# SuperbTUM/real-time-ReID-tracking

Hardware: AMD Instinct MI355X
Metric: crops/sec embedded + NxM distmat ms, ResNet18-SE 128x256 (higher is better)
Workload: dtype f16x3; 1 GPU; BASELINE configs[1]: ResNet18-SE embed 4096 distinct uint8 crops (128x256) per GPU + 4096x4096 L2 distmat; crops_per_gpu=4096, embed_dim=512, chunk=1024

## Files before the change

include/reid_hip_debug.h:

```cpp
#pragma once
#include "reid_hip.h"

#ifdef __cplusplus
extern "C" {
#endif

int reid_debug_set_switch(reid_ctx* ctx, const char* name, long long value);
int reid_debug_get_switch(reid_ctx* ctx, const char* name, long long* value);
int reid_debug_conv_f16(reid_ctx* ctx, int n, int h, int w, int cin, int cout, int r, int stride, int pad, int cfg, int iters,
                        float* ms_per_launch);
int reid_debug_conv_split(reid_ctx* ctx, int n, int h, int w, int c, int cout, int ablate, int iters, float* ms_per_launch);
int reid_debug_conv_f32(reid_ctx* ctx, int n, int h, int w, int cin, int cout, int r, int stride, int pad, int flags,
                        int variant, int iters, float* ms_per_launch);
int reid_debug_conv_c64(reid_ctx* ctx, int n, const float* x, const float* w_krsc, const float* scale, const float* shift,
                        const float* residual, int relu, float* out, float* stats);
int reid_debug_gemm_f16(reid_ctx* ctx, int m, int n, int k, int cfg, int iters, float* ms_per_launch,
                        unsigned long long* diag_host);
int reid_debug_linear(reid_ctx* ctx, int m, int n, int k, int mode, int iters, float* ms_per_launch);
int reid_debug_linear_rows(reid_ctx* ctx, const float* x, const float* w, const float* bias, const float* res, int m, int n, int k,
                           int mode, int flags, float* out);
int reid_debug_conv_layer(reid_ctx* ctx, const float* x, int n, int h, int w, int cin, const float* wgt, int cout, int r, int stride,
                          int pad, const float* scale, const float* shift, const float* residual, int relu, int relu_from, int pack_from,
                          int want_stats, const float* a_scale, const float* a_shift, int a_relu, float* out, uint16_t* packed,
                          float* stats, int* packed_written);
int reid_debug_conv_layer_f16(reid_ctx* ctx, const uint16_t* x, int n, int h, int w, int cin, const uint16_t* wgt, int cout, int r, int stride,
                              int pad, const float* scale, const float* shift, const uint16_t* residual, int relu, int want_stats,
                              uint16_t* out, float* stats, int* form);
int reid_debug_conv_c64_se(reid_ctx* ctx, int n, const uint16_t* x, const uint16_t* w_folded, const float* shift, const uint16_t* residual,
                           int relu, const float* se_w1, const float* se_w2t, uint16_t* out, float* stats, int* form);
int reid_debug_norm_finish(reid_ctx* ctx, int form, int n, int hw, int c, int half, int tiles, const void* x, const float* stats,
                           const float* in_gamma, const float* in_beta, const float* bn_scale, const float* bn_shift, float* out,
                           uint16_t* out16, float* a_scale, float* a_shift);
int reid_debug_se_tail(reid_ctx* ctx, int form, int n, int hw, int c, int mid, int tiles, const float* stats, const float* w1,
                       const float* w2t, const void* y, const void* shortcut, float* out, uint16_t* out16, float* gate);
int reid_debug_sibling_tail(reid_ctx* ctx, int arch, int n, int h, int w, int c, const float* prm, const float* y, const float* shortcut,
                            float* out);
int reid_debug_gem_neck(reid_ctx* ctx, int f16, int n, int hw, int c, float p, const void* x, const float* scale, const float* shift,
                        float* gem_out, float* emb);
int reid_debug_any_norm(reid_ctx* ctx, int n, int hw, int c, int half, const float* x, const float* in_gamma, const float* in_beta,
                        const float* bn_scale, const float* bn_shift, float* out);
int reid_debug_any_se_tail(reid_ctx* ctx, int n, int hw, int c, int mid, const float* w1, const float* w2t, const float* y,
                           const float* shortcut, float* out, float* gate);
int reid_debug_any_gem(reid_ctx* ctx, int n, int hw, int c, float p, const float* x, const float* scale, const float* shift, float* gem_out,
                       float* emb);
int reid_debug_any_conv(reid_ctx* ctx, int hw_precision, const float* x, int n, int h, int w, int cin, const float* wgt, int cout, int r,
                        int stride, int pad, const float* scale, const float* shift, const float* residual, int relu, int relu_from, float* out,
                        int* form_out);
int reid_debug_any_front(reid_ctx* ctx, int fused, const uint8_t* src, int64_t src_bytes, const int64_t* offsets, const int32_t* hw, int n,
                         int pitch, int out_h, int out_w, const float* mean_std6, const float* stem_w, const float* scale, const float* shift,
                         float* out);
int reid_debug_gem_neck_fused(reid_ctx* ctx, int n, int hw, int c, int mid, int tiles, float p, const float* stats, const float* w1,
                              const float* w2t, const float* y, const float* shortcut, const float* scale, const float* shift,
                              float* gem_out, float* emb);
int reid_debug_stem(reid_ctx* ctx, int form, int is_u8, const void* x, int n, const float* w, const float* scale, const float* shift,
                    float* out, uint16_t* out16);
int reid_debug_resize_norm(reid_ctx* ctx, const uint8_t* packed, const long long* offsets, const int* hw, int n, int pitch, float* out);
int reid_debug_swin_crop_front(reid_ctx* ctx, const uint8_t* packed, const long long* offsets, const int* hw, int n, int pitch, int out_h,
                               int out_w, const float* mean_std6, const float* c1_w, const float* c1_b, float* out);
int reid_debug_swin_conv1(reid_ctx* ctx, const float* x, int n, int h, int w, const float* c1_w, const float* c1_b, float* out);
int reid_debug_swin_conv1_mirror(reid_ctx* ctx, const float* x, int n, int h, int w, const float* c1_w, const float* c1_b, float* out);
int reid_debug_swin_crop_front_mirror(reid_ctx* ctx, const uint8_t* packed, const long long* offsets, const int* hw, int n, int pitch, int out_h,
                                      int out_w, const float* mean_std6, const float* c1_w, const float* c1_b, float* out);
int reid_debug_swin_descriptor(reid_ctx* ctx, const float* e1, const float* e2, const float* cls_w, int n, int num_class, int out_rows, int ld,
                               float* out);
int reid_debug_pil_resize(reid_ctx* ctx, const uint8_t* packed, const long long* offsets, const int* hw, int n, int out_h, int out_w,
                          const float* mean_std6, uint8_t* u8_out, float* f32_out);
int reid_debug_maxpool(reid_ctx* ctx, int f16, const void* x, int n, int h, int w, int c, void* out);
int reid_debug_window_attn_cos(reid_ctx* ctx, int mode, const float* qkv, int n, int h, int w, int heads, int shifted, const float* bias,
                               const float* scale, float* out, uint16_t* out16);
int reid_debug_post_norm(reid_ctx* ctx, int side, const float* x, const float* y, int t, int c, const float* g, const float* b, int in_place,
                         float* out, uint16_t* out16);
int reid_debug_window_attn(reid_ctx* ctx, int form, const float* qkv, int n, int h, int w, int heads, int shifted, const float* pos169,
                           float* out, uint16_t* out16);
int reid_debug_layernorm(reid_ctx* ctx, int form, const float* x, int t, int c, const float* g, const float* b, float* out, uint16_t* out16);
int reid_debug_ln_linear(reid_ctx* ctx, const float* x, const float* ln_g, const float* ln_b, const float* w, const float* bias, int t, int c,
                         int n, float* out);
int reid_debug_swin_linear(reid_ctx* ctx, const float* x, const float* w, const float* bias, const float* res, int m, int n, int k,
                           int precision, int flags, int out_form, int ldc, float* out, uint16_t* out16, int* form);
int reid_debug_swin_sfe(reid_ctx* ctx, const float* c1, int n, int h1, int w1, const float* in_g, const float* in_b, const float* bn_s,
                        const float* bn_t, const float* c2_w, const float* c2_b, const float* fc_w, const float* fc_b, float* ab, float* tok);
int reid_debug_swin_tail(reid_ctx* ctx, const float* x, int n, int ntok, const float* g, const float* b, float p, const float* bn_s,
                         const float* bn_t, float* gem, float* emb);
int reid_debug_swin_merge(reid_ctx* ctx, int stage, const float* x, int n, int h, int w, float* out);
int reid_debug_swin_fuse(reid_ctx* ctx, const float* sfe, const float* x1, const float* x2, const float* x3, const float* x4, int n, int h1,
                         int w1, void* a0, void* f3, void* f2, float* f1);
int reid_debug_bank_cost96(reid_ctx* ctx, reid_bank* bank, const int32_t* slots, int t, const float* dets_host, int m, int metric, float gate,
                           float* out_host);
// ... 24 lines not shown
```

real-time-reid-tracking_amd/_ffi.py:

```python
import ctypes as C
import os

_HERE = os.path.dirname(os.path.abspath(__file__))
LIB_PATH = os.path.join(_HERE, "libreid_hip.so")
LIB_PATH = os.environ.get("REID_HIP_LIB", LIB_PATH)

METRIC_L2, METRIC_L2SQR, METRIC_COS_HALF, METRIC_COS, METRIC_DOT = range(5)
COMM_ID_BYTES = 128
K_CONV_GEMM, K_DIST_GEMM, K_ELEMENTWISE, K_SELECT = range(4)

_vp, _i, _sz = C.c_void_p, C.c_int, C.c_size_t
_SIGS = {
    "reid_last_error": (C.c_char_p, []),
    "reid_device_count": (_i, [C.POINTER(_i)]),
    "reid_ctx_create": (_i, [_i, C.POINTER(_vp)]),
    "reid_ctx_destroy": (_i, [_vp]),
    "reid_ctx_set_stream": (_i, [_vp, _vp]),
    "reid_ctx_set_null_stream": (_i, [_vp]),
    "reid_ctx_sync": (_i, [_vp]),
    "reid_device_sync": (_i, [_vp]),
    "reid_ctx_clear_fault": (_i, [_vp]),
    "reid_ctx_set_chunk": (_i, [_vp, _i]),
    "reid_ctx_set_precision": (_i, [_vp, _i]),
    "reid_ctx_precision_ok": (_i, [_vp, _i, _i]),
# ... 46 lines not shown
    "reid_argmin_rows_x3": (_i, [_vp, _vp, _i, _vp, _i, _i, _i, _vp, _vp]),
    "reid_argmin_rows_x3_dev": (_i, [_vp, _vp, _i, _vp, _i, _i, _i, _vp, _vp]),
    "reid_knn_x3": (_i, [_vp, _vp, _i, _vp, _i, _i, _i, _vp, _vp]),
    "reid_knn_x3_dev": (_i, [_vp, _vp, _i, _vp, _i, _i, _i, _vp, _vp]),
    "reid_descriptor_f32_nchw": (_i, [_vp, _vp, _i, _i, _vp]),
    "reid_descriptor_f32_nchw_dev": (_i, [_vp, _vp, _i, _i, _vp]),
    "reid_descriptor_images_u8": (_i, [_vp, _vp, _vp, _vp, _i, _vp, _i, _vp]),
    "reid_descriptor_f32_nchw_hw": (_i, [_vp, _vp, _i, _i, _i, _i, _vp]),
    "reid_descriptor_f32_nchw_hw_dev": (_i, [_vp, _vp, _i, _i, _i, _i, _vp]),
    "reid_descriptor_images_u8_hw": (_i, [_vp, _vp, _vp, _vp, _i, _i, _i, _vp, _i, _vp]),
    "reid_cam_debias": (_i, [_vp, _vp, _vp, _i, _i, C.c_float, _i]),
    "reid_cam_debias_dev": (_i, [_vp, _vp, _vp, _i, _i, C.c_float, _i]),
    "reid_smooth_tracklets": (_i, [_vp, _vp, _vp, _vp, _i, _i, C.c_float]),
    "reid_smooth_tracklets_dev": (_i, [_vp, _vp, _vp, _vp, _i, _i, C.c_float]),
    "reid_bank_create": (_i, [_vp, _i, _i, _i, C.POINTER(_vp)]),
    "reid_bank_destroy": (_i, [_vp]),
    "reid_bank_update": (_i, [_vp, _vp, _vp, _vp, _i]),
    "reid_bank_update_dev": (_i, [_vp, _vp, _vp, _vp, _i]),
    "reid_bank_clear": (_i, [_vp, _vp, _vp, _i]),
    "reid_bank_count": (_i, [_vp, _i, C.POINTER(_i)]),
    "reid_bank_cost": (_i, [_vp, _vp, _vp, _i, _vp, _i, _i, C.c_float, _vp]),
    "reid_bank_cost_dev": (_i, [_vp, _vp, _vp, _i, _vp, _i, _i, C.c_float, _vp]),
    "reid_host_alloc": (_i, [_vp, _sz, C.POINTER(_vp)]),
    "reid_host_free": (_i, [_vp, _vp]),
    "reid_frame_submit": (_i, [_vp, _i, _vp, _vp, _vp, _i]),
    "reid_frame_submit_hw": (_i, [_vp, _i, _vp, _vp, _vp, _i, _i, _i, _vp]),
    "reid_frame_submit_swin": (_i, [_vp, _i, _vp, _vp, _vp, _i, _i, _i, _vp]),
    "reid_frame_cost": (_i, [_vp, _i, _vp, _vp, _i, _i, C.c_float, _vp, _vp, _i]),
    "reid_frame_cost_groups": (_i, [_vp, _i, _i, _vp, _vp, _vp, _vp, _i, C.c_float, _vp, _vp, _i]),
    "reid_frame_match_stream": (_i, [_vp, _i]),
    "reid_frame_fetch": (_i, [_vp, _i, _vp, _vp, _vp]),
    "reid_frame_gather": (_i, [_vp, _i, _i]),
    "reid_frame_update": (_i, [_vp, _i, _vp, _vp, _vp, _i]),
    "reid_rerank_jaccard": (_i, [_vp, _vp, _i, _i, _i, _i, _vp, _vp]),
    "reid_rerank_jaccard_dev": (_i, [_vp, _vp, _i, _i, _i, _i, _vp, _vp]),
    "reid_diou": (_i, [_vp, _vp, _vp, _i, _vp]),
    "reid_diou_cost": (_i, [_vp, _vp, _i, _vp, _i, _vp]),
    "reid_rank_eval": (_i, [_vp, _vp, _vp, _vp, _i, _vp, _vp, _vp, _i, _i, _vp, _vp, _vp]),
    "reid_rank_eval_dev": (_i, [_vp, _vp, _vp, _vp, _i, _vp, _vp, _vp, _i, _i, _vp, _vp, _vp]),
    "reid_comm_unique_id": (_i, [_vp]),
    "reid_comm_init": (_i, [_vp, _i, _i, _vp]),
    "reid_comm_info": (_i, [_vp, C.POINTER(_i), C.POINTER(_i)]),
    "reid_comm_destroy": (_i, [_vp]),
    "reid_allgather_dev": (_i, [_vp, _vp, _vp, _sz]),
    "reid_allgather_rows_dev": (_i, [_vp, _vp, _i, _sz, _vp, _vp, C.POINTER(_i)]),
    "reid_allreduce_f64": (_i, [_vp, C.POINTER(C.c_double), _i, _i]),
    "reid_knn_gallery_sharded_dev": (_i, [_vp, _vp, _i, _vp, _i, _i, _i, _i, _vp, _vp]),
    "reid_conv2d_nhwc": (_i, [_vp, _vp, _i, _i, _i, _i, _vp, _i, _i, _i, _i, _i, _vp, _vp, _vp, _i, _vp]),
    "reid_gemm_nt": (_i, [_vp, _vp, _i, _vp, _i, _i, _vp, _vp]),
}
EXPORTS = tuple(sorted(_SIGS))

DEBUG_LIB_PATH = os.path.join(_HERE, "libreid_hip_debug.so")
DEBUG_EXPORTS = ("reid_debug_any_conv", "reid_debug_any_front", "reid_debug_any_gem", "reid_debug_any_norm", "reid_debug_any_se_tail", "reid_debug_bank_cost96", "reid_debug_coissue", "reid_debug_comm_loopback", "reid_debug_conv_c64", "reid_debug_conv_c64_se", "reid_debug_conv_layer", "reid_debug_conv_layer_f16", "reid_debug_conv_split", "reid_debug_conv_diag", "reid_debug_conv_f16", "reid_debug_conv_f32",
                 "reid_debug_feed", "reid_debug_gem_neck", "reid_debug_gem_neck_fused", "reid_debug_gemm_f16", "reid_debug_knn_merge", "reid_debug_knn_wide", "reid_debug_layernorm", "reid_debug_linear", "reid_debug_linear_rows", "reid_debug_ln_linear", "reid_debug_maxpool", "reid_debug_mfma_bare", "reid_debug_mfma_shape", "reid_debug_norm_finish", "reid_debug_pil_resize", "reid_debug_post_norm", "reid_debug_resize_norm", "reid_debug_se_tail", "reid_debug_stem", "reid_debug_sibling_tail", "reid_debug_swin_conv1", "reid_debug_swin_conv1_mirror", "reid_debug_swin_crop_front", "reid_debug_swin_crop_front_mirror", "reid_debug_swin_descriptor", "reid_debug_swin_fuse", "reid_debug_swin_linear", "reid_debug_swin_merge", "reid_debug_swin_sfe", "reid_debug_swin_tail", "reid_debug_select_exp", "reid_debug_select_x3", "reid_debug_set_switch", "reid_debug_get_switch", "reid_debug_two_linear", "reid_debug_two_linear_ablate", "reid_debug_two_linear_form", "reid_debug_window_attn", "reid_debug_window_attn_cos")

_lib = None
_dbg = None


class ReidHipError(RuntimeError):
    status = None


def lib():
    global _lib
    if _lib is None:
        if not os.path.exists(LIB_PATH):
            raise ReidHipError(
                "HIP extension missing: %s (build it with `python -c 'import __graft_entry__ as g; g.build()'` "
                "or `make -C real-time-reid-tracking_amd/csrc`); there is no CPU fallback" % LIB_PATH)
        l = C.CDLL(LIB_PATH, mode=C.RTLD_GLOBAL)
        for name, (res, args) in _SIGS.items():
            fn = getattr(l, name)
            fn.restype = res
            fn.argtypes = args
        _lib = l
    return _lib


def debug_lib():
    global _dbg
    if _dbg is None:
        lib()
        if not os.path.exists(DEBUG_LIB_PATH):
            raise ReidHipError("debug library missing: %s (make -C real-time-reid-tracking_amd/csrc)" % DEBUG_LIB_PATH)
        _dbg = C.CDLL(DEBUG_LIB_PATH)
    return _dbg


def check(status):
    if status != 0:
        msg = lib().reid_last_error()
        err = ReidHipError("libreid_hip status %d: %s" % (status, msg.decode() if msg else "?"))
        err.status = int(status)
        raise err
```

real-time-reid-tracking_amd/csrc/api.hip:

```cpp
#include "reid_internal.h"
#include "siblings_f16.h"
#include "anysize.h"
#include "anysize_x3.h"
#include "distmat_x3.h"
#include "select_x3.h"
#include "anysize_front.h"
#include <cmath>
#include <dlfcn.h>
#include <mutex>
#include <stdarg.h>
#include <stdio.h>
#include <string.h>
#include <stdlib.h>
#include <sstream>

static thread_local char g_err[1024] = "";

void reid_set_error(const char* fmt, ...) {
    va_list ap;
    va_start(ap, fmt);
    vsnprintf(g_err, sizeof(g_err), fmt, ap);
    va_end(ap);
}

extern "C" const char* reid_last_error(void) { return g_err; }

extern "C" int reid_device_count(int* n) {
    ARG_CHECK(n);
    HIP_TRY(hipGetDeviceCount(n));
    return REID_OK;
}

extern "C" int reid_ctx_create(int device, reid_ctx** out) {
    ARG_CHECK(out);
    int n = 0;
    HIP_TRY(hipGetDeviceCount(&n));
    if (device < 0 || device >= n) {
        reid_set_error("reid_ctx_create: device %d not available (%d visible)", device, n);
        return REID_ERR_ARG;
    }
    DeviceGuard _dev_guard(device);
    reid_ctx* c = new reid_ctx();
    c->device = device;
    if (const char* e = getenv("REID_SWIN_CHUNK_MAX")) {
        const int v = atoi(e);
        if (v > 0 && v < c->swin_chunk_cap) c->swin_chunk_cap = v;
    }
    if (const char* e = getenv("REID_KNN_WIDE_MIN")) c->knn_wide_min = atoll(e);
    HIP_TRY(hipStreamCreateWithFlags(&c->own_stream, hipStreamNonBlocking));
    c->stream = c->own_stream;
    HIP_TRY(hipHostMalloc((void**)&c->fault, 64, hipHostMallocMapped));
    memset(c->fault, 0, 64);
    HIP_TRY(hipEventCreate(&c->t0));
    HIP_TRY(hipEventCreate(&c->t1));
    *out = c;
    return REID_OK;
}

extern "C" int reid_ctx_destroy(reid_ctx* ctx) {
    if (!ctx) return REID_OK;
    DeviceGuard _dev_guard(ctx->device);
// ... 492 lines not shown
        w.num_cams = (int)(cb->second.second / 512);
        w.cam_factor = blob[cf->second.first];
    }
    if (missing) {
        reid_set_error("reid_seres18_load: manifest entry '%s' missing or of unexpected size", first_missing.c_str());
        HIP_TRY(hipFree(w.blob));
        w = Se18Weights();
        return REID_ERR_ARG;
    }
    {
        std::vector<float> ep(8 * 1024, 0.f);
        for (int i = 0; i < 8; ++i) {
            const Se18Block& b = w.blk[i];
            const int half = b.ibn ? b.c / 2 : 0;
            for (int ch = 0; ch < b.c; ++ch) {
                ep[i * 1024 + ch] = ch < half ? 1.f : blob[(b.bn1_scale - w.blob) + (ch - half)];
                ep[i * 1024 + 512 + ch] = ch < half ? 0.f : blob[(b.bn1_shift - w.blob) + (ch - half)];
            }
        }
        HIP_TRY(hipMalloc((void**)&w.ep, ep.size() * sizeof(float)));
        HIP_TRY(hipMemcpy(w.ep, ep.data(), ep.size() * sizeof(float), hipMemcpyHostToDevice));
    }
    HIP_TRY(hipMalloc((void**)&w.blob16, n_floats * sizeof(_Float16)));
    HIP_TRY(hipMalloc((void**)&w.stem_w16, 64 * 256 * sizeof(_Float16)));
    HIP_TRY(hipMalloc((void**)&w.stem_w16s, 64 * 256 * sizeof(_Float16)));
    HIP_TRY(hipMalloc((void**)&w.zero_page, 256));
    HIP_TRY(hipMemsetAsync(w.zero_page, 0, 256, ctx->stream));
    REID_TRY(launch_f32_to_f16(ctx, w.blob, n_floats, w.blob16));
    REID_TRY(launch_stem_w16(ctx, w.stem_w, w.stem_w16));
    REID_TRY(launch_stem_w16_scaled(ctx, w.stem_w, w.stem_scale, w.stem_w16s));
    for (int i = 0; i < 2; ++i) {
        HIP_TRY(hipMalloc((void**)&w.l1_conv2_w16s[i], 64 * 576 * sizeof(_Float16)));
        REID_TRY(launch_scale_rows_f16(ctx, w.blk[i].conv2_w, w.blk[i].bn2_scale, 64, 576, w.l1_conv2_w16s[i]));
    }
    HIP_TRY(hipStreamSynchronize(ctx->stream));
    w.loaded = true;
    return REID_OK;
}

extern "C" int reid_seres18_dims(reid_ctx* ctx, int* embed_dim, int* num_class) {
    ARG_CHECK(ctx);
    CTX_GUARD(ctx);
    if (!ctx->se18.loaded) {
        reid_set_error("no weights loaded");
        return REID_ERR_STATE;
    }
    if (embed_dim) *embed_dim = 512;
    if (num_class) *num_class = ctx->se18.num_class;
    return REID_OK;
}

static const int IMG_H = 256, IMG_W = 128;

static bool conv_split_path(reid_ctx* ctx, int n, int H, int W, int Cin, int Cout, int R, int S, int stride, int pad) {
    if (ctx->precision != 2 || Cin % 64 != 0 || Cout % 64 != 0 || !ctx->se18.zero_page) return false;
    Gemm16Params q;
    memset(&q, 0, sizeof(q));
    q.H = H; q.W = W; q.Cin = ctx->split_terms * Cin; q.R = R; q.S = S; q.stride = stride; q.pad = pad;
    q.Ho = (H + 2 * pad - R) / stride + 1;
    q.Wo = (W + 2 * pad - S) / stride + 1;
    q.M = n * q.Ho * q.Wo; q.N = Cout;
    const bool halo = R == 3 && S == 3 && stride == 1 && pad == 1 && conv3x3_f16_supported(q);
    const bool enough = halo || (Cout % 128 == 0 && (long long)(q.M / 256) * (Cout / 128) >= (R == 3 ? ctx->split_gemm_min_tiles * 3 / 4 : ctx->split_gemm_min_tiles));
    if (q.M % 128 == 0 && !enough && !halo && ctx->conv_x3s == 2) {
        q.split_terms = ctx->split_terms; q.ldb = (long long)R * S * q.Cin; q.ldc = Cout;
        return conv_x3s_supported(ctx, q);
    }
    return q.M % 128 == 0 && enough;
}

int conv_gemm(reid_ctx* ctx, int amode, const void* x, int n, int H, int W, int Cin, const float* wgt, int Cout, int R,
                     int S, int stride, int pad, int Kpad, const float* a_scale, const float* a_shift, int a_relu,
                     const float* col_scale, const float* col_shift, const float* residual, int relu, float* stats,
                     float* out, int relu_from, const _Float16* x_packed, _Float16* out_packed, int pack_from, bool* packed_written) {
    if (packed_written) *packed_written = false;
    GemmParams p;
    memset(&p, 0, sizeof(p));
    p.A = x;
    p.H = H; p.W = W; p.Cin = Cin; p.R = R; p.S = S; p.stride = stride; p.pad_y = pad; p.pad_x = pad;
    p.Ho = (H + 2 * pad - R) / stride + 1;
    p.Wo = (W + 2 * pad - S) / stride + 1;
    p.a_scale = a_scale; p.a_shift = a_shift; p.a_relu = a_relu;
    p.B = wgt; p.ldb = Kpad;
    p.M = n * p.Ho * p.Wo; p.N = Cout; p.K = Kpad;
    p.C = out; p.ldc = Cout;
    p.col_scale = col_scale; p.col_shift = col_shift; p.residual = residual; p.relu = relu; p.stats = stats;
    p.relu_from = relu_from;
    p.diag = ctx->conv_diag;
    const double ktrue = (double)R * S * Cin;
    const double flops = 2.0 * p.M * Cout * ktrue;
    const double in_bytes = (double)n * H * W * Cin * (amode == A_STEM_U8 ? 1.0 : 4.0);
    const double bytes = in_bytes + ((double)p.M * Cout + (double)Cout * ktrue) * 4.0 + (residual ? (double)p.M * Cout * 4.0 : 0.0);
    if (amode == A_IM2COL && !a_scale && conv_split_path(ctx, n, H, W, Cin, Cout, R, S, stride, pad)) {
        Gemm16Params q;
        memset(&q, 0, sizeof(q));
        const int T = ctx->split_terms;
        q.split_terms = T;
        q.H = H; q.W = W; q.Cin = T * Cin; q.R = R; q.S = S; q.stride = stride; q.pad = pad;
        q.Ho = p.Ho; q.Wo = p.Wo;
        q.M = p.M; q.N = Cout; q.K = R * S * T * Cin; q.ldb = q.K;
        const bool halo = R == 3 && S == 3 && stride == 1 && pad == 1 && conv3x3_f16_supported(q);
        {
            const _Float16* a16 = x_packed;
            if (!a16) {
                _Float16* buf;
                const long long rows_in = (long long)n * H * W;
                REID_TRY(ctx_ws(ctx, "split.a", (size_t)rows_in * 2 * Cin * 2, (void**)&buf));
// ... 11 lines not shown
            q.B = (const _Float16*)it->second;
            q.C32 = out; q.ldc = Cout;
            q.col_scale = col_scale; q.col_shift = col_shift; q.res32 = residual; q.relu = relu; q.relu_from = relu_from;
            q.stats = stats;
            q.acc_scale = 1.0f / 2048.0f;
            q.zero_page = ctx->se18.zero_page;
            if (out_packed && packed_written && pack_from % 32 == 0) {
                q.pack16 = out_packed;
                q.pack_from = pack_from;
                *packed_written = true;
            }
            if (halo) return launch_conv3x3_split(ctx, q, REID_K_CONV_GEMM, flops, bytes);
            if (conv_x3s_supported(ctx, q)) return launch_conv_x3s(ctx, q, REID_K_CONV_GEMM, flops, bytes);
            return launch_gemm_f16_split(ctx, q, REID_K_CONV_GEMM, flops, bytes);
        }
    }
    if (amode == A_IM2COL && ctx->f32_conv && conv_f32_supported(p)) return launch_conv_f32(ctx, p, REID_K_CONV_GEMM, flops, bytes);
    return launch_gemm_f32(ctx, amode, E_CONV, p, REID_K_CONV_GEMM, flops, bytes);
}

int conv_weights_fresh(reid_ctx* ctx, const float* d_w) {
    auto it = ctx->split_w.find(d_w);
    if (it != ctx->split_w.end()) {
        HIP_TRY(hipStreamSynchronize(ctx->stream));
        (void)hipFree(it->second);
        ctx->split_w.erase(it);
    }
    return REID_OK;
}

int conv_weights_splittable(reid_ctx* ctx, const float* h_w, size_t count, const char* who) {
    if (ctx->precision != 2) return REID_OK;
    for (size_t i = 0; i < count; ++i)
        if (!(fabsf(h_w[i]) * 2048.0f < 65504.0f)) {
            reid_set_error("%s: weight %zu (%g) is outside the range the fp32-class arithmetic (reid_ctx_set_precision 2) can split "
                           "(|w| 2^11 < 65504); use mode 0", who, i, (double)h_w[i]);
            return REID_ERR_ARG;
        }
    return REID_OK;
}

static int split_weights_of(reid_ctx* ctx, const float* wgt, int Cout, int taps, int Cin, const _Float16** out) {
    auto it = ctx->split_w.find(wgt);
    if (it == ctx->split_w.end()) {
        void* w16;
        HIP_TRY(hipMalloc(&w16, (size_t)Cout * taps * ctx->split_terms * Cin * 2));
        REID_TRY(launch_split_weights(ctx, wgt, Cout, taps, Cin, ctx->split_terms, (_Float16*)w16));
        it = ctx->split_w.emplace(wgt, w16).first;
    }
    *out = (const _Float16*)it->second;
    return REID_OK;
}

#ifdef REID_EXPERIMENTS
static int seres18_chain_layer4(reid_ctx* ctx, int n, const Se18Block& ka, const Se18Block& kb, const _Float16* in16, const float* sc,
                                float* y, float* out_a, float* out, float* stats) {
    const int H = 16, W = 8, hw = 128, C = 512, SK = 4, nnt = C / 128;
    const int nmt = (n * hw + 255) / 256;
    _Float16 *c1_16, *a16;
    float* skws;
    int* cnt;
    REID_TRY(ctx_ws(ctx, "split.c1", (size_t)n * hw * C * 2 * 2, (void**)&c1_16));
    REID_TRY(ctx_ws(ctx, "chain.a16", (size_t)n * hw * C * 2 * 2, (void**)&a16));
    const size_t part = (size_t)nmt * nnt * SK * 256 * 128;
    REID_TRY(ctx_ws(ctx, "chain.splitk", 4 * part * sizeof(float), (void**)&skws));
    const bool fresh = ctx->ws.find("chain.cnt") == ctx->ws.end();
    REID_TRY(ctx_ws(ctx, "chain.cnt", (4 * 1024 + 64 + 8 * 64) * sizeof(int), (void**)&cnt));
    if (fresh) HIP_TRY(hipMemsetAsync(cnt, 0, (4 * 1024 + 64 + 8 * 64) * sizeof(int), ctx->stream));
    ChainParams cp;
    memset(&cp, 0, sizeof(cp));
    cp.n_img = n;
    cp.flags = ctx->chain;
    cp.counters = cnt + 4 * 1024;
    cp.fault = ctx->fault;
    auto conv = [&](int idx, const _Float16* a, int cin, const float* wgt, const float* scale, const float* shift, const float* res, int relu,
                    float* stats_out, _Float16* pack) -> int {
        Gemm16Params& q = cp.conv[idx];
        q.H = H; q.W = W; q.Cin = 3 * cin; q.R = 3; q.S = 3; q.stride = 1; q.pad = 1; q.Ho = H; q.Wo = W;
        q.M = n * hw; q.N = C; q.K = 9 * 3 * cin; q.ldb = q.K;
        q.split_terms = 3;
        q.A = a;
        REID_TRY(split_weights_of(ctx, wgt, C, 9, cin, &q.B));
        q.C32 = y; q.ldc = C;
        q.col_scale = scale; q.col_shift = shift; q.res32 = res; q.relu = relu; q.relu_from = 0;
        q.stats = stats_out;
        q.acc_scale = 1.0f / 2048.0f;
        q.zero_page = ctx->se18.zero_page;
        q.pack16 = pack; q.pack_from = 0;
        q.split_k = SK; q.splitk_ws = skws + (size_t)idx * part; q.splitk_cnt = cnt + idx * 1024;
        q.fault = ctx->fault;
        return REID_OK;
    };
    REID_TRY(conv(0, in16, ka.cin, ka.conv1_w, ka.bn1_scale, ka.bn1_shift, nullptr, 1, nullptr, c1_16));
    REID_TRY(conv(1, c1_16, C, ka.conv2_w, ka.bn2_scale, ka.bn2_shift, nullptr, 0, stats, nullptr));
    REID_TRY(conv(2, a16, C, kb.conv1_w, kb.bn1_scale, kb.bn1_shift, nullptr, 1, nullptr, c1_16));
    REID_TRY(conv(3, c1_16, C, kb.conv2_w, kb.bn2_scale, kb.bn2_shift, out_a, 1, stats, nullptr));
    const int slices = 2;
    auto se = [&](int idx, const Se18Block& k, const float* shortcut, float* o, _Float16* pk) {
        ChainElem& e = cp.el[idx];
        e.x = y; e.stats = stats; e.sc = shortcut; e.g = k.se_w1; e.b = k.se_w2; e.out = o; e.packed = pk;
        e.c = C; e.half = 0; e.hw = hw; e.tiles = 1; e.mid = k.mid; e.slices = slices;
    };
    se(0, ka, sc, out_a, a16);
    se(1, kb, out_a, out, nullptr);
    const int conv_items = nmt * nnt * SK, se_items = n * slices;
    const int kinds[6] = {0, 0, 2, 0, 0, 2}, idxs[6] = {0, 1, 0, 2, 3, 1};
    const int targets[6] = {0, nnt * SK, nnt * SK, slices, nnt * SK, nnt * SK};
    int first = 0;
    for (int s = 0; s < 6; ++s) {
        ChainStage& st = cp.st[s];
        st.kind = kinds[s]; st.idx = idxs[s]; st.first = first; st.items = kinds[s] == 0 ? conv_items : se_items;
        st.dep = s - 1; st.target = targets[s]; st.sk = SK;
        first += st.items;
    }
    cp.n_stages = 6;
    cp.total_items = first;
    prof_begin(ctx, REID_K_CONV_GEMM, 2.0 * n * hw * C * 9.0 * (ka.cin + 3.0 * C), 0.0);
    const int st = launch_chain(ctx, cp, W);
    prof_end(ctx);
    return st;
}
#endif

struct Se18Bufs {
    float *stem, *pool, *t[4], *stats, *a_scale, *a_shift, *se, *gem;
    float* stage[11];
};

static int seres18_forward(reid_ctx* ctx, const void* x, bool is_u8, int n, float* d_emb, float* d_logits) {
    Se18Weights& w = ctx->se18;
    if (!w.loaded) {
        reid_set_error("reid_embed_*: call reid_seres18_load first");
        return REID_ERR_STATE;
    }
    Se18Bufs b;
    const size_t per = 131072;
    const bool keep = ctx->debug_keep != 0;
    REID_TRY(ctx_ws(ctx, "se18.stem", (size_t)n * 524288 * 4, (void**)&b.stem));
    REID_TRY(ctx_ws(ctx, "se18.pool", (size_t)n * per * 4, (void**)&b.pool));
    const int nt = keep ? 1 : 4;
    float* tbase = nullptr;
    REID_TRY(ctx_ws(ctx, "se18.t", (size_t)n * per * 4 * (keep ? 4 * 8 : 4), (void**)&tbase));
    REID_TRY(ctx_ws(ctx, "se18.stats", (size_t)n * 2048 * 4, (void**)&b.stats));
    REID_TRY(ctx_ws(ctx, "se18.ascale", (size_t)n * 512 * 4, (void**)&b.a_scale));
    REID_TRY(ctx_ws(ctx, "se18.ashift", (size_t)n * 512 * 4, (void**)&b.a_shift));
    REID_TRY(ctx_ws(ctx, "se18.se", (size_t)n * 512 * 4, (void**)&b.se));
    REID_TRY(ctx_ws(ctx, "se18.gem", (size_t)n * 512 * 4, (void**)&b.gem));
    (void)nt;

    const bool pool_fused = ctx->f32_conv == 1 && ctx->f32_stem_pool && ctx->debug_keep != 1;
    _Float16* cur16 = nullptr;
    const bool split_mode = ctx->precision == 2 && w.arch == 0 && ctx->f32_conv == 1;
    if (split_mode) REID_TRY(ctx_ws(ctx, "split.cur", (size_t)n * per * 2 * 2, (void**)&cur16));
    const bool stem_split = split_mode && pool_fused && ctx->stem_split;
    if (stem_split) {
        REID_TRY(launch_stem_split(ctx, x, is_u8, n, w.stem_w, w.stem_scale, w.stem_shift, b.pool, cur16));
    } else if (pool_fused) {
        REID_TRY(launch_stem_f32(ctx, x, is_u8, n, w.stem_w, w.stem_scale, w.stem_shift, b.pool, true));
    } else if (ctx->f32_conv == 1) {
        REID_TRY(launch_stem_f32(ctx, x, is_u8, n, w.stem_w, w.stem_scale, w.stem_shift, b.stem, false));
    } else {
        REID_TRY(conv_gemm(ctx, is_u8 ? A_STEM_U8 : A_STEM_F32, x, n, IMG_H, IMG_W, 3, w.stem_w, 64, 7, 7, 2, 3, 192, nullptr,
                           nullptr, 0, w.stem_scale, w.stem_shift, nullptr, 0, nullptr, b.stem));
    }
    if (!pool_fused) REID_TRY(launch_maxpool3s2(ctx, b.stem, n, 128, 64, 64, b.pool));
    b.stage[0] = b.stem;
    b.stage[1] = b.pool;

    const float* cur = b.pool;
    int H = 64, W = 32;
    bool gem_done = false;
    if (split_mode && !stem_split) REID_TRY(launch_split_pack(ctx, b.pool, (long long)n * 64 * 32, 64, cur16));
    for (int i = 0; i < 8; ++i) {
        const Se18Block& k = w.blk[i];
#ifdef REID_EXPERIMENTS
        if (i == 6 && (ctx->chain & 1) && cur16 && !keep && n <= 64 && ctx->pack_epilogue && ctx->split_terms == 3) {
            float* fr[3];
            int nf = 0;
            for (int j = 0; j < 4 && nf < 3; ++j)
                if (tbase + (size_t)j * n * per != cur) fr[nf++] = tbase + (size_t)j * n * per;
            float *sc = fr[0], *y = fr[1], *out_a = fr[2], *out = const_cast<float*>(cur);
            REID_TRY(conv_gemm(ctx, A_IM2COL, cur, n, H, W, k.cin, k.ds_w, k.c, 1, 1, k.stride, 0, k.cin, nullptr, nullptr, 0, k.ds_scale, k.ds_shift,
                               nullptr, 0, nullptr, sc, 0, cur16));
            REID_TRY(seres18_chain_layer4(ctx, n, k, w.blk[7], cur16, sc, y, out_a, out, b.stats));
            b.stage[8] = out_a;
            b.stage[9] = out;
            cur = out;
            break;
        }
#endif
        float* tb[4];
        for (int j = 0; j < 4; ++j) tb[j] = tbase + ((size_t)(keep ? i * 4 : 0) + j) * n * per;
        float* free_[3];
        int nf = 0;
        for (int j = 0; j < 4 && nf < 3; ++j)
            if (tb[j] != cur) free_[nf++] = tb[j];
        float* c1 = free_[0];
        float* y = free_[1];
        float* sc = free_[2];
        const int Ho = (H + 2 - 3) / k.stride + 1, Wo = (W + 2 - 3) / k.stride + 1;
        const int hw = Ho * Wo, tiles = hw / 128;
        const int half = k.ibn ? k.c / 2 : 0;
        _Float16* c1_16 = nullptr;
        if (ctx->f32_conv == 1) {
            bool packed_c1 = false;
            if (cur16 && !keep && ctx->pack_epilogue) REID_TRY(ctx_ws(ctx, "split.c1", (size_t)n * hw * k.c * 2 * 2, (void**)&c1_16));
            if (k.ibn) {
                REID_TRY(conv_gemm(ctx, A_IM2COL, cur, n, H, W, k.cin, k.conv1_w, k.c, 3, 3, k.stride, 1, 9 * k.cin, nullptr, nullptr,
                                   0, w.ep + (size_t)i * 1024, w.ep + (size_t)i * 1024 + 512, nullptr, 1, b.stats, c1, half, cur16,
                                   c1_16, half, &packed_c1));
                if (cur16 && !keep) {
                    if (!c1_16) REID_TRY(ctx_ws(ctx, "split.c1", (size_t)n * hw * k.c * 2 * 2, (void**)&c1_16));
                    REID_TRY(launch_in_apply_pack(ctx, c1, b.stats, n, tiles, k.c, half, hw, k.in_gamma, k.in_beta, c1_16, packed_c1));
                } else {
                    REID_TRY(launch_in_apply(ctx, c1, b.stats, n, tiles, k.c, half, hw, k.in_gamma, k.in_beta));
                }
            } else {
                REID_TRY(conv_gemm(ctx, A_IM2COL, cur, n, H, W, k.cin, k.conv1_w, k.c, 3, 3, k.stride, 1, 9 * k.cin, nullptr, nullptr,
                                   0, k.bn1_scale, k.bn1_shift, nullptr, 1, nullptr, c1, 0, cur16, c1_16, 0, &packed_c1));
                if (!packed_c1) c1_16 = nullptr;
            }
            REID_TRY(conv_gemm(ctx, A_IM2COL, c1, n, Ho, Wo, k.c, k.conv2_w, k.c, 3, 3, 1, 1, 9 * k.c, nullptr, nullptr, 0,
                               k.bn2_scale, k.bn2_shift, k.ds ? nullptr : cur, k.ds ? 0 : 1, b.stats, y, 0, c1_16));
        } else {
        REID_TRY(conv_gemm(ctx, A_IM2COL, cur, n, H, W, k.cin, k.conv1_w, k.c, 3, 3, k.stride, 1, 9 * k.cin, nullptr, nullptr, 0,
                           nullptr, nullptr, nullptr, 0, b.stats, c1));
        REID_TRY(launch_norm_finalize(ctx, b.stats, n, tiles, k.c, half, hw, k.in_gamma, k.in_beta, k.bn1_scale, k.bn1_shift,
                                      b.a_scale, b.a_shift));
        REID_TRY(conv_gemm(ctx, A_IM2COL, c1, n, Ho, Wo, k.c, k.conv2_w, k.c, 3, 3, 1, 1, 9 * k.c, b.a_scale, b.a_shift, 1,
                           k.bn2_scale, k.bn2_shift, k.ds ? nullptr : cur, k.ds ? 0 : 1, b.stats, y));
        }
        const float* shortcut = cur;
        if (k.ds) {
            REID_TRY(conv_gemm(ctx, A_IM2COL, cur, n, H, W, k.cin, k.ds_w, k.c, 1, 1, k.stride, 0, k.cin, nullptr, nullptr, 0,
                               k.ds_scale, k.ds_shift, nullptr, 0, nullptr, sc, 0, cur16));
            shortcut = sc;
        }
        float* out = c1;
        if (w.arch == 1) {
            REID_TRY(launch_ta_tail(ctx, y, shortcut, n, Ho, Wo, k.c, k.ta, out));
        } else if (w.arch == 2) {
            REID_TRY(launch_ema_tail(ctx, y, shortcut, n, Ho, Wo, k.c, k.ema, out));
        } else if (ctx->f32_conv == 1) {
            bool fp32_read = true;
            if (cur16 && !keep && i < 7 && w.blk[i + 1].ds && ctx->pack_epilogue) {
                const Se18Block& nx = w.blk[i + 1];
                fp32_read = !(conv_split_path(ctx, n, Ho, Wo, nx.cin, nx.c, 3, 3, nx.stride, 1) &&
                              conv_split_path(ctx, n, Ho, Wo, nx.cin, nx.c, 1, 1, nx.stride, 0));
            }
            if (i == 7 && !keep && n >= ctx->gem_tail_min) {
                REID_TRY(launch_gem_neck_tail(ctx, b.stats, n, tiles, k.c, k.mid, hw, k.se_w1, k.se_w2, y, shortcut, w.gem_p, w.neck_scale,
                                              w.neck_shift, b.gem, d_emb));
                gem_done = true;
            } else {
                REID_TRY(launch_se_tail(ctx, b.stats, n, tiles, k.c, k.mid, hw, k.se_w1, k.se_w2, y, shortcut, fp32_read ? out : nullptr,
                                        i < 7 ? cur16 : nullptr));
            }
        } else {
            REID_TRY(launch_se_finalize(ctx, b.stats, n, tiles, k.c, k.mid, hw, k.se_w1, k.se_w2, b.se));
            REID_TRY(launch_se_combine(ctx, y, shortcut, b.se, n, hw, k.c, out));
        }
        b.stage[2 + i] = out;
        cur = out;
        H = Ho;
        W = Wo;
    }
    if (!gem_done) REID_TRY(launch_gem_neck(ctx, cur, n, H * W, 512, w.gem_p, w.neck_scale, w.neck_shift, b.gem, d_emb));
    {
        const int32_t* d_cam;
        REID_TRY(ctx_take_side(ctx, n, w.num_cams, "reid_embed (camera bias)", &d_cam));
        if (d_cam) REID_TRY(launch_add_indexed_rows(ctx, d_emb, n, 1, 512, w.cam_bias, d_cam, w.cam_factor));
    }
    b.stage[10] = b.gem;
    if (d_logits) {
        if (!w.cls_w) {
            reid_set_error("logits requested but the weight blob has no classifier (cls.w)");
            return REID_ERR_STATE;
        }
        GemmParams p;
        memset(&p, 0, sizeof(p));
        p.A = d_emb; p.lda = 512;
        p.B = w.cls_w; p.ldb = 512;
        p.M = n; p.N = w.num_class; p.K = 512;
        p.C = d_logits; p.ldc = w.num_class;
        REID_TRY(launch_gemm_f32(ctx, A_DENSE, E_BIAS, p, REID_K_CONV_GEMM, 2.0 * n * w.num_class * 512,
                                 ((double)n * 512 + (double)w.num_class * 512 + (double)n * w.num_class) * 4.0));
    }
    ctx->last_n = n;
    ctx->last_f16 = false;
    for (int s = 0; s < 11; ++s) { ctx->stage_ptr[s] = b.stage[s]; ctx->stage_elems[s] = 0; }
    return REID_OK;
}

int open_beside_self(const char* file, const char* what, std::initializer_list<const char*> names, void** fns) {
    Dl_info info;
    std::string path = file;
    if (dladdr((const void*)&open_beside_self, &info) && info.dli_fname) {
        const std::string self = info.dli_fname;
        const size_t slash = self.rfind('/');
        if (slash != std::string::npos) path = self.substr(0, slash + 1) + path;
    }
    void* h = dlopen(path.c_str(), RTLD_NOW | RTLD_LOCAL);
    if (!h) {
// ... 1465 lines not shown
```

real-time-reid-tracking_amd/csrc/conv3x3_x3.hip:

```cpp
#include "reid_internal.h"
#include "conv3x3_geom.h"
#include "lin_math.h"
#include <type_traits>
#include <utility>

typedef _Float16 f16;
typedef f16 half8 __attribute__((ext_vector_type(8)));
typedef float f32x16 __attribute__((ext_vector_type(16)));

namespace {

#define GPTR(p) ((const __attribute__((address_space(1))) void*)(p))
#define LPTR(p) ((__attribute__((address_space(3))) void*)(uintptr_t)(p))
#define RAW_BARRIER() asm volatile("s_barrier" ::: "memory")
#define LDS_READ(dst, addr, off) asm volatile("ds_read_b128 %0, %1 offset:%2" : "=v"(dst) : "v"(addr), "n"(off))

template <int N>
__device__ __forceinline__ void lgkm_wait2(half8& x, half8& y) { asm volatile("s_waitcnt lgkmcnt(%2)" : "+v"(x), "+v"(y) : "n"(N)); }
template <int N>
__device__ __forceinline__ void lgkm_wait1(half8& x) { asm volatile("s_waitcnt lgkmcnt(%1)" : "+v"(x) : "n"(N)); }

__device__ __forceinline__ void wait_vm(int n) {
    switch (n) {
        case 0: asm volatile("s_waitcnt vmcnt(0)" ::: "memory"); break;
// ... 263 lines not shown
                            dst[p.N] = (f16)((v - (float)hv) * 2048.0f);
                        } else {
                            p.C32[(long long)(m_blk + row) * ldc + col] = v;
                        }
                    }
                }
            }
            s1[b] = t1;
            s2[b] = t2;
        }
    }
    if (p.fault && !(vmax < 65504.f)) p.fault[0] = 1;
    if (p.stats) {
        float* stat_lds = (float*)lds;
#pragma unroll
        for (int b = 0; b < TN; ++b) {
            const int lcol = b * 32 + li;
            const float t1 = s1[b] + __shfl_xor(s1[b], 32);
            const float t2 = s2[b] + __shfl_xor(s2[b], 32);
            if (lh == 0) {
                stat_lds[(wm * BN + lcol) * 2 + 0] = t1;
                stat_lds[(wm * BN + lcol) * 2 + 1] = t2;
            }
        }
        __syncthreads();
        for (int t = tid; t < 2 * BN; t += 256) {
            const int half = t / BN, cc = t - half * BN;
            if (half * 128 >= m_valid) continue;
            float* o = p.stats + ((long long)(mtile * 2 + half) * p.N + n_blk + cc) * 2;
            o[0] = stat_lds[((half * 2) * BN + cc) * 2 + 0] + stat_lds[((half * 2 + 1) * BN + cc) * 2 + 0];
            o[1] = stat_lds[((half * 2) * BN + cc) * 2 + 1] + stat_lds[((half * 2 + 1) * BN + cc) * 2 + 1];
        }
    }
}

typedef float f32x4 __attribute__((ext_vector_type(4)));

__device__ __forceinline__ int pi16(int i) { return i < 8 ? i : (i < 12 ? i + 4 : i - 4); }

typedef unsigned u32x2 __attribute__((ext_vector_type(2)));
typedef unsigned u32x4 __attribute__((ext_vector_type(4)));

__device__ __forceinline__ float row16_sum(float v) {
    v += __builtin_bit_cast(float, __builtin_amdgcn_update_dpp(0, __builtin_bit_cast(int, v), 0xB1, 0xf, 0xf, false));
    v += __builtin_bit_cast(float, __builtin_amdgcn_update_dpp(0, __builtin_bit_cast(int, v), 0x4E, 0xf, 0xf, false));
    v += __builtin_bit_cast(float, __builtin_amdgcn_update_dpp(0, __builtin_bit_cast(int, v), 0x141, 0xf, 0xf, false));
    v += __builtin_bit_cast(float, __builtin_amdgcn_update_dpp(0, __builtin_bit_cast(int, v), 0x140, 0xf, 0xf, false));
    return v;
}

template <int N>
__device__ __forceinline__ void lgkm_wait0() { asm volatile("s_waitcnt lgkmcnt(%0)" ::"n"(N) : "memory"); }

template <int TW, int IMGS, int BN, bool LIN = false, int COH = 0>
__device__ __forceinline__ void x3m16_tail(const Gemm16Params& p, f32x4 (&acc)[4][BN / 16], char* lds, int tid, int wm, int mtile, int n_blk,
                                           int tile_id, int ksplit, int SK) {
    constexpr int TM = 4, TN = BN / 16;
    const int lane = tid & 63;
    const int l16 = lane & 15, lq = lane >> 4;
    const int pj = pi16(l16);
    asm volatile("s_nop 15\n\ts_nop 15" ::: "memory");
#pragma unroll
    for (int a = 0; a < TM; ++a) {
        if constexpr (TN == 8)
            asm volatile("" : "+v"(acc[a][0]), "+v"(acc[a][1]), "+v"(acc[a][2]), "+v"(acc[a][3]), "+v"(acc[a][4]), "+v"(acc[a][5]), "+v"(acc[a][6]), "+v"(acc[a][7]));
        else
            asm volatile("" : "+v"(acc[a][0]), "+v"(acc[a][1]), "+v"(acc[a][2]), "+v"(acc[a][3]));
    }
    __syncthreads();

    bool sk_path = false;
    if (SK > 1) {
        sk_path = true;
        constexpr int PART_B = 256 * BN * 4;
        char* part = (char*)(p.splitk_ws + (long long)tile_id * SK * (256 * BN));
        const __amdgpu_buffer_rsrc_t w_rs = __builtin_amdgcn_make_buffer_rsrc((void*)part, 0, SK * PART_B, 0x00020000);
        const int nb_own = TN / SK;
        const unsigned own32 = (unsigned)(uintptr_t)lds + 4096u + (unsigned)tid * 16u;
#pragma unroll
        for (int a = 0; a < TM; ++a)
#pragma unroll
            for (int b = 0; b < TN; ++b) {
                if (b / nb_own == ksplit)
                    asm volatile("ds_write_b128 %0, %1" ::"v"(own32 + (unsigned)((a * nb_own + (b - ksplit * nb_own)) * 4096)), "v"(acc[a][b]) : "memory");
                else
                    __builtin_amdgcn_raw_buffer_store_b128(__builtin_bit_cast(u32x4, acc[a][b]), w_rs, tid * 16, ksplit * PART_B + (a * TN + b) * 4096, 16 );
            }
        asm volatile("s_waitcnt vmcnt(0)" ::: "memory");
        __syncthreads();
        if (tid == 0) {
            __hip_atomic_fetch_add(p.splitk_cnt + tile_id, 1, __ATOMIC_RELAXED, __HIP_MEMORY_SCOPE_AGENT);
            int spins = 0;
            while (__hip_atomic_load(p.splitk_cnt + tile_id, __ATOMIC_RELAXED, __HIP_MEMORY_SCOPE_AGENT) < SK) {
                __builtin_amdgcn_s_sleep(1);
                if (++spins > (1 << 23)) {
                    if (p.fault) p.fault[2] = 1;
                    break;
                }
            }
        }
        __syncthreads();
    }

    if (p.ablate & 32) return;
    const int ldc = (int)p.ldc;
    const int m_blk = mtile * 256;
    const int m_valid = p.M - m_blk;
    const bool wave_live = wm * 64 < m_valid;
    const int pq = lq < 2 ? lq : 5 - lq;
    const int lrow = TW == 8 ? 32 * (pj >> 3) + (pj & 7) : pj;
    const int col0 = n_blk + 4 * pq;
    const __amdgpu_buffer_rsrc_t c_rs = __builtin_amdgcn_make_buffer_rsrc((void*)(p.C32 + (long long)m_blk * ldc), 0, 256 * ldc * 4, 0x00020000);
    const __amdgpu_buffer_rsrc_t r_rs =
        __builtin_amdgcn_make_buffer_rsrc((void*)((p.res32 ? p.res32 : p.C32) + (long long)m_blk * ldc), 0, 256 * ldc * 4, 0x00020000);
    const __amdgpu_buffer_rsrc_t k_rs =
        __builtin_amdgcn_make_buffer_rsrc((void*)((p.pack16 ? p.pack16 : (f16*)p.C32) + (long long)m_blk * 2 * p.N), 0, 256 * 2 * p.N * 2, 0x00020000);
    int voff_a[TM], koff_a[TM];
#pragma unroll
    for (int a = 0; a < TM; ++a) {
        const bool row_ok = wm * 64 + (TW == 8 ? a * 8 : a * 16) + lrow < m_valid;
        voff_a[a] = row_ok ? (lrow * ldc + col0) * 4 : 0x7fffff00;
        koff_a[a] = row_ok ? (lrow * 2 * p.N + col0) * 2 : 0x7fffff00;
    }
    const bool has_stats = p.stats != nullptr;
    float vmax = 0.f;
    auto run = [&](auto res_c, auto st_c) {
        constexpr bool RES = decltype(res_c)::value, ST = decltype(st_c)::value;
#pragma unroll
        for (int b = 0; b < TN; ++b) {
            const int col = col0 + b * 16, tcol = n_blk + b * 16;
            f32x4 cs = f32x4{p.acc_scale, p.acc_scale, p.acc_scale, p.acc_scale}, sh = f32x4{0.f, 0.f, 0.f, 0.f};
            if (p.col_scale) {
                cs = *(const f32x4*)(p.col_scale + col) * p.acc_scale;
                sh = *(const f32x4*)(p.col_shift + col);
            } else if (LIN && p.col_shift) {
                sh = *(const f32x4*)(p.col_shift + col);
            }
            const bool gelu = LIN && p.act == 1;
            const float lo = (p.relu && tcol >= p.relu_from) ? 0.f : -INFINITY;
            const bool pk = p.pack16 && tcol >= p.pack_from;
            constexpr int AB = BN == 64 ? 4 : 1;
            f32x4 t1 = f32x4{0.f, 0.f, 0.f, 0.f}, t2 = f32x4{0.f, 0.f, 0.f, 0.f};
#pragma unroll
            for (int a0 = 0; a0 < TM; a0 += AB) {
                f32x4 v[AB];
#pragma unroll
                for (int i = 0; i < AB; ++i) {
                    const int a = a0 + i;
                    v[i] = acc[a][b] * cs + sh;
                    if (gelu) {
                        const gelu_f32x2 g0 = gelu2_f16_storage(gelu_f32x2{v[i][0], v[i][1]}), g1 = gelu2_f16_storage(gelu_f32x2{v[i][2], v[i][3]});
                        v[i] = f32x4{g0.x, g0.y, g1.x, g1.y};
                    }
                    if constexpr (RES)
                        v[i] += __builtin_bit_cast(f32x4, __builtin_amdgcn_raw_buffer_load_b128(r_rs, voff_a[a] + b * 64, (wm * 64 + (TW == 8 ? a * 8 : a * 16)) * ldc * 4, COH));
                    if (!LIN) {
#pragma unroll
                        for (int e = 0; e < 4; ++e) v[i][e] = fmaxf(v[i][e], lo);
                    }
                    if constexpr (ST) {
                        t1 += v[i];
                        t2 += v[i] * v[i];
                    }
                }
                if (pk) {
#pragma unroll
                    for (int i = 0; i < AB; ++i) {
                        const int ubase = wm * 64 + (TW == 8 ? (a0 + i) * 8 : (a0 + i) * 16);
                        u32x2 hw, lw;
#pragma unroll
                        for (int h = 0; h < 2; ++h) {
                            const float v0 = v[i][2 * h], v1 = v[i][2 * h + 1];
                            vmax = fmaxf(vmax, fmaxf(fabsf(v0), fabsf(v1)));
                            const f16 h0 = cvt_f16_rn(v0), h1 = cvt_f16_rn(v1);
                            const f16 l0 = cvt_f16_rn((v0 - (float)h0) * 2048.0f), l1 = cvt_f16_rn((v1 - (float)h1) * 2048.0f);
                            hw[h] = (unsigned)__builtin_bit_cast(unsigned short, h0) | ((unsigned)__builtin_bit_cast(unsigned short, h1) << 16);
                            lw[h] = (unsigned)__builtin_bit_cast(unsigned short, l0) | ((unsigned)__builtin_bit_cast(unsigned short, l1) << 16);
                        }
                        __builtin_amdgcn_raw_buffer_store_b64(hw, k_rs, koff_a[a0 + i] + b * 32, ubase * 2 * p.N * 2, COH);
                        __builtin_amdgcn_raw_buffer_store_b64(lw, k_rs, koff_a[a0 + i] + b * 32 + p.N * 2, ubase * 2 * p.N * 2, COH);
// ... 69 lines not shown
                    rr[a] = __builtin_bit_cast(f32x4, __builtin_amdgcn_raw_buffer_load_b128(r_rs, voff_a[a] + b * 64, (wm * 64 + (TW == 8 ? a * 8 : a * 16)) * ldc * 4, COH));
            }
#pragma unroll
            for (int a = 0; a < TM; ++a) {
                f32x4 x = v[a] * cs + sh;
                if constexpr (RES) x += rr[a];
                if (pk) vm_sk = range_acc(range_acc(range_acc(range_acc(vm_sk, x[0]), x[1]), x[2]), x[3]);
#pragma unroll
                for (int e = 0; e < 4; ++e) x[e] = fmaxf(x[e], lo);
                if constexpr (ST) {
                    t1 += x;
                    t2 += x * x;
                }
                const int ubase = wm * 64 + (TW == 8 ? a * 8 : a * 16);
                if (pk) {
                    u32x2 hw, lw;
#pragma unroll
                    for (int h = 0; h < 2; ++h) {
                        const float v0 = x[2 * h], v1 = x[2 * h + 1];
                        const f16 h0 = cvt_f16_rn(v0), h1 = cvt_f16_rn(v1);
                        const f16 l0 = cvt_f16_rn((v0 - (float)h0) * 2048.0f), l1 = cvt_f16_rn((v1 - (float)h1) * 2048.0f);
                        hw[h] = (unsigned)__builtin_bit_cast(unsigned short, h0) | ((unsigned)__builtin_bit_cast(unsigned short, h1) << 16);
                        lw[h] = (unsigned)__builtin_bit_cast(unsigned short, l0) | ((unsigned)__builtin_bit_cast(unsigned short, l1) << 16);
                    }
                    __builtin_amdgcn_raw_buffer_store_b64(hw, k_rs, koff_a[a] + b * 32, ubase * 2 * p.N * 2, COH);
                    __builtin_amdgcn_raw_buffer_store_b64(lw, k_rs, koff_a[a] + b * 32 + p.N * 2, ubase * 2 * p.N * 2, COH);
                } else {
                    __builtin_amdgcn_raw_buffer_store_b128(__builtin_bit_cast(u32x4, x), c_rs, voff_a[a] + b * 64, ubase * ldc * 4, COH);
                }
            }
            if constexpr (ST) {
                float* stat_lds = (float*)lds;
#pragma unroll
                for (int e = 0; e < 4; ++e) {
                    const float r1 = row16_sum(t1[e]), r2 = row16_sum(t2[e]);
                    if (l16 == 0) {
                        const int lcol = b * 16 + 4 * pq + e;
                        stat_lds[(wm * BN + lcol) * 2 + 0] = r1;
                        stat_lds[(wm * BN + lcol) * 2 + 1] = r2;
                    }
                }
            }
        }
    };
    auto run_sk_n = [&](auto sk_c) {
        if (p.res32) {
            if (has_stats) run_sk(sk_c, std::true_type{}, std::true_type{});
            else run_sk(sk_c, std::true_type{}, std::false_type{});
        } else {
            if (has_stats) run_sk(sk_c, std::false_type{}, std::true_type{});
            else run_sk(sk_c, std::false_type{}, std::false_type{});
        }
    };
    if (sk_path) {
        if constexpr (!LIN) {
            if (wave_live) {
                if (SK == 2) run_sk_n(std::integral_constant<int, 2>{});
                else if (SK == 4) run_sk_n(std::integral_constant<int, 4>{});
                else if constexpr (TN == 8) run_sk_n(std::integral_constant<int, 8>{});
            }
            range_raise(p.fault, vm_sk);
        }
    } else if (wave_live) {
        if (p.res32) {
            if (has_stats) run(std::true_type{}, std::true_type{});
            else run(std::true_type{}, std::false_type{});
        } else {
            if (has_stats) run(std::false_type{}, std::true_type{});
            else run(std::false_type{}, std::false_type{});
        }
    }
    if (p.fault && !(vmax < 65504.f)) p.fault[0] = 1;
    if (sk_path) {
        __syncthreads();
        if (tid == 0) {
            const int old = __hip_atomic_fetch_add(p.splitk_cnt + 512 + tile_id, 1, __ATOMIC_RELAXED, __HIP_MEMORY_SCOPE_AGENT);
            if (old == SK - 1) {
                __hip_atomic_store(p.splitk_cnt + tile_id, 0, __ATOMIC_RELAXED, __HIP_MEMORY_SCOPE_AGENT);
                __hip_atomic_store(p.splitk_cnt + 512 + tile_id, 0, __ATOMIC_RELAXED, __HIP_MEMORY_SCOPE_AGENT);
            }
        }
    }
    if (has_stats) {
        const float* stat_lds = (const float*)lds;
        __syncthreads();
        const int cc_lo = sk_path ? ksplit * (BN / SK) : 0, cc_hi = sk_path ? cc_lo + BN / SK : BN;
        for (int t = tid; t < 2 * BN; t += 256) {
            const int half = t / BN, cc = t - half * BN;
            if (half * 128 >= m_valid || cc < cc_lo || cc >= cc_hi) continue;
            float* o = p.stats + ((long long)(mtile * 2 + half) * p.N + n_blk + cc) * 2;
            const float o0 = stat_lds[((half * 2) * BN + cc) * 2 + 0] + stat_lds[((half * 2 + 1) * BN + cc) * 2 + 0];
            const float o1 = stat_lds[((half * 2) * BN + cc) * 2 + 1] + stat_lds[((half * 2 + 1) * BN + cc) * 2 + 1];
            if constexpr (COH != 0) {
                __hip_atomic_store(o, o0, __ATOMIC_RELAXED, __HIP_MEMORY_SCOPE_AGENT);
                __hip_atomic_store(o + 1, o1, __ATOMIC_RELAXED, __HIP_MEMORY_SCOPE_AGENT);
            } else {
                o[0] = o0;
                o[1] = o1;
            }
        }
    }
}

template <int TW, int IMGS, int BN, int COH, class WaitFn>
__device__ __forceinline__ void x3m16_item(const Gemm16Params& p, char* lds, int tile_id, int ksplit, int SK, WaitFn&& wait_deps) {
    constexpr int TH = 256 / (IMGS * TW);
    constexpr int WP = TW + 2, HP = TH + 2;
    constexpr int NPX = IMGS * HP * WP;
    constexpr int NPI = (NPX + 15) / 16;
    static_assert(NPI <= 24, "one halo piece per wave and tile over six tiles");
    constexpr int HALO_BYTES = NPI * 1024;
    constexpr int B_BYTES = BN * 64;
    constexpr int BJ = BN / 64;
    constexpr int TM = 4, TN = BN / 16;
    constexpr int NS = 4;
    constexpr int NHB = BN == 64 ? 1 : 2;
    static_assert((BN == 64 ? 4 : 2) * (NHB * HALO_BYTES + NS * B_BYTES) <= 160 * 1024, "blocks per CU");

    const int tid = threadIdx.x, lane = tid & 63;
    const int wm = __builtin_amdgcn_readfirstlane(tid >> 6);
    const int l16 = lane & 15, lq = lane >> 4;

// ... 791 lines not shown
            if (!last) issue_w(c + 1, 1, (s0 + 3) & 3);
            const unsigned ba = bx + (unsigned)(((s0 + 1) & 3) * B_SLOT);
            if (!(abl & 4)) { LIN_B_READS(fb, ba); }
            lgkm_wait1<7>(fb[0]); MMA(0, 0);
            lgkm_wait1<6>(fb[1]); MMA(0, 1);
            lgkm_wait1<5>(fb[2]); MMA(0, 2);
            lgkm_wait1<4>(fb[3]); MMA(0, 3);
            lgkm_wait1<3>(fb[4]); MMA(0, 4);
            lgkm_wait1<2>(fb[5]); MMA(0, 5);
            lgkm_wait1<1>(fb[6]); MMA(0, 6);
            lgkm_wait1<0>(fb[7]); MMA(0, 7);
#pragma unroll
            for (int b = 0; b < TN; ++b) MMA(1, b);
#pragma unroll
            for (int b = 0; b < TN; ++b) MMA(2, b);
#pragma unroll
            for (int b = 0; b < TN; ++b) MMA(3, b);
        }
        {
            if (last) wait_vm_imm<0>(); else wait_vm_imm<2 * BJ + 4>();
            RAW_BARRIER();
            if (!last) issue_a(2 * c + 3, sa_h);
            const unsigned ao = (unsigned)(sa_l * A_SLOT);
            if (!(abl & 4)) {
                LDS_READ(fa[0], aa[0] + ao, 0);
                LDS_READ(fa[1], aa[1] + ao, 0);
                LDS_READ(fa[2], aa[2] + ao, 0);
                LDS_READ(fa[3], aa[3] + ao, 0);
            }
            lgkm_wait1<3>(fa[0]);
#pragma unroll
            for (int b = 0; b < TN; ++b) MMAW(0, b);
            lgkm_wait1<2>(fa[1]);
#pragma unroll
            for (int b = 0; b < TN; ++b) MMAW(1, b);
            lgkm_wait1<1>(fa[2]);
#pragma unroll
            for (int b = 0; b < TN; ++b) MMAW(2, b);
            lgkm_wait1<0>(fa[3]);
#pragma unroll
            for (int b = 0; b < TN; ++b) MMAW(3, b);
        }
#undef LIN_B_READS
#undef MMAW
#undef MMA
        const int nh = sa_h == 0 ? 2 : sa_h - 1;
        sa_l = sa_h;
        sa_h = nh;
    }
    x3m16_tail<16, 1, BN, true>(p, acc, lds, tid, wm, mtile, n_blk, 0, 0, 1);
#endif
}

template <int BN>
__global__ __launch_bounds__(256, 2) void conv_x3s_kernel(const Gemm16Params p) {
#if defined(__HIP_DEVICE_COMPILE__)
    constexpr int TM = 4, TN = BN / 16, BJ = BN / 64;
    constexpr int A_SLOT = 256 * 64, B_SLOT = BN * 64;
    static_assert(2 * (3 * A_SLOT + 4 * B_SLOT) <= 160 * 1024, "two blocks per CU");
    static_assert(TN == 8, "fragment reads below are written for the 128-wide tile");
    __shared__ __attribute__((aligned(16))) char lds[3 * A_SLOT + 4 * B_SLOT];
    const int tid = threadIdx.x, lane = tid & 63;
    const int wm = __builtin_amdgcn_readfirstlane(tid >> 6);
    const int l16 = lane & 15, lq = lane >> 4;
    const int nnt = p.N / BN;
    const int SK = p.split_k > 1 ? p.split_k : 1;
    int mtile, ntile, tile_id, ksplit;
    {
        const int nwg = gridDim.x, b = blockIdx.x, xcd = b & 7, q = nwg >> 3, r = nwg & 7;
        const int L = (xcd < r ? xcd * (q + 1) : r * (q + 1) + (xcd - r) * q) + (b >> 3);
        tile_id = L / SK;
        ksplit = L - tile_id * SK;
        mtile = tile_id / nnt;
        ntile = tile_id - mtile * nnt;
    }
    const int m_blk = mtile * 256, n_blk = ntile * BN;
    const int m_valid = p.M - m_blk < 256 ? p.M - m_blk : 256;
    const int C = p.Cin / 3;
    const int ncr = C / 32;
    const int nq = p.R * p.S * ncr;
    const int q0 = ksplit * nq / SK, q1 = (ksplit + 1) * nq / SK;
    const int pix_b = 2 * C * 2;
    const unsigned a32 = (unsigned)(uintptr_t)lds, b32 = a32 + 3 * A_SLOT;

    const int n_img = p.M / (p.Ho * p.Wo);
    const __amdgpu_buffer_rsrc_t a_rs = __builtin_amdgcn_make_buffer_rsrc((void*)p.A, 0, (int)((long long)n_img * p.H * p.W * pix_b), 0x00020000);
    const __amdgpu_buffer_rsrc_t w_rs =
        __builtin_amdgcn_make_buffer_rsrc((void*)(p.B + (long long)n_blk * p.ldb), 0, (int)((long long)BN * p.ldb * 2), 0x00020000);
    int av[4], rmask[4], cmask[4], wv[BJ];
#pragma unroll
    for (int j = 0; j < 4; ++j) {
        const int row = (wm * 4 + j) * 16 + (lane >> 2);
        const int cg = (lane & 3) ^ (((row >> 3) & 1) << 1);
        const int m = m_blk + row;
        const int img = m / (p.Ho * p.Wo), rem = m - img * (p.Ho * p.Wo);
        const int oy = rem / p.Wo, ox = rem - oy * p.Wo;
        const int iy0 = oy * p.stride - p.pad, ix0 = ox * p.stride - p.pad;
        av[j] = ((img * p.H + iy0) * p.W + ix0) * pix_b + cg * 16;
        int rm = 0, cm = 0;
        if (row < m_valid) {
#pragma unroll
            for (int t = 0; t < 3; ++t) {
                rm |= ((unsigned)(iy0 + t) < (unsigned)p.H && t < p.R) ? 1 << t : 0;
                cm |= ((unsigned)(ix0 + t) < (unsigned)p.W && t < p.S) ? 1 << t : 0;
            }
        }
        rmask[j] = rm; cmask[j] = cm;
    }
// ... 83 lines not shown
        {
            if (last) wait_vm_imm<4>(); else wait_vm_imm<BJ + 8>();
            RAW_BARRIER();
            if (!last) issue_w(nt, nc, 1, (s0 + 3) & 3);
            const unsigned ba = bx + (unsigned)(((s0 + 1) & 3) * B_SLOT);
            LIN_B_READS(fb, ba);
            lgkm_wait1<7>(fb[0]); MMA(0, 0);
            lgkm_wait1<6>(fb[1]); MMA(0, 1);
            lgkm_wait1<5>(fb[2]); MMA(0, 2);
            lgkm_wait1<4>(fb[3]); MMA(0, 3);
            lgkm_wait1<3>(fb[4]); MMA(0, 4);
            lgkm_wait1<2>(fb[5]); MMA(0, 5);
            lgkm_wait1<1>(fb[6]); MMA(0, 6);
            lgkm_wait1<0>(fb[7]); MMA(0, 7);
#pragma unroll
            for (int b = 0; b < TN; ++b) MMA(1, b);
#pragma unroll
            for (int b = 0; b < TN; ++b) MMA(2, b);
#pragma unroll
            for (int b = 0; b < TN; ++b) MMA(3, b);
        }
        {
            if (last) wait_vm_imm<0>(); else wait_vm_imm<2 * BJ + 4>();
            RAW_BARRIER();
            if (!last) {
                issue_a(nr, ns, nc, 1, sa_h);
                advance();
            }
            const unsigned ao = (unsigned)(sa_l * A_SLOT);
            LDS_READ(fa[0], aa[0] + ao, 0);
            LDS_READ(fa[1], aa[1] + ao, 0);
            LDS_READ(fa[2], aa[2] + ao, 0);
            LDS_READ(fa[3], aa[3] + ao, 0);
            lgkm_wait1<3>(fa[0]);
#pragma unroll
            for (int b = 0; b < TN; ++b) MMAW(0, b);
            lgkm_wait1<2>(fa[1]);
#pragma unroll
            for (int b = 0; b < TN; ++b) MMAW(1, b);
            lgkm_wait1<1>(fa[2]);
#pragma unroll
            for (int b = 0; b < TN; ++b) MMAW(2, b);
            lgkm_wait1<0>(fa[3]);
#pragma unroll
            for (int b = 0; b < TN; ++b) MMAW(3, b);
        }
#undef LIN_B_READS
#undef MMAW
#undef MMA
        const int nh = sa_h == 0 ? 2 : sa_h - 1;
        sa_l = sa_h;
        sa_h = nh;
    }
    x3m16_tail<16, 1, BN, false>(p, acc, lds, tid, wm, mtile, n_blk, tile_id, ksplit, SK);
#endif
}

static int x3_split(const reid_ctx* ctx, int tiles, int ncr, bool wide, int slots = 512) {
    int sk = 1;
    while (ctx->f16_split_k && tiles * sk * 2 <= slots && ncr % (sk * 2) == 0 && sk * 2 <= (wide ? 8 : 4)) sk *= 2;
    const int cap = ctx->x3_sk_cap > 0 ? ctx->x3_sk_cap : 4;
    return sk > cap ? cap : sk;
}

static bool x3_wide_tiles(const reid_ctx* ctx, const Gemm16Params& p) {
    if (p.N % 128 != 0 || (p.W == 16 && (ctx->x3_narrow & 1)) || (p.W == 8 && (ctx->x3_narrow & 2))) return false;
    if (p.W == 8 && p.N == 256 && !(ctx->x3_narrow & 4)) {
        const int nmt = (p.M + 255) / 256, ncr = p.Cin / 3 / 32;
        const int t128 = nmt * 2, t64 = nmt * 4;
        const int s128 = x3_split(ctx, t128, ncr, true);
        (void)t64;
        if (t128 * s128 < 256) return false;
    }
    if (p.W == 8 && p.N == 512 && ctx->x3_l4_narrow_nmt > 0) {
        const int nmt = (p.M + 255) / 256, ncr = p.Cin / 3 / 32;
        const int t128 = nmt * 4, s128 = x3_split(ctx, t128, ncr, true);
        if (s128 == 4 && t128 * s128 > 256 && nmt <= ctx->x3_l4_narrow_nmt) return false;
        if (s128 == 1 && t128 % 256 != 0 && t128 % 256 <= 128) return false;
        if (s128 == 2 && t128 > 128 && t128 * 4 <= 768) return false;
    }
    return true;
}

static int x3_slots(const Gemm16Params& p, bool wide) { return (!wide && p.W == 8 && p.N == 512 && (p.M + 255) / 256 > 32) ? 768 : 512; }

template <int TW, int IMGS>
int launch_x3m16(reid_ctx* ctx, const Gemm16Params& p0) {
    Gemm16Params p = p0;
    const int nmt = (p.M + 255) / 256;
    const bool wide = x3_wide_tiles(ctx, p);
    const int tiles = nmt * (wide ? p.N / 128 : p.N / 64);
    const int sk = x3_split(ctx, tiles, p.Cin / 3 / 32, wide, x3_slots(p, wide));
    if (sk > 1) {
        float* ws;
        int* cnt;
        const bool fresh = ctx->ws.find("x3.splitk_cnt") == ctx->ws.end();
        ARG_CHECK(tiles <= 512);
        REID_TRY(ctx_ws(ctx, "x3.splitk_ws", (size_t)tiles * sk * 256 * (wide ? 128 : 64) * sizeof(float), (void**)&ws));
        REID_TRY(ctx_ws(ctx, "x3.splitk_cnt", 1024 * sizeof(int), (void**)&cnt));
        if (fresh) HIP_TRY(hipMemsetAsync(cnt, 0, 1024 * sizeof(int), ctx->stream));
        p.split_k = sk; p.splitk_ws = ws; p.splitk_cnt = cnt;
    } else {
        p.split_k = 1;
    }
    const bool unrolled = ctx->x3_unroll && (long long)p.M * (p.Cin / 3) * 4 < 0x7f000000ll && (long long)p.N * p.ldb * 2 < 0x7f000000ll;
    if (wide && unrolled) hipLaunchKernelGGL((conv3x3_x3u_kernel<TW, IMGS, 128, 2>), dim3(tiles * sk), dim3(256), 0, ctx->stream, p);
    else if (wide) hipLaunchKernelGGL((conv3x3_x3m16_kernel<TW, IMGS, 128>), dim3(tiles * sk), dim3(256), 0, ctx->stream, p);
    else if (unrolled && ctx->x3_unroll == 3) hipLaunchKernelGGL((conv3x3_x3u_kernel<TW, IMGS, 64, 3>), dim3(tiles * sk), dim3(256), 0, ctx->stream, p);
#ifdef REID_EXPERIMENTS
// ... 17 lines not shown
    const int nmt = (p.M + 255) / 256;
    return nmt * (x3_wide_tiles(ctx, p) ? p.N / 128 : p.N / 64);
}

bool conv3x3_x3_supported(const reid_ctx* ctx, const Gemm16Params& p) {
    if (!ctx->split_x3 || p.split_terms != 3 || p.Cin % 96 != 0 || p.N % 64 != 0 || p.M % 128 != 0 || !conv3x3_f16_supported(p)) return false;
    if (p.relu_from % 16 != 0 || (p.pack16 && p.pack_from % 32 != 0)) return false;
    if (p.N % 128 != 0 && ctx->split_x3 < 3) return false;
    const int nmt = (p.M + 255) / 256;
    const long long blocks = (long long)nmt * (p.N % 128 == 0 ? p.N / 128 : p.N / 64);
    if (blocks >= ctx->split_x3_min_blocks) return true;
    if (ctx->split_x3 < 2 || !ctx->split_x3_small) return false;
    if (ctx->split_x3_small == 1) return true;
    const int tiles = launch_tiles(ctx, p);
    if (p.W == 8) return true;
    if (p.W == 32) return p.M / 256 > 256 || tiles >= 384;
    return p.M / 256 > 128 || tiles >= 384;
}

int launch_conv3x3_x3(reid_ctx* ctx, const Gemm16Params& p0) {
    Gemm16Params p = p0;
    p.fault = ctx->fault;
    p.ablate |= ctx->x3_ablate;
    if (ctx->split_x3 >= 2) {
        if (p.W == 32) REID_TRY((launch_x3m16<32, 1>(ctx, p)));
        else if (p.W == 16) REID_TRY((launch_x3m16<16, 1>(ctx, p)));
        else REID_TRY((launch_x3m16<8, 2>(ctx, p)));
    } else if (p.W == 32) launch_x3<32, 1>(ctx, p);
    else if (p.W == 16) launch_x3<16, 1>(ctx, p);
    else launch_x3<8, 2>(ctx, p);
    LAUNCH_CHECK();
    return REID_OK;
}

#ifdef REID_EXPERIMENTS
int launch_chain(reid_ctx* ctx, const ChainParams& cp, int W) {
    ARG_CHECK(cp.n_img >= 1 && cp.n_img <= 64 && cp.n_stages >= 1 && cp.n_stages <= 8 && cp.counters && W == 8);
    const int blocks = cp.total_items < 512 ? cp.total_items : 512;
    hipLaunchKernelGGL((chain_kernel<8, 2, 128>), dim3(blocks), dim3(256), 0, ctx->stream, cp);
    LAUNCH_CHECK();
    return REID_OK;
}
#endif

bool conv_x3s_supported(const reid_ctx* ctx, const Gemm16Params& p) {
    if (!ctx->conv_x3s || ctx->split_x3 < 2 || p.split_terms != 3 || p.Cin % 96 != 0 || p.N % 128 != 0 || p.M % 128 != 0) return false;
    if (!((p.R == 1 || p.R == 3) && p.S == p.R && p.pad == (p.R - 1) / 2 && (p.stride == 1 || p.stride == 2))) return false;
    if (p.R == 3 && p.stride == 1) return false;
    if (p.relu_from % 16 != 0 || (p.pack16 && p.pack_from % 32 != 0)) return false;
    const long long a_bytes = (long long)(p.M / (p.Ho * p.Wo)) * p.H * p.W * (p.Cin / 3) * 4;
    return a_bytes < 0x7f000000ll && 128ll * p.ldb * 2 < 0x7f000000ll && 256ll * p.ldc * 4 < 0x7f000000ll && (long long)p.M * 2 < 0x7f000000ll;
}

int launch_conv_x3s(reid_ctx* ctx, const Gemm16Params& p0, int kind, double flops, double bytes) {
    Gemm16Params p = p0;
    p.fault = ctx->fault;
    p.ablate = 0;
    const int tiles = ((p.M + 255) / 256) * (p.N / 128), nq = p.R * p.S * (p.Cin / 3 / 32);
    int sk = 1;
    while (ctx->f16_split_k && tiles * sk * 2 <= 512 && nq / (sk * 2) >= 2 && sk * 2 <= ctx->x3s_sk_cap) sk *= 2;
    if (sk > 1) {
        float* ws;
        int* cnt;
        const bool fresh = ctx->ws.find("x3.splitk_cnt") == ctx->ws.end();
        ARG_CHECK(tiles <= 512);
        REID_TRY(ctx_ws(ctx, "x3.splitk_ws", (size_t)tiles * sk * 256 * 128 * sizeof(float), (void**)&ws));
        REID_TRY(ctx_ws(ctx, "x3.splitk_cnt", 1024 * sizeof(int), (void**)&cnt));
        if (fresh) HIP_TRY(hipMemsetAsync(cnt, 0, 1024 * sizeof(int), ctx->stream));
        p.split_k = sk; p.splitk_ws = ws; p.splitk_cnt = cnt;
    } else {
        p.split_k = 1;
    }
    prof_begin(ctx, kind, flops, bytes);
    hipLaunchKernelGGL((conv_x3s_kernel<128>), dim3(tiles * sk), dim3(256), 0, ctx->stream, p);
    prof_end(ctx);
    LAUNCH_CHECK();
    return REID_OK;
}

bool lin_x3_supported(const reid_ctx* ctx, const Gemm16Params& p) {
    const int Kr = p.K / 3;
    return ctx->lin_x3 && ctx->split_x3 >= 2 && p.lin && p.split_terms == 3 && p.K % 96 == 0 && p.N % 128 == 0 && p.n_real == p.N && p.lda == 2 * Kr &&
           p.ldb == 3 * Kr && !p.scat_h && !p.par4 && (p.C32 != nullptr) != (p.pack_out != 0) &&
           256ll * p.lda * 2 < 0x7f000000ll && 128ll * p.ldb * 2 < 0x7f000000ll && 256ll * p.ldc * 4 < 0x7f000000ll;
}

int launch_lin_x3(reid_ctx* ctx, const Gemm16Params& p0, int kind, double flops, double bytes) {
    Gemm16Params p = p0;
    p.fault = ctx->fault;
    p.ablate = ctx->x3_ablate;
    p.stats = nullptr; p.col_scale = nullptr; p.relu = 0; p.split_k = 1;
    if (p.pack_out) {
        p.pack16 = p.C;
        p.pack_from = 0;
        p.C32 = nullptr;
    } else {
        p.pack16 = nullptr;
    }
    prof_begin(ctx, kind, flops, bytes);
    hipLaunchKernelGGL((lin_x3_kernel<128>), dim3(((p.M + 255) / 256) * (p.N / 128)), dim3(256), 0, ctx->stream, p);
    ctx->conv_form = 7128000;
    prof_end(ctx);
    LAUNCH_CHECK();
    return REID_OK;
}
```

real-time-reid-tracking_amd/csrc/debug.hip:

```cpp
#include "reid_internal.h"
#include "pil_launch.h"
#include <string.h>
#include <stdlib.h>
#include <vector>

namespace {
struct Switch { const char* name; int reid_ctx::* field; };
const Switch kSwitches[] = {
    {"f16_cfg", &reid_ctx::f16_cfg}, {"f16_lin_256", &reid_ctx::f16_lin_256}, {"f16_split_k", &reid_ctx::f16_split_k},
    {"bank_fast", &reid_ctx::bank_fast}, {"side_copy", &reid_ctx::side_copy}, {"f32_stem_pool", &reid_ctx::f32_stem_pool},
    {"stem_split", &reid_ctx::stem_split}, {"split_pair", &reid_ctx::split_pair}, {"split_lean_epi", &reid_ctx::split_lean_epi},
    {"knn_wide", &reid_ctx::knn_wide}, {"f16_loader_prio", &reid_ctx::f16_loader_prio}, {"f16_frag_ahead", &reid_ctx::f16_frag_ahead},
    {"pack_epilogue", &reid_ctx::pack_epilogue}, {"f16_wide_splitk", &reid_ctx::f16_wide_splitk}, {"f32_split_k", &reid_ctx::f32_split_k},
    {"swin_fold", &reid_ctx::swin_fold}, {"swin_stop", &reid_ctx::swin_stop}, {"select_two_pass", &reid_ctx::select_two_pass},
    {"split_terms", &reid_ctx::split_terms}, {"f32_conv", &reid_ctx::f32_conv}, {"swin_attn_mfma", &reid_ctx::swin_attn_mfma},
    {"swin_attn_split", &reid_ctx::swin_attn_split}, {"swin_two_linear", &reid_ctx::swin_two_linear},
    {"f16_loader_waves", &reid_ctx::f16_loader_waves}, {"f16_halo", &reid_ctx::f16_halo}, {"f16_stem_fused", &reid_ctx::f16_stem_fused},
    {"f16_se_tail", &reid_ctx::f16_se_tail}, {"f16_c64", &reid_ctx::f16_c64}, {"swin_chunk_cap", &reid_ctx::swin_chunk_cap},
    {"split_x3", &reid_ctx::split_x3}, {"x3_ablate", &reid_ctx::x3_ablate}, {"x3_unroll", &reid_ctx::x3_unroll}, {"x3_narrow", &reid_ctx::x3_narrow}, {"conv_x3s", &reid_ctx::conv_x3s}, {"x3s_sk_cap", &reid_ctx::x3s_sk_cap}, {"x3_l4_narrow_nmt", &reid_ctx::x3_l4_narrow_nmt}, {"split_x3_small", &reid_ctx::split_x3_small}, {"split_x3_min_blocks", &reid_ctx::split_x3_min_blocks}, {"f32_dist_bk16", &reid_ctx::f32_dist_bk16}, {"lin_x3", &reid_ctx::lin_x3},
    {"host_pipeline", &reid_ctx::host_pipeline}, {"x3_sk_cap", &reid_ctx::x3_sk_cap}, {"chain", &reid_ctx::chain}, {"split_gemm_min_tiles", &reid_ctx::split_gemm_min_tiles},
    {"rerank_hbm_acc", &reid_ctx::rerank_hbm_acc}, {"gem_tail_min", &reid_ctx::gem_tail_min}, {"anysize_force", &reid_ctx::anysize_force},
    {"any_front", &reid_ctx::any_front},
};
}

extern "C" int reid_debug_set_switch(reid_ctx* ctx, const char* name, long long value) {
    ARG_CHECK(ctx && name);
    CTX_GUARD(ctx);
    HIP_TRY(hipStreamSynchronize(ctx->stream));
    if (!strcmp(name, "knn_wide_min")) {
        ctx->knn_wide_min = value;
        return REID_OK;
    }
    for (const Switch& s : kSwitches)
        if (!strcmp(name, s.name)) {
            if (!strcmp(name, "split_terms") && value != 3 && value != 4) break;
            ctx->*(s.field) = (int)value;
            return REID_OK;
        }
    reid_set_error("reid_debug_set_switch: no switch '%s' (or a value it does not take)", name);
    return REID_ERR_ARG;
}

extern "C" int reid_debug_get_switch(reid_ctx* ctx, const char* name, long long* value) {
    ARG_CHECK(ctx && name && value);
    if (!strcmp(name, "knn_wide_min")) {
        *value = ctx->knn_wide_min;
        return REID_OK;
    }
    for (const Switch& s : kSwitches)
        if (!strcmp(name, s.name)) {
            *value = ctx->*(s.field);
            return REID_OK;
        }
    reid_set_error("reid_debug_get_switch: no switch '%s'", name);
    return REID_ERR_ARG;
}

extern "C" int reid_debug_conv_f16(reid_ctx* ctx, int n, int h, int w, int cin, int cout, int r, int stride, int pad, int cfg,
                                   int iters, float* ms_per_launch) {
    ARG_CHECK(ctx && ms_per_launch && ctx->se18.loaded);
    CTX_GUARD(ctx);
    typedef _Float16 f16;
    const int ho = (h + 2 * pad - r) / stride + 1, wo = (w + 2 * pad - r) / stride + 1;
    const size_t nin = (size_t)n * h * w * cin, nw = (size_t)cout * r * r * cin, nout = (size_t)n * ho * wo * cout;
    f16 *x, *wt, *out;
    REID_TRY(ctx_ws(ctx, "dbg.x", nin * 2, (void**)&x));
    REID_TRY(ctx_ws(ctx, "dbg.w", nw * 2, (void**)&wt));
    REID_TRY(ctx_ws(ctx, "dbg.out", nout * 2, (void**)&out));
    const size_t src_n = ctx->se18.n_floats;
    for (size_t o = 0; o < nin; o += src_n) REID_TRY(launch_f32_to_f16(ctx, ctx->se18.blob, nin - o < src_n ? nin - o : src_n, x + o));
    for (size_t o = 0; o < nw; o += src_n) REID_TRY(launch_f32_to_f16(ctx, ctx->se18.blob, nw - o < src_n ? nw - o : src_n, wt + o));
    if (getenv("REID_DEBUG_ZERO")) {
        HIP_TRY(hipMemsetAsync(x, 0, nin * 2, ctx->stream));
        HIP_TRY(hipMemsetAsync(wt, 0, nw * 2, ctx->stream));
// ... 475 lines not shown
    }
    if (dx) REID_TRY(dbg_download(ctx, out, dx, nx));
    if (dh) REID_TRY(dbg_download(ctx, (_Float16*)out16, dh, form == 2 || form == 3 ? nx * 2 : nx));
    if (da) {
        REID_TRY(dbg_download(ctx, a_scale, da, nab));
        REID_TRY(dbg_download(ctx, a_shift, dbb, nab));
    }
    HIP_TRY(hipStreamSynchronize(ctx->stream));
    return ctx_fault_status(ctx);
}

extern "C" int reid_debug_se_tail(reid_ctx* ctx, int form, int n, int hw, int c, int mid, int tiles, const float* stats, const float* w1,
                                  const float* w2t, const void* y, const void* shortcut, float* out, uint16_t* out16, float* gate) {
    ARG_CHECK(ctx && form >= 0 && form <= 11 && n >= 1 && hw >= 1 && c >= 4 && mid >= 1 && tiles >= 1 && stats && w1 && w2t && y && shortcut);
    const bool f16 = form >= 10, tail = form >= 1 && form <= 9;
    const bool want_out = !f16 && (!tail || ((form - 1) % 3 != 1)), want_pk = tail && (form - 1) % 3 != 0;
    ARG_CHECK((!want_out || out) && ((!want_pk && !f16) || out16) && ((form != 0 && form != 11) || gate));
    CTX_ENTER(ctx);
    const size_t ny = (size_t)n * hw * c;
    float *dst, *dw1, *dw2, *dy = nullptr, *dsc = nullptr, *dout = nullptr, *dgate = nullptr;
    _Float16 *dy16 = nullptr, *dsc16 = nullptr, *dh = nullptr;
    REID_TRY(dbg_upload(ctx, "dbgt.stats", stats, (size_t)n * tiles * c * 2, &dst));
    REID_TRY(dbg_upload(ctx, "dbgt.w1", w1, (size_t)mid * c, &dw1));
    REID_TRY(dbg_upload(ctx, "dbgt.w2", w2t, (size_t)mid * c, &dw2));
    if (f16) {
        REID_TRY(dbg_upload(ctx, "dbgt.x16", (const _Float16*)y, ny, &dy16));
        REID_TRY(dbg_upload(ctx, "dbgt.sc16", (const _Float16*)shortcut, ny, &dsc16));
        REID_TRY(dbg_output(ctx, "dbgt.pk", ny, &dh));
    } else {
        REID_TRY(dbg_upload(ctx, "dbgt.x", (const float*)y, ny, &dy));
        REID_TRY(dbg_upload(ctx, "dbgt.sc", (const float*)shortcut, ny, &dsc));
        if (want_out) REID_TRY(dbg_output(ctx, "dbgt.out", ny, &dout));
        if (want_pk) REID_TRY(dbg_output(ctx, "dbgt.pk", ny * 2, &dh));
    }
    if (form == 0 || form == 11) REID_TRY(dbg_output(ctx, "dbgt.a", (size_t)n * c, &dgate));
    if (form == 0) {
        REID_TRY(launch_se_finalize(ctx, dst, n, tiles, c, mid, hw, dw1, dw2, dgate));
        REID_TRY(launch_se_combine(ctx, dy, dsc, dgate, n, hw, c, dout));
    } else if (tail) {
        REID_TRY(launch_se_tail_form(ctx, (form - 1) / 3 - 1, dst, n, tiles, c, mid, hw, dw1, dw2, dy, dsc, dout, dh));
    } else if (form == 10) {
        REID_TRY(launch_se_tail_f16(ctx, dst, n, tiles, c, mid, hw, dw1, dw2, dy16, dsc16, dh));
    } else {
        REID_TRY(launch_se_finalize(ctx, dst, n, tiles, c, mid, hw, dw1, dw2, dgate));
        REID_TRY(launch_se_combine_f16(ctx, dy16, dsc16, dgate, n, hw, c, dh));
    }
    if (dout) REID_TRY(dbg_download(ctx, out, dout, ny));
    if (dh) REID_TRY(dbg_download(ctx, (_Float16*)out16, dh, f16 ? ny : ny * 2));
    if (dgate) REID_TRY(dbg_download(ctx, gate, dgate, (size_t)n * c));
    HIP_TRY(hipStreamSynchronize(ctx->stream));
    return ctx_fault_status(ctx);
}

extern "C" int reid_debug_sibling_tail(reid_ctx* ctx, int arch, int n, int h, int w, int c, const float* prm, const float* y,
                                       const float* shortcut, float* out) {
    ARG_CHECK(ctx && (arch == 1 || arch == 2) && n >= 1 && h >= 1 && w >= 1 && c >= 32 && c % 32 == 0 && prm && y && shortcut && out);
    CTX_ENTER(ctx);
    const size_t ny = (size_t)n * h * w * c, cg = (size_t)c / 32;
    float *dp, *dy, *dsc, *dout;
    REID_TRY(dbg_upload(ctx, "dbgt.w1", prm, arch == 1 ? (size_t)300 : cg * cg * 10 + 4 * cg, &dp));
    REID_TRY(dbg_upload(ctx, "dbgt.x", y, ny, &dy));
    REID_TRY(dbg_upload(ctx, "dbgt.sc", shortcut, ny, &dsc));
    REID_TRY(dbg_output(ctx, "dbgt.out", ny, &dout));
    if (arch == 1) REID_TRY(launch_ta_tail(ctx, dy, dsc, n, h, w, c, dp, dout));
    else REID_TRY(launch_ema_tail(ctx, dy, dsc, n, h, w, c, dp, dout));
    REID_TRY(dbg_download(ctx, out, dout, ny));
    HIP_TRY(hipStreamSynchronize(ctx->stream));
    return ctx_fault_status(ctx);
}

extern "C" int reid_debug_gem_neck(reid_ctx* ctx, int f16, int n, int hw, int c, float p, const void* x, const float* scale,
                                   const float* shift, float* gem_out, float* emb) {
    ARG_CHECK(ctx && n >= 1 && hw >= 1 && c >= 64 && x && scale && shift && emb);
    CTX_ENTER(ctx);
    const size_t nx = (size_t)n * hw * c, ne = (size_t)n * c;
    float *dx = nullptr, *dp, *dsc, *dsh, *dg = nullptr, *de;
    _Float16* dh = nullptr;
    REID_TRY(dbg_upload(ctx, "dbgt.p", &p, 1, &dp));
    REID_TRY(dbg_upload(ctx, "dbgt.bns", scale, (size_t)c, &dsc));
    REID_TRY(dbg_upload(ctx, "dbgt.bnh", shift, (size_t)c, &dsh));
    if (gem_out) REID_TRY(dbg_output(ctx, "dbgt.a", ne, &dg));
    REID_TRY(dbg_output(ctx, "dbgt.b", ne, &de));
    if (f16) {
        REID_TRY(dbg_upload(ctx, "dbgt.x16", (const _Float16*)x, nx, &dh));
        REID_TRY(launch_gem_neck_f16(ctx, dh, n, hw, c, dp, dsc, dsh, dg, de));
    } else {
        REID_TRY(dbg_upload(ctx, "dbgt.x", (const float*)x, nx, &dx));
        REID_TRY(launch_gem_neck(ctx, dx, n, hw, c, dp, dsc, dsh, dg, de));
    }
    if (dg) REID_TRY(dbg_download(ctx, gem_out, dg, ne));
    REID_TRY(dbg_download(ctx, emb, de, ne));
    HIP_TRY(hipStreamSynchronize(ctx->stream));
    return ctx_fault_status(ctx);
}

extern "C" int reid_debug_any_norm(reid_ctx* ctx, int n, int hw, int c, int half, const float* x, const float* in_gamma, const float* in_beta,
                                   const float* bn_scale, const float* bn_shift, float* out) {
    ARG_CHECK(ctx && n >= 1 && hw >= 1 && c >= 64 && half >= 32 && half <= c && x && in_gamma && in_beta && out &&
              (bn_scale == nullptr) == (bn_shift == nullptr));
    CTX_ENTER(ctx);
    const size_t nx = (size_t)n * hw * c;
    float *dx, *dg, *db, *dbs = nullptr, *dbh = nullptr;
    REID_TRY(dbg_output(ctx, "dbgt.x", nx + c, &dx));
    HIP_TRY(hipMemcpyAsync(dx, x, nx * 4, hipMemcpyHostToDevice, ctx->stream));
    REID_TRY(dbg_upload(ctx, "dbgt.gamma", in_gamma, (size_t)half, &dg));
    REID_TRY(dbg_upload(ctx, "dbgt.beta", in_beta, (size_t)half, &db));
// ... 963 lines not shown
```

real-time-reid-tracking_amd/csrc/elementwise.hip:

```cpp
#include "reid_internal.h"
#include <math.h>

typedef float f32x4 __attribute__((ext_vector_type(4)));

namespace {

__device__ __forceinline__ float wave_sum(float v) {
#pragma unroll
    for (int o = 32; o > 0; o >>= 1) v += __shfl_xor(v, o);
    return v;
}
__device__ __forceinline__ double wave_sum_d(double v) {
#pragma unroll
    for (int o = 32; o > 0; o >>= 1) v += __shfl_xor(v, o);
    return v;
}

template <int NV, int B>
__device__ __forceinline__ void tile_batch(const float* __restrict__ st, int& t, int c, double (&s)[NV]) {
    float v[B][NV];
#pragma unroll
    for (int u = 0; u < B; ++u)
#pragma unroll
        for (int k = 0; k < NV; ++k) v[u][k] = st[(long long)(t + u) * c * 2 + k];
#pragma unroll
    for (int u = 0; u < B; ++u)
#pragma unroll
        for (int k = 0; k < NV; ++k) s[k] += (double)v[u][k];
    t += B;
}
template <int NV>
__device__ __forceinline__ void tile_sums(const float* __restrict__ st, int tiles, int c, double (&s)[NV]) {
#pragma unroll
    for (int k = 0; k < NV; ++k) s[k] = 0.0;
    int t = 0;
    while (tiles - t >= 16) tile_batch<NV, 16>(st, t, c, s);
    if (tiles - t >= 8) tile_batch<NV, 8>(st, t, c, s);
    if (tiles - t >= 4) tile_batch<NV, 4>(st, t, c, s);
    if (tiles - t >= 2) tile_batch<NV, 2>(st, t, c, s);
    if (tiles - t >= 1) tile_batch<NV, 1>(st, t, c, s);
}

typedef _Float16 h4 __attribute__((ext_vector_type(4)));
__device__ __forceinline__ void store_pair(_Float16* __restrict__ p, int c, const f32x4 v) {
    const h4 hi = {(_Float16)v.x, (_Float16)v.y, (_Float16)v.z, (_Float16)v.w};
    const h4 lo = {(_Float16)((v.x - (float)hi.x) * 2048.0f), (_Float16)((v.y - (float)hi.y) * 2048.0f),
                   (_Float16)((v.z - (float)hi.z) * 2048.0f), (_Float16)((v.w - (float)hi.w) * 2048.0f)};
    *(h4*)p = hi;
    *(h4*)(p + c) = lo;
}

__global__ void nchw_to_nhwc3_kernel(const float* __restrict__ x, long long npix, int hw, float* __restrict__ out) {
    for (long long i = blockIdx.x * (long long)blockDim.x + threadIdx.x; i < npix; i += (long long)gridDim.x * blockDim.x) {
        const long long img = i / hw;
        const int p = (int)(i - img * hw);
        const float* src = x + img * 3 * hw + p;
        float* dst = out + i * 3;
        dst[0] = src[0];
        dst[1] = src[hw];
        dst[2] = src[2 * hw];
    }
}

__device__ __forceinline__ void lin_tap(int d, int dst, int src, int& s, float& f) {
#pragma clang fp contract(off)
    const double scale = (double)src / (double)dst;
    float fx = (float)(((double)d + 0.5) * scale - 0.5);
    int sx = (int)floorf(fx);
    fx = fx - (float)sx;
    if (sx < 0) { sx = 0; fx = 0.f; }
    if (sx >= src - 1) { sx = src - 1; fx = 0.f; }
    s = sx;
    f = fx;
}
__global__ void resize_norm_kernel(const uint8_t* __restrict__ packed, const long long* __restrict__ offsets,
                                   const int* __restrict__ hw, int n, int H, int W, int pitch, float* __restrict__ out) {
#pragma clang fp contract(off)
    const long long total = (long long)n * H * W;
    for (long long i = blockIdx.x * (long long)blockDim.x + threadIdx.x; i < total; i += (long long)gridDim.x * blockDim.x) {
        const int img = (int)(i / (H * W));
        const int rem = (int)(i - (long long)img * H * W);
        const int dy = rem / W, dx = rem - dy * W;
        const int h = hw[2 * img], w = hw[2 * img + 1];
        const uint8_t* src = packed + offsets[img];
        const long long ps = pitch ? pitch : w;
        int sx, sy;
        float fx, fy;
        lin_tap(dx, W, w, sx, fx);
        lin_tap(dy, H, h, sy, fy);
        const int sx1 = min(sx + 1, w - 1), sy1 = min(sy + 1, h - 1);
        const float gx = 1.0f - fx, gy = 1.0f - fy;
#pragma unroll
        for (int c = 0; c < 3; ++c) {
// ... 154 lines not shown
            xp += xs;
            pp += ps;
        }
    } else {
        for (int i = tid; i < total; i += 256) {
            const int row = i / q, cc = i - row * q;
            const f32x4 v = *(const f32x4*)(x + (pix0 + row) * c + cc * 4);
            finish(v, cc * 4 < half, *(const f32x4*)&sa[cc * 4], *(const f32x4*)&sb[cc * 4], packed + (pix0 + row) * 2 * c + cc * 4);
        }
    }
    range_raise(fault, vm);
}

__global__ __launch_bounds__(256) void se_finalize_kernel(const float* __restrict__ stats, int tiles, int c, int mid,
                                                          int hw, const float* __restrict__ w1,
                                                          const float* __restrict__ w2, float* __restrict__ s) {
    __shared__ float pooled[512];
    __shared__ float hid[64];
    const int img = blockIdx.x, tid = threadIdx.x, lane = tid & 63, wave = tid >> 6;
    for (int ch = tid; ch < c; ch += 256) {
        double acc = 0.0;
        for (int t = 0; t < tiles; ++t) acc += (double)stats[(((long long)img * tiles + t) * c + ch) * 2];
        pooled[ch] = (float)(acc / hw);
    }
    __syncthreads();
    for (int m = wave; m < mid; m += 4) {
        float acc = 0.f;
        for (int ch = lane; ch < c; ch += 64) acc += w1[m * c + ch] * pooled[ch];
        acc = wave_sum(acc);
        if (lane == 0) hid[m] = fmaxf(acc, 0.f);
    }
    __syncthreads();
    for (int ch = tid; ch < c; ch += 256) {
        float acc = 0.f;
        for (int m = 0; m < mid; ++m) acc += w2[m * c + ch] * hid[m];
        s[(long long)img * c + ch] = 1.0f / (1.0f + expf(-acc));
    }
}

__global__ void se_combine_kernel(const float* __restrict__ y, const float* __restrict__ sc, const float* __restrict__ s,
                                  long long total4, int hw, int c, float* __restrict__ out) {
    const int c4n = c >> 2;
    for (long long i = blockIdx.x * (long long)blockDim.x + threadIdx.x; i < total4; i += (long long)gridDim.x * blockDim.x) {
        const int cc = (int)(i % c4n);
        const long long pix = i / c4n;
        const long long img = pix / hw;
        const f32x4 yy = *(const f32x4*)(y + i * 4);
        const f32x4 rr = *(const f32x4*)(sc + i * 4);
        const f32x4 ss = *(const f32x4*)(s + img * c + cc * 4);
        f32x4 o = ss * yy + rr;
        o.x = fmaxf(o.x, 0.f); o.y = fmaxf(o.y, 0.f); o.z = fmaxf(o.z, 0.f); o.w = fmaxf(o.w, 0.f);
        *(f32x4*)(out + i * 4) = o;
    }
}

template <bool SMALL>
__device__ __forceinline__ void se_gate(const float* __restrict__ stats, int tiles, int c, int mid, int hw, const float* __restrict__ w1,
                                        const float* __restrict__ w2, int img, float* pooled, float* hid, float* gate) {
    const int tid = threadIdx.x, lane = tid & 63, wave = __builtin_amdgcn_readfirstlane(tid >> 6);
    constexpr int MJ = SMALL ? 8 : 16, MW2 = 32;
    constexpr int W1PRE = SMALL ? 8 : 4;
    const int c4v = c >> 2;
    f32x4 w1v[W1PRE][2];
    float w2v[SMALL ? 2 : 1][SMALL ? MW2 : 1];
#pragma unroll
    for (int j = 0; j < W1PRE; ++j)
#pragma unroll
        for (int k = 0; k < 2; ++k)
            w1v[j][k] = *(const f32x4*)(w1 + (long long)min(wave + 4 * j, mid - 1) * c + min(lane + 64 * k, c4v - 1) * 4);
    if constexpr (SMALL) {
#pragma unroll
        for (int q = 0; q < 2; ++q)
#pragma unroll
            for (int m = 0; m < MW2; ++m) {
                const int ch = tid + 256 * q;
                if (ch < c && m < mid) w2v[q][m] = w2[m * c + ch];
            }
    }
    for (int ch = tid; ch < c; ch += 256) {
        double acc[1];
        tile_sums<1>(stats + ((long long)img * tiles * c + ch) * 2, tiles, c, acc);
        pooled[ch] = (float)(acc[0] / hw);
    }
    __syncthreads();
    {
        float acc[16];
#pragma unroll
        for (int j = 0; j < 16; ++j) acc[j] = 0.f;
#pragma unroll
        for (int g = 0; g < MJ / 4; ++g) {
            if (wave + 16 * g >= mid) break;
            f32x4 wg[4][2];
#pragma unroll
            for (int jj = 0; jj < 4; ++jj)
#pragma unroll
                for (int k = 0; k < 2; ++k) {
                    const int j = 4 * g + jj, m = wave + 4 * j, c4 = lane + 64 * k;
                    if (j < W1PRE) wg[jj][k] = w1v[j < W1PRE ? j : 0][k];
                    else wg[jj][k] = *(const f32x4*)(w1 + (long long)min(m, mid - 1) * c + min(c4, c4v - 1) * 4);
                }
#pragma unroll
            for (int jj = 0; jj < 4; ++jj)
#pragma unroll
                for (int k = 0; k < 2; ++k) {
                    const int j = 4 * g + jj, m = wave + 4 * j, c4 = lane + 64 * k;
                    if (m < mid && c4 < c4v) {
                        const f32x4 wv = wg[jj][k];
                        const f32x4 pv = *(const f32x4*)(pooled + c4 * 4);
                        acc[j] += wv.x * pv.x + wv.y * pv.y + wv.z * pv.z + wv.w * pv.w;
                    }
                }
        }
#pragma unroll
        for (int j = 0; j < 16; ++j) {
            if (wave + 4 * j < mid) {
                const float v = wave_sum(acc[j]);
                if (lane == 0) hid[wave + 4 * j] = fmaxf(v, 0.f);
            }
        }
    }
    __syncthreads();
    if constexpr (SMALL) {
#pragma unroll
        for (int q = 0; q < 2; ++q) {
            const int ch = tid + 256 * q;
            if (ch < c) {
                float acc = 0.f;
#pragma unroll
                for (int m = 0; m < MW2; ++m)
                    if (m < mid) acc += w2v[q][m] * hid[m];
                gate[ch] = 1.0f / (1.0f + expf(-acc));
            }
        }
    } else {
        for (int ch = tid; ch < c; ch += 256) {
            float acc = 0.f;
            for (int m0 = 0; m0 < mid; m0 += 8) {
                float wv[8];
#pragma unroll
                for (int u = 0; u < 8; ++u)
                    if (m0 + u < mid) wv[u] = w2[(m0 + u) * c + ch];
#pragma unroll
                for (int u = 0; u < 8; ++u)
                    if (m0 + u < mid) acc += wv[u] * hid[m0 + u];
            }
            gate[ch] = 1.0f / (1.0f + expf(-acc));
        }
    }
    __syncthreads();
}

template <bool SMALL>
__global__ __launch_bounds__(256) void se_tail_kernel(const float* __restrict__ stats, int tiles, int c, int mid, int hw,
                                                      const float* __restrict__ w1, const float* __restrict__ w2,
                                                      const float* __restrict__ y, const float* __restrict__ sc, int rows,
                                                      float* __restrict__ out, _Float16* __restrict__ packed, int* __restrict__ fault) {
    __shared__ __attribute__((aligned(16))) float pooled[512];
    __shared__ float hid[64];
    __shared__ __attribute__((aligned(16))) float gate[512];
    const int img = blockIdx.y, tid = threadIdx.x;
    se_gate<SMALL>(stats, tiles, c, mid, hw, w1, w2, img, pooled, hid, gate);
    const int c4n = c >> 2;
    const long long pix0 = (long long)img * hw + (long long)blockIdx.x * rows;
    const long long base = pix0 * c;
    const int total4 = rows * c4n;
    unsigned vm = 0u;
    auto finish = [&](const f32x4 ss, const f32x4 yy, const f32x4 rr, long long off, long long pk) {
        f32x4 o = ss * yy + rr;
        if (packed) vm = range_acc(range_acc(range_acc(range_acc(vm, o.x), o.y), o.z), o.w);
        o.x = fmaxf(o.x, 0.f); o.y = fmaxf(o.y, 0.f); o.z = fmaxf(o.z, 0.f); o.w = fmaxf(o.w, 0.f);
        if (out) *(f32x4*)(out + off) = o;
        if (packed) store_pair(packed + pk, c, o);
    };
    if (256 % c4n == 0) {
        const int cc = tid % c4n;
        const f32x4 ss = *(const f32x4*)&gate[cc * 4];
        long long off = base + (long long)tid * 4;
        long long pk = (pix0 + tid / c4n) * 2 * c + cc * 4;
        const long long ps = (long long)(256 / c4n) * 2 * c;
        int i = tid;
        for (; i + 3 * 256 < total4; i += 4 * 256) {
            f32x4 yy[4], rr[4];
#pragma unroll
            for (int u = 0; u < 4; ++u) {
                yy[u] = *(const f32x4*)(y + off + u * 1024);
                rr[u] = *(const f32x4*)(sc + off + u * 1024);
            }
#pragma unroll
            for (int u = 0; u < 4; ++u) finish(ss, yy[u], rr[u], off + u * 1024, pk + u * ps);
            off += 4096;
            pk += 4 * ps;
        }
        for (; i < total4; i += 256) {
            finish(ss, *(const f32x4*)(y + off), *(const f32x4*)(sc + off), off, pk);
            off += 1024;
            pk += ps;
        }
    } else {
        for (int i = tid; i < total4; i += 256) {
            const int cc = i % c4n;
            const long long off = base + (long long)i * 4;
            finish(*(const f32x4*)&gate[cc * 4], *(const f32x4*)(y + off), *(const f32x4*)(sc + off), off,
// ... 169 lines not shown
                       in_gamma, in_beta, packed, in_half_only ? 1 : 0, ctx->fault);
    prof_end(ctx);
    LAUNCH_CHECK();
    return REID_OK;
}

int launch_se_finalize(reid_ctx* ctx, const float* stats, int n_img, int tiles, int c, int mid, int hw, const float* w1,
                       const float* w2, float* s) {
    ARG_CHECK(c <= 512 && mid <= 64);
    prof_begin(ctx, REID_K_ELEMENTWISE, 0, (double)n_img * c * (tiles * 8.0 + 4.0));
    hipLaunchKernelGGL(se_finalize_kernel, dim3(n_img), dim3(256), 0, ctx->stream, stats, tiles, c, mid, hw, w1, w2, s);
    prof_end(ctx);
    LAUNCH_CHECK();
    return REID_OK;
}

int launch_se_combine(reid_ctx* ctx, const float* y, const float* sc, const float* s, int n_img, int hw, int c, float* out) {
    ARG_CHECK(c % 4 == 0);
    const long long total4 = (long long)n_img * hw * (c / 4);
    prof_begin(ctx, REID_K_ELEMENTWISE, 0, total4 * 48.0);
    hipLaunchKernelGGL(se_combine_kernel, dim3(grid_for(total4, 256)), dim3(256), 0, ctx->stream, y, sc, s, total4, hw, c, out);
    prof_end(ctx);
    LAUNCH_CHECK();
    return REID_OK;
}

int tail_slices(int n_img, int hw) {
    int s = 1;
    while ((long long)n_img * s < 1024 && hw / (s * 2) >= 16 && hw % (s * 2) == 0) s *= 2;
    return s;
}

int launch_se_tail(reid_ctx* ctx, const float* stats, int n_img, int tiles, int c, int mid, int hw, const float* w1, const float* w2,
                   const float* y, const float* sc, float* out, _Float16* packed) {
    return launch_se_tail_form(ctx, -1, stats, n_img, tiles, c, mid, hw, w1, w2, y, sc, out, packed);
}

int launch_se_tail_form(reid_ctx* ctx, int form, const float* stats, int n_img, int tiles, int c, int mid, int hw, const float* w1,
                        const float* w2, const float* y, const float* sc, float* out, _Float16* packed) {
    ARG_CHECK(c % 4 == 0 && c <= 512 && mid <= 64 && (out || packed) && form >= -1 && form <= 1 && (form != 1 || mid <= 32));
    const int slices = tail_slices(n_img, hw);
    prof_begin(ctx, REID_K_ELEMENTWISE, 0, (double)n_img * hw * c * 12.0);
    if (form < 0 ? (long long)slices * n_img <= 512 && c >= 512 && mid <= 32 : form == 1)
        hipLaunchKernelGGL(se_tail_kernel<true>, dim3(slices, n_img), dim3(256), 0, ctx->stream, stats, tiles, c, mid, hw, w1, w2, y, sc,
                           hw / slices, out, packed, ctx->fault);
    else
        hipLaunchKernelGGL(se_tail_kernel<false>, dim3(slices, n_img), dim3(256), 0, ctx->stream, stats, tiles, c, mid, hw, w1, w2, y, sc,
                           hw / slices, out, packed, ctx->fault);
    prof_end(ctx);
    LAUNCH_CHECK();
    return REID_OK;
}

int launch_gem_neck(reid_ctx* ctx, const float* x, int n_img, int hw, int c, const float* p, const float* scale,
                    const float* shift, float* gem_out, float* emb) {
    ARG_CHECK(c % 64 == 0);
    prof_begin(ctx, REID_K_ELEMENTWISE, 0, (double)n_img * hw * c * 4.0);
    hipLaunchKernelGGL(gem_neck_kernel, dim3(c / 64, n_img), dim3(256), 0, ctx->stream, x, hw, c, p, scale, shift, gem_out, emb,
                       ctx->fault, nullptr, nullptr, nullptr, 0, 0, nullptr, nullptr);
    prof_end(ctx);
    LAUNCH_CHECK();
    return REID_OK;
}

int launch_gem_neck_tail(reid_ctx* ctx, const float* stats, int n_img, int tiles, int c, int mid, int hw, const float* w1, const float* w2,
                         const float* y, const float* sc, const float* p, const float* scale, const float* shift, float* gem_out,
                         float* emb) {
    ARG_CHECK(c % 64 == 0 && c <= 512 && mid <= 64 && y && sc && stats && w1 && w2);
    int gx = 1;
    while (gx < c / 64 && (long long)n_img * gx < 1024 && (c / 64) % (gx * 2) == 0) gx *= 2;
    prof_begin(ctx, REID_K_ELEMENTWISE, 0, (double)n_img * hw * c * 8.0);
    hipLaunchKernelGGL(gem_neck_kernel, dim3(gx, n_img), dim3(256), 0, ctx->stream, nullptr, hw, c, p, scale, shift, gem_out, emb,
                       ctx->fault, y, sc, stats, tiles, mid, w1, w2);
    prof_end(ctx);
    LAUNCH_CHECK();
    return REID_OK;
}

int launch_row_sqnorm(reid_ctx* ctx, const float* x, int m, int d, long long ld, float* out) {
    prof_begin(ctx, REID_K_ELEMENTWISE, 0, (double)m * d * 4.0);
    hipLaunchKernelGGL(row_sqnorm_kernel, dim3((m + 3) / 4), dim3(256), 0, ctx->stream, x, m, d, ld, out);
    prof_end(ctx);
    LAUNCH_CHECK();
    return REID_OK;
}

namespace {
__global__ void add_indexed_rows_kernel(float* __restrict__ x, long long per_img, int C, const float* __restrict__ table,
                                        const int32_t* __restrict__ idx, float coeff) {
    const int img = blockIdx.y;
    const float* row = table + (long long)idx[img] * C;
    float* xi = x + (long long)img * per_img;
    for (long long i = (long long)blockIdx.x * blockDim.x + threadIdx.x; i < per_img; i += (long long)gridDim.x * blockDim.x)
        xi[i] += coeff * row[i % C];
}
}

int launch_add_indexed_rows(reid_ctx* ctx, float* x, int n, long long hw, int C, const float* table, const int32_t* d_idx, float coeff) {
    ARG_CHECK(x && table && d_idx && n >= 1 && hw >= 1 && C >= 1);
    const long long per_img = hw * C;
    const int gx = (int)((per_img + 256 * 8 - 1) / (256 * 8));
    prof_begin(ctx, REID_K_ELEMENTWISE, (double)n * per_img * 2.0, (double)n * per_img * 8.0);
    hipLaunchKernelGGL(add_indexed_rows_kernel, dim3(gx < 1 ? 1 : gx, n), dim3(256), 0, ctx->stream, x, per_img, C, table, d_idx, coeff);
    prof_end(ctx);
    LAUNCH_CHECK();
    return REID_OK;
// ... 2 lines not shown
```

real-time-reid-tracking_amd/csrc/reid_internal.h:

```cpp
#pragma once
#include <hip/hip_runtime.h>
#include <stdint.h>
#include <stddef.h>
#include <stdio.h>
#include <initializer_list>
#include <string>
#include <map>
#include <tuple>
#include <vector>
#include "../../include/reid_hip.h"
struct reid_ctx;

void reid_set_error(const char* fmt, ...);

#define HIP_TRY(expr)                                                                         \
    do {                                                                                      \
        hipError_t _e = (expr);                                                               \
        if (_e != hipSuccess) {                                                               \
            reid_set_error("%s:%d %s -> %s", __FILE__, __LINE__, #expr, hipGetErrorString(_e)); \
            return REID_ERR_HIP;                                                              \
        }                                                                                     \
    } while (0)

#define REID_TRY(expr)            \
// ... 68 lines not shown
    int* counts;
    unsigned long long* final_keys;
};
int select_segments(int m, int n);
bool dist_select_supported(const SelectParams& p);
int launch_dist_bound(reid_ctx* ctx, const SelectParams& p);
int launch_dist_select(reid_ctx* ctx, const SelectParams& p, float* d_D, int32_t* d_I);

enum A16Mode {
    A16_DENSE = 0,
    A16_IM2COL = 1,
    A16_STEM = 2
};
struct Gemm16Params {
    const _Float16* A;
    long long lda;
    int H, W, Cin, Ho, Wo, R, S, stride, pad, Hp, Wp;
    const _Float16* B;
    long long ldb;
    int M, N, K;
    _Float16* C;
    long long ldc;
    const float* col_scale;
    const float* col_shift;
    const _Float16* residual;
    int relu;
    float* stats;
    const _Float16* zero_page;
    unsigned long long* diag;
    int lin, act, n_real;
    int asym, pad_y, pad_x;
    int scat_h, scat_w, scat_py, scat_px;
    float* C32;
    const float* res32;
    unsigned scat_mhw, scat_mw;
    int par4;
    long long par_stride;
    int split_k;
    float* splitk_ws;
    int* splitk_cnt;
    _Float16* pack16;
    int pack_from;
    int loader_prio;
    int frag_ahead;
    float acc_scale;
    int relu_from;
    int split_terms;
    int pack_out;
    int a_k;
    int pair_early;
    int general_epi;
    int ablate;
    int* fault;
};

__device__ __forceinline__ float l2sqr_of(float dot, float rs, float cq) { return fmaf(-2.0f, dot, rs + cq); }
__device__ __forceinline__ float l2_of_sqr(float v) { return sqrtf(__builtin_elementwise_maximum(v, 1e-12f)); }

__device__ __forceinline__ unsigned range_acc(unsigned m, float v) {
    const unsigned b = __float_as_uint(v) & 0x7fffffffu;
    return b > m ? b : m;
}
__device__ __forceinline__ void range_raise(int* fault, unsigned m) {
    if (fault && m >= 0x477fe000u) fault[0] = 1;
}

template <class P>
inline void set_scatter(P& p, int scat_h, int scat_w, int py, int px) {
    p.scat_h = scat_h; p.scat_w = scat_w; p.scat_py = py; p.scat_px = px;
    p.scat_mhw = p.scat_mw = 0;
    if (scat_h > 0) {
        p.scat_mhw = (unsigned)(((1ull << 32) + (unsigned long long)(scat_h * scat_w) - 1) / (unsigned long long)(scat_h * scat_w));
        p.scat_mw = (unsigned)(((1ull << 32) + (unsigned long long)scat_w - 1) / (unsigned long long)scat_w);
    }
}

struct reid_ctx;
int launch_gemm_f16(reid_ctx* ctx, int amode, const Gemm16Params& p, int kind, double flops, double bytes);
bool conv3x3_f16_supported(const Gemm16Params& p);
int launch_conv3x3_f16(reid_ctx* ctx, const Gemm16Params& p, int kind, double flops, double bytes);
int launch_conv3x3_split(reid_ctx* ctx, const Gemm16Params& p, int kind, double flops, double bytes);
bool conv3x3_x3_supported(const reid_ctx* ctx, const Gemm16Params& p);
int launch_conv3x3_x3(reid_ctx* ctx, const Gemm16Params& p);
bool lin_x3_supported(const reid_ctx* ctx, const Gemm16Params& p);
int launch_lin_x3(reid_ctx* ctx, const Gemm16Params& p, int kind, double flops, double bytes);
bool conv_x3s_supported(const reid_ctx* ctx, const Gemm16Params& p);
int launch_conv_x3s(reid_ctx* ctx, const Gemm16Params& p, int kind, double flops, double bytes);
int launch_gemm_f16_split(reid_ctx* ctx, const Gemm16Params& p, int kind, double flops, double bytes);
bool two_linear_supported(const reid_ctx*, long long T, int C, int hid);
int launch_two_linear(reid_ctx*, const _Float16* a16, long long T, int C, int hid, const float* w1, const float* b1, const float* w2,
                      const float* b2, int act, const float* res, float* out, const float* x32 = nullptr, const float* ln_g = nullptr,
                      const float* ln_b = nullptr);
bool ln_linear_supported(const reid_ctx*, long long T, int C, int n);
int launch_ln_linear(reid_ctx*, const float* x32, const float* ln_g, const float* ln_b, long long T, int C, int n, const float* w, const float* bias,
                     float* out, int ldc);
int launch_window_attn_cos(reid_ctx* ctx, int mode, const void* qkv, int ldq, int n_img, int H, int W, int heads, int shifted,
                           const float* bias_t, const float* scale, void* out);
int launch_post_norm(reid_ctx* ctx, int side_mode, const float* x, const float* y, long long T, int C, const float* g, const float* b,
                     float* out, _Float16* side);
void swin_bias_table(const float* pos169, float* tab4096);
int swin_attn_ldq(const reid_ctx* ctx, int C);
int launch_window_attn(reid_ctx* ctx, const void* qkv, int n, int Hs, int Ws, int heads, int shifted, const float* pos, const float* bias_tab,
                       void* out);
int launch_swin_layernorm(reid_ctx* ctx, int form, const float* x, long long T, int C, const float* g, const float* b, void* out);
int launch_sfe_norm_fc(reid_ctx* ctx, const float* c1, int n, int h1, int w1, const float* in_g, const float* in_b, const float* bn_s,
                       const float* bn_t, const float* c2_w, const float* c2_b, const float* fc_w, const float* fc_b, float* ab, float* tok);
int launch_swin_tail(reid_ctx* ctx, const float* x, int n, int ntok, const float* g, const float* b, const float* p, const float* bn_s,
                     const float* bn_t, float* gem, float* emb);
int swin_loaded_merge(reid_ctx* ctx, int stage, const float* x, int n, int h, int w, float* scratch, float* out);
int swin_loaded_fuse(reid_ctx* ctx, const float* sfe, float* const* xs, int n, int h1, int w1, float* scratch16, float* a0, float* f3, float* f2,
                     float* f1);
int swin_linear_for_test(reid_ctx* ctx, int f16_storage, const float* x32, const _Float16* x16, long long m, int k, const void* w,
                         const float* bias, int n, int act, const float* res, float* out32, _Float16* out16, int ldc);
int launch_sfe_conv1(reid_ctx* ctx, const float* x, int n, int h, int w, const float* c1_w, const float* c1_b, float* c1);
int swin_crops_check(int out_h, int out_w, const float* mean_std6);
int launch_swin_crop_front(reid_ctx* ctx, const uint8_t* d_src, const long long* d_off, const int* d_hw, int n, int h, int w, int pitch,
                           const float* mean_std6, const float* c1_w, const float* c1_b, float* c1);
int launch_sfe_conv1_mirror(reid_ctx* ctx, const float* x, int n, int h, int w, const float* c1_w, const float* c1_b, float* c1);
int launch_swin_crop_front_mirror(reid_ctx* ctx, const uint8_t* d_src, const long long* d_off, const int* d_hw, int n, int h, int w, int pitch,
                                  const float* mean_std6, const float* c1_w, const float* c1_b, float* c1);
int launch_swin_descriptor(reid_ctx* ctx, const float* e1, const float* e2, const float* cls_w, int n, int num_class, long long ld, float* out);
int launch_split_pack(reid_ctx* ctx, const float* x, long long rows, int C, _Float16* out, const float* d_scale = nullptr);
int launch_split_weights(reid_ctx* ctx, const float* w, int cout, int taps, int cin, int terms, _Float16* out, const float* d_scale = nullptr);
int launch_prep_u8_pad_f16(reid_ctx*, const uint8_t* crops, int n, int h, int w, int hp, int wp, _Float16* out);
int launch_prep_f32_pad_f16(reid_ctx*, const float* nhwc3, int n, int h, int w, int hp, int wp, _Float16* out);
int launch_maxpool3s2_f16(reid_ctx*, const _Float16* x, int n, int h, int w, int c, _Float16* out);
int launch_affine_relu_f16(reid_ctx*, _Float16* x, const float* a_scale, const float* a_shift, int n_img, int hw, int c);
int launch_norm_apply_f16(reid_ctx*, _Float16* x, const float* stats, int n_img, int tiles, int c, int half, int hw,
                          const float* in_gamma, const float* in_beta, const float* bn_scale, const float* bn_shift);
int launch_se_tail_f16(reid_ctx*, const float* stats, int n_img, int tiles, int c, int mid, int hw, const float* w1, const float* w2t,
                       const _Float16* y, const _Float16* sc, _Float16* out);
int launch_se_combine_f16(reid_ctx*, const _Float16* y, const _Float16* sc, const float* s, int n_img, int hw, int c,
                          _Float16* out);
int launch_gem_neck_f16(reid_ctx*, const _Float16* x, int n_img, int hw, int c, const float* p, const float* scale,
                        const float* shift, float* gem_out, float* emb);
int launch_f32_to_f16(reid_ctx*, const float* x, size_t n, _Float16* out);
int launch_stem_w16(reid_ctx*, const float* stem_w_f32, _Float16* out);
bool conv3x3_c64_f16_supported(int H, int W, int Cin, int Cout, int R, int S, int stride, int pad);
int launch_scale_rows_f16(reid_ctx*, const float* w, const float* scale, int rows, int k, _Float16* out);
int launch_conv3x3_c64_f16(reid_ctx*, const _Float16* in, int n, const _Float16* w_scaled, const float* shift,
                           const _Float16* residual, int relu, float* stats, _Float16* out, const _Float16* zero_page,
                           const float* se_w1 = nullptr, const float* se_w2t = nullptr);
int launch_stem_w16_scaled(reid_ctx*, const float* stem_w_f32, const float* scale, _Float16* out);
int launch_stem_pool_f16(reid_ctx*, const _Float16* pad_in, const uint8_t* crops_u8, int n, const _Float16* w16s, const float* shift,
                         _Float16* pooled);
int launch_conv_w16_chunked(reid_ctx*, const float* w_f32, int cout, int rs, int cin, _Float16* out);
int launch_gemm_f32(reid_ctx* ctx, int amode, int epi, const GemmParams& p, int kind, double flops, double bytes);
int launch_ta_tail(reid_ctx* ctx, const float* y, const float* sc, int n_img, int H, int W, int C, const float* wts, float* out);
int launch_ema_tail(reid_ctx* ctx, const float* y, const float* sc, int n_img, int H, int W, int C, const float* prm, float* out);
int launch_stem_split(reid_ctx* ctx, const void* x, bool is_u8, int n, const float* wgt, const float* scale, const float* shift, float* out,
                      _Float16* packed);
int launch_stem_f32(reid_ctx* ctx, const void* x, bool is_u8, int n, const float* wgt, const float* scale, const float* shift,
                    float* out, bool pooled);
bool gemm_f32_dma_supported(int amode, int epi, const GemmParams& p);
int launch_gemm_f32_dma(reid_ctx* ctx, int epi, const GemmParams& p, int kind, double flops, double bytes);
bool conv_f32_supported(const GemmParams& p);
int launch_conv_f32(reid_ctx* ctx, const GemmParams& p, int kind, double flops, double bytes);
bool conv_f32_general_supported(const GemmParams& p);
int launch_conv_f32_general(reid_ctx* ctx, const GemmParams& p, int kind, double flops, double bytes);

int launch_nchw_to_nhwc3(reid_ctx*, const float* x_nchw, int n, int h, int w, float* out_nhwc);
int launch_resize_norm(reid_ctx*, const uint8_t* packed, const long long* offsets, const int* hw, int n, int H, int W,
                       int pitch, float* out_nhwc);
int launch_maxpool3s2(reid_ctx*, const float* x, int n, int h, int w, int c, float* out);
int launch_norm_finalize(reid_ctx*, const float* stats, int n_img, int tiles, int c, int half, int hw,
                         const float* in_gamma, const float* in_beta, const float* bn_scale, const float* bn_shift,
                         float* a_scale, float* a_shift);
int launch_in_apply(reid_ctx*, float* x, const float* stats, int n_img, int tiles, int c, int half, int hw, const float* in_gamma,
                    const float* in_beta);
int launch_se_finalize(reid_ctx*, const float* stats, int n_img, int tiles, int c, int mid, int hw, const float* w1,
                       const float* w2, float* s);
int tail_slices(int n_img, int hw);
int launch_se_tail(reid_ctx*, const float* stats, int n_img, int tiles, int c, int mid, int hw, const float* w1, const float* w2,
                   const float* y, const float* sc, float* out, _Float16* packed = nullptr);
int launch_se_tail_form(reid_ctx*, int form, const float* stats, int n_img, int tiles, int c, int mid, int hw, const float* w1,
                        const float* w2, const float* y, const float* sc, float* out, _Float16* packed);
int launch_se_combine(reid_ctx*, const float* y, const float* sc, const float* s, int n_img, int hw, int c, float* out);
int launch_in_apply_pack(reid_ctx*, const float* x, const float* stats, int n_img, int tiles, int c, int half, int hw,
                         const float* in_gamma, const float* in_beta, _Float16* packed,
                         bool in_half_only = false);
int launch_gem_neck(reid_ctx*, const float* x, int n_img, int hw, int c, const float* p, const float* scale,
                    const float* shift, float* gem_out, float* emb);
int launch_gem_neck_tail(reid_ctx*, const float* stats, int n_img, int tiles, int c, int mid, int hw, const float* w1, const float* w2,
                         const float* y, const float* sc, const float* p, const float* scale, const float* shift, float* gem_out,
                         float* emb);
int launch_row_sqnorm(reid_ctx*, const float* x, int m, int d, long long ld, float* out);
int launch_argmin_rows(reid_ctx*, const float* dist, int m, int n, long long ld, int32_t* idx, float* val);
int launch_topk_rows(reid_ctx*, const float* dist, int m, int n, long long ld, int k, float* D, int32_t* I);
int launch_rank_eval(reid_ctx*, const float* score, int nq, int ng, long long ld, const long long* ql,
                     const long long* qc, const long long* gl, const long long* gc, int32_t* cmc_sum, double* ap,
                     int32_t* valid);
int launch_diou_cost(reid_ctx*, const double* tracks, int t, const double* dets, int m, double* out, int as_cost);

struct ProfSlot {
    double ms = 0, flops = 0, bytes = 0;
    long long launches = 0;
};

struct Se18Block {
    int c, cin, stride, ibn, ds, mid;
    const float *conv1_w, *in_gamma, *in_beta, *bn1_scale, *bn1_shift, *conv2_w, *bn2_scale, *bn2_shift;
    const float *ds_w, *ds_scale, *ds_shift, *se_w1, *se_w2;
    const float *ta, *ema;
};

struct Se18Weights {
    bool loaded = false;
    float* blob = nullptr;
    size_t n_floats = 0;
    int num_class = 0;
    int arch = 0;
    const float *stem_w, *stem_scale, *stem_shift;
    Se18Block blk[8];
    const float *gem_p, *neck_scale, *neck_shift, *cls_w;
    const float* cam_bias = nullptr;
    int num_cams = 0;
    float cam_factor = -1.0f;
    _Float16* blob16 = nullptr;
    _Float16* stem_w16 = nullptr;
    _Float16* l1_conv2_w16s[2] = {nullptr, nullptr};
    _Float16* stem_w16s = nullptr;
    _Float16* zero_page = nullptr;
    float* ep = nullptr;
    const _Float16* h(const float* p) const { return blob16 + (p - blob); }
};

struct reid_comm_loop {
    virtual int allgather(int rank, const void* d_send, void* d_recv, size_t bytes, hipStream_t st) = 0;
    virtual int allreduce(int rank, double* inout, int count, int op) = 0;
// ... 2 lines not shown
};
struct reid_comm {
    void* comm = nullptr;
    int rank = 0, world = 1;
    reid_comm_loop* loop = nullptr;
};
void comm_release(reid_ctx* ctx);
int launch_knn_merge(reid_ctx* ctx, const float* Dall, const int32_t* Iall, int world, int nq, int kk, int k, float* D, int32_t* I);

struct reid_ctx {
    int device = 0;
    reid_comm* comm = nullptr;
    hipStream_t stream = nullptr;
    hipStream_t own_stream = nullptr;
    int chunk = 1024;
    int precision = 0;
    bool profile = false;
    ProfSlot prof[REID_K_COUNT];
    std::vector<std::pair<hipEvent_t, hipEvent_t>> ev_pool;
    struct Pending { int kind; hipEvent_t a, b; double flops, bytes; };
    std::vector<Pending> pending;
    hipEvent_t t0 = nullptr, t1 = nullptr;
    std::map<std::string, std::pair<void*, size_t>> ws;
    std::map<std::string, std::pair<void*, size_t>> pinned;
    std::map<const void*, void*> split_w;
    int bank_fast = 1;
    Se18Weights se18;
    int last_n = 0;
    int swin_last_n = 0, swin_last_tok = 0;
    int debug_keep = 0;
    bool last_f16 = false;
    int f16_wide_splitk = 1;
    int f16_frag_ahead = 1;
    int f16_loader_prio = 1;
    int f16_loader_waves = 1;
    int f16_halo = 1;
    int gem_tail_min = 120;
    int f16_se_tail = 1;
    int f16_c64 = 2;
    int f16_stem_fused = 2;
    int f32_conv = 1;
    int f32_split_k = 1;
    int lin_x3 = 1;
    int f32_dist_bk16 = 1;
    int pack_epilogue = 1;
    int split_lean_epi = 1;
    int split_x3 = 3;
    int split_gemm_min_tiles = 128;
    int chain = 0;
    int x3_sk_cap = 0;
    int split_x3_small = 2;
    int x3s_sk_cap = 8;
    int conv_x3s = 1;
    int x3_l4_narrow_nmt = 31;
    int x3_narrow = 1;
    int x3_unroll = 3;
    int x3_ablate = 0;
    int split_x3_min_blocks = 512;
    int split_pair = 0;
    int stem_split = 1;
    int f32_stem_pool = 1;
    int split_terms = 3;
    int knn_wide = 1;
    long long knn_wide_min = 1ll << 25;
    int knn_wide_force = 0;
    int select_exp = 0;
    int select_two_pass = 0;
    int rerank_hbm_acc = 0;
    int swin_stop = -1;
    int swin_fold = 1;
    int swin_two_linear = 1;
    int swin_attn_split = 0;
    int two_linear_ablate = 0;
    int swin_attn_mfma = 1;
    int f16_split_k = 1;
    int swin_chunk_cap = 1024;
    int f16_lin_256 = 1;
    int f16_cfg = 0;
    int frame_m[2] = {0, 0};
    float* frame_emb[2] = {nullptr, nullptr};
    int frame_d[2] = {512, 512};
    int frame_pending[2] = {0, 0}, frame_has[2] = {0, 0};
    size_t frame_tm[2] = {0, 0};
    hipEvent_t frame_ev[2] = {nullptr, nullptr};
    hipStream_t match_stream = nullptr;
    int match_async = 0;
    hipEvent_t join_ev = nullptr;
    hipEvent_t fwd_ev[2] = {nullptr, nullptr}, match_ev[2] = {nullptr, nullptr};
    hipStream_t copy_stream = nullptr;
    hipEvent_t copy_ev = nullptr;
    std::vector<hipEvent_t> pipe_ev;
    int host_pipeline = 1;
    int side_copy = 1;
    std::vector<int32_t> side_idx;
    size_t side_cursor = 0;
    const char* frame_out[2] = {nullptr, nullptr};
    float* stage_ptr[11] = {nullptr};
    size_t stage_elems[11] = {0};
    int anysize_force = 0;
    int any_front = 2;
    int hw_precision = -1;
    int any_conv_form = 0;
    unsigned long long* conv_diag = nullptr;
    int conv_form = 0;
    std::string split_bad_se18, split_bad_swin;
    int* fault = nullptr;
// ... 230 lines not shown
```

real-time-reid-tracking_amd/engine.py:

```python
import ctypes as C

import numpy as np

from . import _ffi
from ._ffi import check

_ENGINES = {}

IMG_H, IMG_W = 256, 128
SIZE_MIN, SIZE_MAX = 32, 512
HW_PRECISION_NAMES = {"f32": 0, "fp32": 0, "exact": 0, "f16x3": 2, "fp32-class": 2}
DISTMAT_PRECISION_NAMES = {"f32": 0, "f16x3": 2}
SELECT_X3_KMAX = 24


def check_hw(size):
    try:
        h, w = size
        if int(h) != h or int(w) != w:
            raise TypeError
        h, w = int(h), int(w)
    except (TypeError, ValueError):
        raise ValueError("size must be (H, W) integers, got %r" % (size,))
    if not (SIZE_MIN <= h <= SIZE_MAX and SIZE_MIN <= w <= SIZE_MAX):
# ... 649 lines not shown
        return out.view(np.float16), st, form.value

    def debug_conv_c64_se(self, x, w_folded, shift=None, residual=None, relu=False, se_w1=None, se_w2t=None, stats=False):
        bits = lambda a: None if a is None else np.ascontiguousarray(a).view(np.uint16)
        xb, wb, rb = bits(x), bits(w_folded), bits(residual)
        n = xb.shape[0]
        if xb.shape[1:] != (64, 32, 64) or wb.size != 64 * 576 or (rb is not None and rb.shape != xb.shape):
            raise ValueError("debug_conv_c64_se expects x / residual [n, 64, 32, 64] and w_folded [64, 576]")
        out = np.empty(xb.shape, np.uint16)
        st = np.empty((n, 64, 2), np.float32) if stats else None
        sh, w1, w2 = (None if a is None else _f32(a) for a in (shift, se_w1, se_w2t))
        if (sh is not None and sh.size != 64) or any(a is not None and a.size != 512 for a in (w1, w2)):
            raise ValueError("debug_conv_c64_se expects shift [64] and se_w1 / se_w2t [8, 64]")
        form = C.c_int(0)
        check(_ffi.debug_lib().reid_debug_conv_c64_se(
            self.h, C.c_int(n), _ptr(xb), _ptr(wb), _ptr(sh), _ptr(rb), C.c_int(int(bool(relu))), _ptr(w1), _ptr(w2), _ptr(out), _ptr(st),
            C.byref(form)))
        return out.view(np.float16), st, form.value

    def debug_norm_finish(self, form, x, stats, in_gamma, in_beta, bn_scale=None, bn_shift=None, hw=None):
        stats = _f32(stats)
        n, tiles, c, _ = stats.shape
        half = int(np.asarray(in_gamma).size)
        hw = int(hw) if x is None else x.shape[1]
        xa = None if form == 0 else (np.ascontiguousarray(x, np.uint16) if form >= 4 else _f32(x))
        out = np.empty((n, hw, c), np.float32) if 1 <= form <= 3 else None
        o16 = np.empty((n * hw, 2 * c), np.uint16) if form in (2, 3) else (np.empty((n, hw, c), np.uint16) if form >= 4 else None)
        ab = [np.empty((n, c), np.float32) for _ in range(2)] if form in (0, 5) else [None, None]
        opt = [_f32(a) if a is not None else None for a in (in_gamma, in_beta, bn_scale, bn_shift)]
        check(_ffi.debug_lib().reid_debug_norm_finish(
            self.h, C.c_int(form), C.c_int(n), C.c_int(hw), C.c_int(c), C.c_int(half), C.c_int(tiles), _ptr(xa), _ptr(stats),
            _ptr(opt[0]), _ptr(opt[1]), _ptr(opt[2]), _ptr(opt[3]), _ptr(out), _ptr(o16), _ptr(ab[0]), _ptr(ab[1])))
        return out, o16, ab[0], ab[1]

    def debug_se_tail(self, form, stats, w1, w2t, y, shortcut):
        stats = _f32(stats)
        n, tiles, c, _ = stats.shape
        mid = w1.shape[0]
        hw = y.shape[1]
        f16 = form >= 10
        cv = (lambda a: np.ascontiguousarray(a, np.uint16)) if f16 else _f32
        ya, sa = cv(y), cv(shortcut)
        tail = 1 <= form <= 9
        want_out = not f16 and (not tail or (form - 1) % 3 != 1)
        want_pk = tail and (form - 1) % 3 != 0
        out = np.empty((n, hw, c), np.float32) if want_out else None
        o16 = np.empty((n, hw, c), np.uint16) if f16 else (np.empty((n * hw, 2 * c), np.uint16) if want_pk else None)
        gate = np.empty((n, c), np.float32) if form in (0, 11) else None
        check(_ffi.debug_lib().reid_debug_se_tail(
            self.h, C.c_int(form), C.c_int(n), C.c_int(hw), C.c_int(c), C.c_int(mid), C.c_int(tiles), _ptr(stats), _ptr(_f32(w1)),
            _ptr(_f32(w2t)), _ptr(ya), _ptr(sa), _ptr(out), _ptr(o16), _ptr(gate)))
        return out, o16, gate

    def debug_sibling_tail(self, arch, prm, y, shortcut):
        y, shortcut = _f32(y), _f32(shortcut)
        n, h, w, c = y.shape
        out = np.empty((n, h, w, c), np.float32)
        check(_ffi.debug_lib().reid_debug_sibling_tail(self.h, C.c_int(arch), C.c_int(n), C.c_int(h), C.c_int(w), C.c_int(c), _ptr(_f32(prm)),
                                                       _ptr(y), _ptr(shortcut), _ptr(out)))
        return out

    def debug_gem_neck(self, x, p, scale, shift, f16=False):
        x = np.ascontiguousarray(x, np.uint16) if f16 else _f32(x)
        n, hw, c = x.shape
        g, e = np.empty((n, c), np.float32), np.empty((n, c), np.float32)
        check(_ffi.debug_lib().reid_debug_gem_neck(
            self.h, C.c_int(int(bool(f16))), C.c_int(n), C.c_int(hw), C.c_int(c), C.c_float(p), _ptr(x), _ptr(_f32(scale)),
            _ptr(_f32(shift)), _ptr(g), _ptr(e)))
        return g, e

    def debug_gem_neck_fused(self, stats, w1, w2t, y, shortcut, p, scale, shift):
        stats = _f32(stats)
        n, tiles, c, _ = stats.shape
        y, shortcut = _f32(y), _f32(shortcut)
        g, e = np.empty((n, c), np.float32), np.empty((n, c), np.float32)
        check(_ffi.debug_lib().reid_debug_gem_neck_fused(
            self.h, C.c_int(n), C.c_int(y.shape[1]), C.c_int(c), C.c_int(w1.shape[0]), C.c_int(tiles), C.c_float(p), _ptr(stats),
            _ptr(_f32(w1)), _ptr(_f32(w2t)), _ptr(y), _ptr(shortcut), _ptr(_f32(scale)), _ptr(_f32(shift)), _ptr(g), _ptr(e)))
        return g, e

    def debug_stem(self, form, x, w, scale, shift):
        is_u8 = np.asarray(x).dtype == np.uint8
        x = np.ascontiguousarray(x, np.uint8) if is_u8 else _f32(x)
        n = x.shape[0]
        if x.shape[1:] != (IMG_H, IMG_W, 3) or np.shape(w) != (64, 7, 7, 3):
            raise ValueError("debug_stem expects x[n, 256, 128, 3] and w[64, 7, 7, 3]")
        out = np.empty((n, 128, 64, 64) if form == 0 else (n, 64, 32, 64), np.float32) if form in (0, 1, 2, 6) else None
        o16 = np.empty((n * 2048, 128), np.uint16) if form == 2 else (np.empty((n, 64, 32, 64), np.uint16) if form in (3, 4, 5) else None)
        check(_ffi.debug_lib().reid_debug_stem(self.h, C.c_int(form), C.c_int(int(is_u8)), _ptr(x), C.c_int(n), _ptr(_f32(w)),
                                               _ptr(_f32(scale)), _ptr(_f32(shift)), _ptr(out), _ptr(o16)))
        return out, o16

    def debug_resize_norm(self, packed, offsets, hw, pitch=0):
        packed = np.ascontiguousarray(packed, np.uint8).reshape(-1)
        offsets = np.ascontiguousarray(offsets, np.int64)
        hw = np.ascontiguousarray(hw, np.int32).reshape(-1, 2)
        n = len(offsets)
        end = max(int(o) + ((int(h) - 1) * (pitch or int(w)) + int(w)) * 3 for o, (h, w) in zip(offsets, hw))
        if len(hw) != n or end > packed.size:
            raise ValueError("debug_resize_norm: a window leaves the buffer")
        out = np.empty((n, IMG_H, IMG_W, 3), np.float32)
        check(_ffi.debug_lib().reid_debug_resize_norm(self.h, _ptr(packed), _ptr(offsets), _ptr(hw), C.c_int(n), C.c_int(int(pitch)), _ptr(out)))
        return out

    def debug_pil_resize(self, images, size, mean_std=None, want_u8=True, packed=None, offsets=None, hw=None):
        try:
# ... 504 lines not shown
```

Baseline: 84470 crops/s.

## Fuse downsample 1x1 conv with SE gate, residual and pack in ds blocks

In the fp32-class split mode, the downsample blocks no longer run a separate 1x1 shortcut conv followed by an SE-tail kernel. The SE gate is computed first, then one x3s GEMM kernel with a new SE epilogue applies the BN scale/shift and adds gate*y. The same epilogue does ReLU and writes the fp32 output plus the packed f16 hi/lo representation for the next layer. This removes the shortcut tensor round trip through memory and one or more launches. In exchange it adds a separately loaded shared library, an extra workspace buffer, and restrictions: no split-K, and Ho*Wo must be a multiple of 128.

Result: no change. 85010 crops/s (median of 6 runs) (+0.6%).

```diff
diff --git a/include/reid_hip_debug.h b/include/reid_hip_debug.h
--- a/include/reid_hip_debug.h
+++ b/include/reid_hip_debug.h
@@ -33,6 +33,9 @@
                            uint16_t* out16, float* a_scale, float* a_shift);
 int reid_debug_se_tail(reid_ctx* ctx, int form, int n, int hw, int c, int mid, int tiles, const float* stats, const float* w1,
                        const float* w2t, const void* y, const void* shortcut, float* out, uint16_t* out16, float* gate);
+int reid_debug_ds_tail(reid_ctx* ctx, int form, int n, int h, int w, int cin, int cout, int stride, int mid, int tiles,
+                       const uint16_t* x16, const float* wgt, const float* scale, const float* shift, const float* y, const float* stats,
+                       const float* w1, const float* w2t, float* out, uint16_t* out16);
 int reid_debug_sibling_tail(reid_ctx* ctx, int arch, int n, int h, int w, int c, const float* prm, const float* y, const float* shortcut,
                             float* out);
 int reid_debug_gem_neck(reid_ctx* ctx, int f16, int n, int hw, int c, float p, const void* x, const float* scale, const float* shift,
diff --git a/real-time-reid-tracking_amd/_ffi.py b/real-time-reid-tracking_amd/_ffi.py
--- a/real-time-reid-tracking_amd/_ffi.py
+++ b/real-time-reid-tracking_amd/_ffi.py
@@ -122,7 +122,7 @@
 EXPORTS = tuple(sorted(_SIGS))
 
 DEBUG_LIB_PATH = os.path.join(_HERE, "libreid_hip_debug.so")
-DEBUG_EXPORTS = ("reid_debug_any_conv", "reid_debug_any_front", "reid_debug_any_gem", "reid_debug_any_norm", "reid_debug_any_se_tail", "reid_debug_bank_cost96", "reid_debug_coissue", "reid_debug_comm_loopback", "reid_debug_conv_c64", "reid_debug_conv_c64_se", "reid_debug_conv_layer", "reid_debug_conv_layer_f16", "reid_debug_conv_split", "reid_debug_conv_diag", "reid_debug_conv_f16", "reid_debug_conv_f32",
+DEBUG_EXPORTS = ("reid_debug_any_conv", "reid_debug_any_front", "reid_debug_any_gem", "reid_debug_any_norm", "reid_debug_any_se_tail", "reid_debug_bank_cost96", "reid_debug_coissue", "reid_debug_comm_loopback", "reid_debug_conv_c64", "reid_debug_conv_c64_se", "reid_debug_conv_layer", "reid_debug_conv_layer_f16", "reid_debug_conv_split", "reid_debug_conv_diag", "reid_debug_conv_f16", "reid_debug_conv_f32", "reid_debug_ds_tail",
                  "reid_debug_feed", "reid_debug_gem_neck", "reid_debug_gem_neck_fused", "reid_debug_gemm_f16", "reid_debug_knn_merge", "reid_debug_knn_wide", "reid_debug_layernorm", "reid_debug_linear", "reid_debug_linear_rows", "reid_debug_ln_linear", "reid_debug_maxpool", "reid_debug_mfma_bare", "reid_debug_mfma_shape", "reid_debug_norm_finish", "reid_debug_pil_resize", "reid_debug_post_norm", "reid_debug_resize_norm", "reid_debug_se_tail", "reid_debug_stem", "reid_debug_sibling_tail", "reid_debug_swin_conv1", "reid_debug_swin_conv1_mirror", "reid_debug_swin_crop_front", "reid_debug_swin_crop_front_mirror", "reid_debug_swin_descriptor", "reid_debug_swin_fuse", "reid_debug_swin_linear", "reid_debug_swin_merge", "reid_debug_swin_sfe", "reid_debug_swin_tail", "reid_debug_select_exp", "reid_debug_select_x3", "reid_debug_set_switch", "reid_debug_get_switch", "reid_debug_two_linear", "reid_debug_two_linear_ablate", "reid_debug_two_linear_form", "reid_debug_window_attn", "reid_debug_window_attn_cos")
 
 _lib = None
diff --git a/real-time-reid-tracking_amd/csrc/api.hip b/real-time-reid-tracking_amd/csrc/api.hip
--- a/real-time-reid-tracking_amd/csrc/api.hip
+++ b/real-time-reid-tracking_amd/csrc/api.hip
@@ -7,6 +7,7 @@
 #include "anysize_front.h"
 #include <cmath>
 #include <dlfcn.h>
+#include "ds_tail.h"
 #include <mutex>
 #include <stdarg.h>
 #include <stdio.h>
@@ -605,7 +606,7 @@
 
 static const int IMG_H = 256, IMG_W = 128;
 
-static bool conv_split_path(reid_ctx* ctx, int n, int H, int W, int Cin, int Cout, int R, int S, int stride, int pad) {
+bool conv_split_path(reid_ctx* ctx, int n, int H, int W, int Cin, int Cout, int R, int S, int stride, int pad) {
     if (ctx->precision != 2 || Cin % 64 != 0 || Cout % 64 != 0 || !ctx->se18.zero_page) return false;
     Gemm16Params q;
     memset(&q, 0, sizeof(q));
@@ -723,6 +724,51 @@
     return REID_OK;
 }
 
+int ds_tail_api(const DsTailApi** out) {
+    static std::mutex m;
+    static DsTailApi api;
+    std::lock_guard<std::mutex> lk(m);
+    if (!api.conv) {
+        void* f[2];
+        REID_TRY(open_beside_self("libreid_hip_ds_tail.so", "the fused end of the down-sampling blocks in the fp32-class mode needs",
+                                  {"dstail_gate", "dstail_conv"}, f));
+        api.gate = (decltype(&dstail_gate))f[0];
+        api.conv = (decltype(&dstail_conv))f[1];
+    }
+    *out = &api;
+    return REID_OK;
+}
+
+bool ds_tail_geometry(const reid_ctx* ctx, int n, int H, int W, int Cin, int Cout, int stride, Gemm16Params& q) {
+    memset(&q, 0, sizeof(q));
+    if (ctx->split_terms != 3 || stride < 1) return false;
+    q.split_terms = 3;
+    q.H = H; q.W = W; q.Cin = 3 * Cin; q.R = 1; q.S = 1; q.stride = stride; q.pad = 0;
+    q.Ho = (H - 1) / stride + 1; q.Wo = (W - 1) / stride + 1;
+    q.M = n * q.Ho * q.Wo; q.N = Cout; q.K = 3 * Cin; q.ldb = q.K; q.ldc = Cout;
+    return true;
+}
+
+int ds_tail_conv(reid_ctx* ctx, const Gemm16Params& geom, const _Float16* in16, const float* wgt, const float* scale, const float* shift,
+                 const float* y, const float* stats, int tiles, int mid, const float* se_w1, const float* se_w2, float* gate, float* out,
+                 _Float16* out16) {
+    Gemm16Params q = geom;
+    const int n = q.M / (q.Ho * q.Wo), cin = q.Cin / 3;
+    ARG_CHECK(in16 && out16 && in16 != out16 && y && gate);
+    REID_TRY(launch_se_gate(ctx, stats, n, tiles, q.N, mid, q.Ho * q.Wo, se_w1, se_w2, gate));
+    REID_TRY(split_weights_of(ctx, wgt, q.N, 1, cin, &q.B));
+    q.A = in16;
+    q.C32 = out;
+    q.col_scale = scale; q.col_shift = shift;
+    q.res32 = y; q.se_gate = gate;
+    q.pack16 = out16; q.pack_from = 0;
+    q.acc_scale = 1.0f / 2048.0f;
+    q.zero_page = ctx->se18.zero_page;
+    const double mn = (double)q.M * q.N;
+    const double bytes = (double)q.M * cin * 4.0 + mn * (out ? 12.0 : 8.0) + (double)q.N * 3.0 * cin * 2.0;
+    return launch_conv_x3s_se(ctx, q, REID_K_CONV_GEMM, 2.0 * mn * cin, bytes);
+}
+
 #ifdef REID_EXPERIMENTS
 static int seres18_chain_layer4(reid_ctx* ctx, int n, const Se18Block& ka, const Se18Block& kb, const _Float16* in16, const float* sc,
                                 float* y, float* out_a, float* out, float* stats) {
@@ -820,7 +866,7 @@
     (void)nt;
 
     const bool pool_fused = ctx->f32_conv == 1 && ctx->f32_stem_pool && ctx->debug_keep != 1;
-    _Float16* cur16 = nullptr;
+    _Float16 *cur16 = nullptr, *alt16 = nullptr;
     const bool split_mode = ctx->precision == 2 && w.arch == 0 && ctx->f32_conv == 1;
     if (split_mode) REID_TRY(ctx_ws(ctx, "split.cur", (size_t)n * per * 2 * 2, (void**)&cur16));
     const bool stem_split = split_mode && pool_fused && ctx->stem_split;
@@ -902,7 +948,11 @@
                            k.bn2_scale, k.bn2_shift, k.ds ? nullptr : cur, k.ds ? 0 : 1, b.stats, y));
         }
         const float* shortcut = cur;
-        if (k.ds) {
+        Gemm16Params dsq;
+        const bool ds_fused = k.ds && w.arch == 0 && ctx->f32_conv == 1 && ctx->ds_tail_fused == 1 && cur16 && !keep && ctx->pack_epilogue &&
+                              conv_split_path(ctx, n, H, W, k.cin, k.c, 1, 1, k.stride, 0) &&
+                              ds_tail_geometry(ctx, n, H, W, k.cin, k.c, k.stride, dsq) && conv_x3s_se_supported(ctx, dsq);
+        if (k.ds && !ds_fused) {
             REID_TRY(conv_gemm(ctx, A_IM2COL, cur, n, H, W, k.cin, k.ds_w, k.c, 1, 1, k.stride, 0, k.cin, nullptr, nullptr, 0,
                                k.ds_scale, k.ds_shift, nullptr, 0, nullptr, sc, 0, cur16));
             shortcut = sc;
@@ -919,7 +969,13 @@
                 fp32_read = !(conv_split_path(ctx, n, Ho, Wo, nx.cin, nx.c, 3, 3, nx.stride, 1) &&
                               conv_split_path(ctx, n, Ho, Wo, nx.cin, nx.c, 1, 1, nx.stride, 0));
             }
-            if (i == 7 && !keep && n >= ctx->gem_tail_min) {
+            if (ds_fused) {
+                ARG_CHECK((size_t)hw * k.c <= 65536);
+                if (!alt16) REID_TRY(ctx_ws(ctx, "split.cur2", (size_t)n * 65536 * 2 * 2, (void**)&alt16));
+                REID_TRY(ds_tail_conv(ctx, dsq, cur16, k.ds_w, k.ds_scale, k.ds_shift, y, b.stats, tiles, k.mid, k.se_w1, k.se_w2, b.se,
+                                      fp32_read ? out : nullptr, alt16));
+                std::swap(cur16, alt16);
+            } else if (i == 7 && !keep && n >= ctx->gem_tail_min) {
                 REID_TRY(launch_gem_neck_tail(ctx, b.stats, n, tiles, k.c, k.mid, hw, k.se_w1, k.se_w2, y, shortcut, w.gem_p, w.neck_scale,
                                               w.neck_shift, b.gem, d_emb));
                 gem_done = true;
diff --git a/real-time-reid-tracking_amd/csrc/conv3x3_x3.hip b/real-time-reid-tracking_amd/csrc/conv3x3_x3.hip
--- a/real-time-reid-tracking_amd/csrc/conv3x3_x3.hip
+++ b/real-time-reid-tracking_amd/csrc/conv3x3_x3.hip
@@ -339,7 +339,7 @@
 template <int N>
 __device__ __forceinline__ void lgkm_wait0() { asm volatile("s_waitcnt lgkmcnt(%0)" ::"n"(N) : "memory"); }
 
-template <int TW, int IMGS, int BN, bool LIN = false, int COH = 0>
+template <int TW, int IMGS, int BN, bool LIN = false, int COH = 0, bool SE = false>
 __device__ __forceinline__ void x3m16_tail(const Gemm16Params& p, f32x4 (&acc)[4][BN / 16], char* lds, int tid, int wm, int mtile, int n_blk,
                                            int tile_id, int ksplit, int SK) {
     constexpr int TM = 4, TN = BN / 16;
@@ -357,7 +357,7 @@
     __syncthreads();
 
     bool sk_path = false;
-    if (SK > 1) {
+    if (!SE && SK > 1) {
         sk_path = true;
         constexpr int PART_B = 256 * BN * 4;
         char* part = (char*)(p.splitk_ws + (long long)tile_id * SK * (256 * BN));
@@ -409,10 +409,60 @@
         voff_a[a] = row_ok ? (lrow * ldc + col0) * 4 : 0x7fffff00;
         koff_a[a] = row_ok ? (lrow * 2 * p.N + col0) * 2 : 0x7fffff00;
     }
-    const bool has_stats = p.stats != nullptr;
+    const bool has_stats = !SE && p.stats != nullptr;
     float vmax = 0.f;
-    auto run = [&](auto res_c, auto st_c) {
-        constexpr bool RES = decltype(res_c)::value, ST = decltype(st_c)::value;
+    unsigned vm_se = 0u;
+    __amdgpu_buffer_rsrc_t g_rs = c_rs;
+    if constexpr (SE) {
+        const int img = (m_blk + (wm >> 1) * 128) / (p.Ho * p.Wo);
+        g_rs = __builtin_amdgcn_make_buffer_rsrc((void*)(p.se_gate + (long long)img * p.N), 0, p.N * 4, 0x00020000);
+    }
+    auto run = [&](auto res_c, auto st_c, auto se_c) {
+        constexpr bool RES = decltype(res_c)::value, ST = decltype(st_c)::value, SEC = decltype(se_c)::value;
+        if constexpr (SEC) {
+            f32x4 yy[2][TM], gg[2], csr[2], shr[2];
+            gg[0] = __builtin_bit_cast(f32x4, __builtin_amdgcn_raw_buffer_load_b128(g_rs, col0 * 4, 0, 0));
+            csr[0] = *(const f32x4*)(p.col_scale + col0);
+            shr[0] = *(const f32x4*)(p.col_shift + col0);
+#pragma unroll
+            for (int a = 0; a < TM; ++a)
+                yy[0][a] = __builtin_bit_cast(f32x4, __builtin_amdgcn_raw_buffer_load_b128(r_rs, voff_a[a], (wm * 64 + a * 16) * ldc * 4, COH));
+#pragma unroll
+            for (int b = 0; b < TN; ++b) {
+                if (b + 1 < TN) {
+                    gg[(b + 1) & 1] = __builtin_bit_cast(f32x4, __builtin_amdgcn_raw_buffer_load_b128(g_rs, col0 * 4 + (b + 1) * 64, 0, 0));
+                    csr[(b + 1) & 1] = *(const f32x4*)(p.col_scale + col0 + (b + 1) * 16);
+                    shr[(b + 1) & 1] = *(const f32x4*)(p.col_shift + col0 + (b + 1) * 16);
+#pragma unroll
+                    for (int a = 0; a < TM; ++a)
+                        yy[(b + 1) & 1][a] =
+                            __builtin_bit_cast(f32x4, __builtin_amdgcn_raw_buffer_load_b128(r_rs, voff_a[a] + (b + 1) * 64, (wm * 64 + a * 16) * ldc * 4, COH));
+                }
+                const f32x4 cs = csr[b & 1] * p.acc_scale, sh = shr[b & 1];
+#pragma unroll
+                for (int a = 0; a < TM; ++a) {
+                    const int ubase = wm * 64 + a * 16;
+                    const f32x4 v = acc[a][b] * cs + sh;
+                    f32x4 o = gg[b & 1] * yy[b & 1][a] + v;
+                    vm_se = range_acc(range_acc(range_acc(range_acc(vm_se, o[0]), o[1]), o[2]), o[3]);
+#pragma unroll
+                    for (int e = 0; e < 4; ++e) o[e] = fmaxf(o[e], 0.f);
+                    if (p.C32) __builtin_amdgcn_raw_buffer_store_b128(__builtin_bit_cast(u32x4, o), c_rs, voff_a[a] + b * 64, ubase * ldc * 4, COH);
+                    u32x2 hw, lw;
+#pragma unroll
+                    for (int h = 0; h < 2; ++h) {
+                        const float v0 = o[2 * h], v1 = o[2 * h + 1];
+                        const f16 h0 = cvt_f16_rn(v0), h1 = cvt_f16_rn(v1);
+                        const f16 l0 = cvt_f16_rn((v0 - (float)h0) * 2048.0f), l1 = cvt_f16_rn((v1 - (float)h1) * 2048.0f);
+                        hw[h] = (unsigned)__builtin_bit_cast(unsigned short, h0) | ((unsigned)__builtin_bit_cast(unsigned short, h1) << 16);
+                        lw[h] = (unsigned)__builtin_bit_cast(unsigned short, l0) | ((unsigned)__builtin_bit_cast(unsigned short, l1) << 16);
+                    }
+                    __builtin_amdgcn_raw_buffer_store_b64(hw, k_rs, koff_a[a] + b * 32, ubase * 2 * p.N * 2, COH);
+                    __builtin_amdgcn_raw_buffer_store_b64(lw, k_rs, koff_a[a] + b * 32 + p.N * 2, ubase * 2 * p.N * 2, COH);
+                }
+            }
+            return;
+        }
 #pragma unroll
         for (int b = 0; b < TN; ++b) {
             const int col = col0 + b * 16, tcol = n_blk + b * 16;
@@ -588,7 +638,11 @@
             else run_sk(sk_c, std::false_type{}, std::false_type{});
         }
     };
-    if (sk_path) {
+    if constexpr (SE) {
+        static_assert(!SE || (TW == 16 && !LIN && COH == 0), "the SE form: conv_x3s_se_kernel's epilogue only");
+        if (wave_live) run(std::false_type{}, std::false_type{}, std::true_type{});
+        range_raise(p.fault, vm_se);
+    } else if (sk_path) {
         if constexpr (!LIN) {
             if (wave_live) {
                 if (SK == 2) run_sk_n(std::integral_constant<int, 2>{});
@@ -599,11 +653,11 @@
         }
     } else if (wave_live) {
         if (p.res32) {
-            if (has_stats) run(std::true_type{}, std::true_type{});
-            else run(std::true_type{}, std::false_type{});
+            if (has_stats) run(std::true_type{}, std::true_type{}, std::false_type{});
+            else run(std::true_type{}, std::false_type{}, std::false_type{});
         } else {
-            if (has_stats) run(std::false_type{}, std::true_type{});
-            else run(std::false_type{}, std::false_type{});
+            if (has_stats) run(std::false_type{}, std::true_type{}, std::false_type{});
+            else run(std::false_type{}, std::false_type{}, std::false_type{});
         }
     }
     if (p.fault && !(vmax < 65504.f)) p.fault[0] = 1;
@@ -1501,8 +1555,8 @@
 #endif
 }
 
-template <int BN>
-__global__ __launch_bounds__(256, 2) void conv_x3s_kernel(const Gemm16Params p) {
+template <int BN, bool SE>
+__device__ __forceinline__ void conv_x3s_body(const Gemm16Params& p) {
 #if defined(__HIP_DEVICE_COMPILE__)
     constexpr int TM = 4, TN = BN / 16, BJ = BN / 64;
     constexpr int A_SLOT = 256 * 64, B_SLOT = BN * 64;
@@ -1692,9 +1746,14 @@
         sa_l = sa_h;
         sa_h = nh;
     }
-    x3m16_tail<16, 1, BN, false>(p, acc, lds, tid, wm, mtile, n_blk, tile_id, ksplit, SK);
+    x3m16_tail<16, 1, BN, false, 0, SE>(p, acc, lds, tid, wm, mtile, n_blk, tile_id, ksplit, SK);
 #endif
 }
+template <int BN>
+__global__ __launch_bounds__(256, 2) void conv_x3s_kernel(const Gemm16Params p) { conv_x3s_body<BN, false>(p); }
+#ifdef REID_X3_DEVICE_ONLY
+}
+#else
 
 static int x3_split(const reid_ctx* ctx, int tiles, int ncr, bool wide, int slots = 512) {
     int sk = 1;
@@ -1818,13 +1877,41 @@
     return a_bytes < 0x7f000000ll && 128ll * p.ldb * 2 < 0x7f000000ll && 256ll * p.ldc * 4 < 0x7f000000ll && (long long)p.M * 2 < 0x7f000000ll;
 }
 
+static int x3s_split(const reid_ctx* ctx, const Gemm16Params& p) {
+    const int tiles = ((p.M + 255) / 256) * (p.N / 128), nq = p.R * p.S * (p.Cin / 3 / 32);
+    int sk = 1;
+    while (ctx->f16_split_k && tiles * sk * 2 <= 512 && nq / (sk * 2) >= 2 && sk * 2 <= ctx->x3s_sk_cap) sk *= 2;
+    return sk;
+}
+
+bool conv_x3s_se_supported(const reid_ctx* ctx, const Gemm16Params& p) {
+    return conv_x3s_supported(ctx, p) && p.R == 1 && p.S == 1 && p.Ho * p.Wo > 0 && (p.Ho * p.Wo) % 128 == 0 && x3s_split(ctx, p) == 1;
+}
+
+int launch_conv_x3s_se(reid_ctx* ctx, const Gemm16Params& p0, int kind, double flops, double bytes) {
+    Gemm16Params p = p0;
+    ARG_CHECK(conv_x3s_se_supported(ctx, p) && p.res32 && p.se_gate && p.pack16 && p.pack_from == 0 && !p.stats && p.ldc == p.N &&
+              p.col_scale && p.col_shift);
+    const DsTailApi* api;
+    REID_TRY(ds_tail_api(&api));
+    p.fault = ctx->fault;
+    p.ablate = 0;
+    p.split_k = 1;
+    p.relu = 0;
+    prof_begin(ctx, kind, flops, bytes);
+    const hipError_t e = api->conv(ctx->stream, &p);
+    prof_end(ctx);
+    HIP_TRY(e);
+    ++ctx->ds_tail_launches;
+    return REID_OK;
+}
+
 int launch_conv_x3s(reid_ctx* ctx, const Gemm16Params& p0, int kind, double flops, double bytes) {
     Gemm16Params p = p0;
     p.fault = ctx->fault;
     p.ablate = 0;
-    const int tiles = ((p.M + 255) / 256) * (p.N / 128), nq = p.R * p.S * (p.Cin / 3 / 32);
-    int sk = 1;
-    while (ctx->f16_split_k && tiles * sk * 2 <= 512 && nq / (sk * 2) >= 2 && sk * 2 <= ctx->x3s_sk_cap) sk *= 2;
+    const int tiles = ((p.M + 255) / 256) * (p.N / 128);
+    const int sk = x3s_split(ctx, p);
     if (sk > 1) {
         float* ws;
         int* cnt;
@@ -1870,3 +1957,4 @@
     LAUNCH_CHECK();
     return REID_OK;
 }
+#endif
diff --git a/real-time-reid-tracking_amd/csrc/debug.hip b/real-time-reid-tracking_amd/csrc/debug.hip
--- a/real-time-reid-tracking_amd/csrc/debug.hip
+++ b/real-time-reid-tracking_amd/csrc/debug.hip
@@ -20,7 +20,8 @@
     {"split_x3", &reid_ctx::split_x3}, {"x3_ablate", &reid_ctx::x3_ablate}, {"x3_unroll", &reid_ctx::x3_unroll}, {"x3_narrow", &reid_ctx::x3_narrow}, {"conv_x3s", &reid_ctx::conv_x3s}, {"x3s_sk_cap", &reid_ctx::x3s_sk_cap}, {"x3_l4_narrow_nmt", &reid_ctx::x3_l4_narrow_nmt}, {"split_x3_small", &reid_ctx::split_x3_small}, {"split_x3_min_blocks", &reid_ctx::split_x3_min_blocks}, {"f32_dist_bk16", &reid_ctx::f32_dist_bk16}, {"lin_x3", &reid_ctx::lin_x3},
     {"host_pipeline", &reid_ctx::host_pipeline}, {"x3_sk_cap", &reid_ctx::x3_sk_cap}, {"chain", &reid_ctx::chain}, {"split_gemm_min_tiles", &reid_ctx::split_gemm_min_tiles},
     {"rerank_hbm_acc", &reid_ctx::rerank_hbm_acc}, {"gem_tail_min", &reid_ctx::gem_tail_min}, {"anysize_force", &reid_ctx::anysize_force},
-    {"any_front", &reid_ctx::any_front},
+    {"any_front", &reid_ctx::any_front}, {"ds_tail_fused", &reid_ctx::ds_tail_fused},
+    {"ds_tail_launches", &reid_ctx::ds_tail_launches},
 };
 }
 
@@ -602,6 +603,47 @@
     return ctx_fault_status(ctx);
 }
 
+extern "C" int reid_debug_ds_tail(reid_ctx* ctx, int form, int n, int h, int w, int cin, int cout, int stride, int mid, int tiles,
+                                  const uint16_t* x16, const float* wgt, const float* scale, const float* shift, const float* y,
+                                  const float* stats, const float* w1, const float* w2t, float* out, uint16_t* out16) {
+    ARG_CHECK(ctx && (form == 0 || form == 1) && n >= 1 && h >= 1 && w >= 1 && cin >= 32 && cout >= 128 && cout <= 512 && mid >= 1 && mid <= 64 &&
+              tiles >= 1 && x16 && wgt && scale && shift && y && stats && w1 && w2t && out16);
+    CTX_ENTER(ctx);
+    Gemm16Params q;
+    ARG_CHECK(ctx->precision == 2 && conv_split_path(ctx, n, h, w, cin, cout, 1, 1, stride, 0) &&
+              ds_tail_geometry(ctx, n, h, w, cin, cout, stride, q) && conv_x3s_se_supported(ctx, q));
+    const int hw = q.Ho * q.Wo;
+    ARG_CHECK(tiles == hw / 128);
+    const size_t nin = (size_t)n * h * w * 2 * cin, nw = (size_t)cout * cin, ny = (size_t)n * hw * cout;
+    REID_TRY(conv_weights_splittable(ctx, wgt, nw, "reid_debug_ds_tail"));
+    _Float16 *dx, *dpk;
+    float *dw, *dsc, *dsh, *dy, *dst, *dw1, *dw2, *dout = nullptr, *dshort, *dgate;
+    REID_TRY(dbg_upload(ctx, "dbgd.x16", (const _Float16*)x16, nin, &dx));
+    REID_TRY(dbg_upload(ctx, "dbgd.w", wgt, nw, &dw));
+    REID_TRY(dbg_upload(ctx, "dbgd.scale", scale, (size_t)cout, &dsc));
+    REID_TRY(dbg_upload(ctx, "dbgd.shift", shift, (size_t)cout, &dsh));
+    REID_TRY(dbg_upload(ctx, "dbgt.x", y, ny, &dy));
+    REID_TRY(dbg_upload(ctx, "dbgt.stats", stats, (size_t)n * tiles * cout * 2, &dst));
+    REID_TRY(dbg_upload(ctx, "dbgt.w1", w1, (size_t)mid * cout, &dw1));
+    REID_TRY(dbg_upload(ctx, "dbgt.w2", w2t, (size_t)mid * cout, &dw2));
+    if (out) REID_TRY(dbg_output(ctx, "dbgt.out", ny, &dout));
+    REID_TRY(dbg_output(ctx, "dbgt.pk", ny * 2, &dpk));
+    REID_TRY(dbg_output(ctx, "dbgt.sc", ny, &dshort));
+    REID_TRY(dbg_output(ctx, "dbgt.a", (size_t)n * cout, &dgate));
+    REID_TRY(conv_weights_fresh(ctx, dw));
+    if (form == 0) {
+        REID_TRY(conv_gemm(ctx, A_IM2COL, nullptr, n, h, w, cin, dw, cout, 1, 1, stride, 0, cin, nullptr, nullptr, 0, dsc, dsh, nullptr, 0,
+                           nullptr, dshort, 0, dx));
+        REID_TRY(launch_se_tail(ctx, dst, n, tiles, cout, mid, hw, dw1, dw2, dy, dshort, dout, dpk));
+    } else {
+        REID_TRY(ds_tail_conv(ctx, q, dx, dw, dsc, dsh, dy, dst, tiles, mid, dw1, dw2, dgate, dout, dpk));
+    }
+    REID_TRY(dbg_download(ctx, out, dout, ny));
+    REID_TRY(dbg_download(ctx, (_Float16*)out16, dpk, ny * 2));
+    HIP_TRY(hipStreamSynchronize(ctx->stream));
+    return ctx_fault_status(ctx);
+}
+
 extern "C" int reid_debug_sibling_tail(reid_ctx* ctx, int arch, int n, int h, int w, int c, const float* prm, const float* y,
                                        const float* shortcut, float* out) {
     ARG_CHECK(ctx && (arch == 1 || arch == 2) && n >= 1 && h >= 1 && w >= 1 && c >= 32 && c % 32 == 0 && prm && y && shortcut && out);
diff --git a/real-time-reid-tracking_amd/csrc/ds_tail.h b/real-time-reid-tracking_amd/csrc/ds_tail.h
--- /dev/null
+++ b/real-time-reid-tracking_amd/csrc/ds_tail.h
@@ -0,0 +1,9 @@
+#pragma once
+#include <hip/hip_runtime.h>
+#include "reid_internal.h"
+
+extern "C" {
+hipError_t dstail_gate(hipStream_t stream, int small, const float* stats, int n_img, int tiles, int c, int mid, int hw, const float* w1,
+                        const float* w2, float* gate);
+hipError_t dstail_conv(hipStream_t stream, const Gemm16Params* p);
+}
diff --git a/real-time-reid-tracking_amd/csrc/ds_tail.hip b/real-time-reid-tracking_amd/csrc/ds_tail.hip
--- /dev/null
+++ b/real-time-reid-tracking_amd/csrc/ds_tail.hip
@@ -0,0 +1,34 @@
+#include "ds_tail.h"
+#include "se_gate.h"
+#define REID_X3_DEVICE_ONLY 1
+#include "conv3x3_x3.hip"
+
+namespace {
+
+template <bool SMALL>
+__global__ __launch_bounds__(256) void se_gate_kernel(const float* __restrict__ stats, int tiles, int c, int mid, int hw,
+                                                      const float* __restrict__ w1, const float* __restrict__ w2, float* __restrict__ out) {
+    __shared__ __attribute__((aligned(16))) float pooled[512];
+    __shared__ float hid[64];
+    __shared__ __attribute__((aligned(16))) float gate[512];
+    const int img = blockIdx.x;
+    se_gate<SMALL>(stats, tiles, c, mid, hw, w1, w2, img, pooled, hid, gate);
+    for (int ch = threadIdx.x; ch < c; ch += 256) out[(long long)img * c + ch] = gate[ch];
+}
+
+template <int BN>
+__global__ __launch_bounds__(256, 2) void conv_x3s_se_kernel(const Gemm16Params p) { conv_x3s_body<BN, true>(p); }
+
+}
+
+extern "C" hipError_t dstail_gate(hipStream_t stream, int small, const float* stats, int n_img, int tiles, int c, int mid, int hw,
+                                   const float* w1, const float* w2, float* gate) {
+    if (small) hipLaunchKernelGGL(se_gate_kernel<true>, dim3(n_img), dim3(256), 0, stream, stats, tiles, c, mid, hw, w1, w2, gate);
+    else hipLaunchKernelGGL(se_gate_kernel<false>, dim3(n_img), dim3(256), 0, stream, stats, tiles, c, mid, hw, w1, w2, gate);
+    return hipGetLastError();
+}
+
+extern "C" hipError_t dstail_conv(hipStream_t stream, const Gemm16Params* p) {
+    hipLaunchKernelGGL((conv_x3s_se_kernel<128>), dim3(((p->M + 255) / 256) * (p->N / 128)), dim3(256), 0, stream, *p);
+    return hipGetLastError();
+}
diff --git a/real-time-reid-tracking_amd/csrc/elementwise.hip b/real-time-reid-tracking_amd/csrc/elementwise.hip
--- a/real-time-reid-tracking_amd/csrc/elementwise.hip
+++ b/real-time-reid-tracking_amd/csrc/elementwise.hip
@@ -1,44 +1,15 @@
 #include "reid_internal.h"
+#include "se_gate.h"
 #include <math.h>
 
 typedef float f32x4 __attribute__((ext_vector_type(4)));
 
 namespace {
 
-__device__ __forceinline__ float wave_sum(float v) {
+__device__ __forceinline__ double wave_sum_d(double v) {
 #pragma unroll
     for (int o = 32; o > 0; o >>= 1) v += __shfl_xor(v, o);
     return v;
-}
-__device__ __forceinline__ double wave_sum_d(double v) {
-#pragma unroll
-    for (int o = 32; o > 0; o >>= 1) v += __shfl_xor(v, o);
-    return v;
-}
-
-template <int NV, int B>
-__device__ __forceinline__ void tile_batch(const float* __restrict__ st, int& t, int c, double (&s)[NV]) {
-    float v[B][NV];
-#pragma unroll
-    for (int u = 0; u < B; ++u)
-#pragma unroll
-        for (int k = 0; k < NV; ++k) v[u][k] = st[(long long)(t + u) * c * 2 + k];
-#pragma unroll
-    for (int u = 0; u < B; ++u)
-#pragma unroll
-        for (int k = 0; k < NV; ++k) s[k] += (double)v[u][k];
-    t += B;
-}
-template <int NV>
-__device__ __forceinline__ void tile_sums(const float* __restrict__ st, int tiles, int c, double (&s)[NV]) {
-#pragma unroll
-    for (int k = 0; k < NV; ++k) s[k] = 0.0;
-    int t = 0;
-    while (tiles - t >= 16) tile_batch<NV, 16>(st, t, c, s);
-    if (tiles - t >= 8) tile_batch<NV, 8>(st, t, c, s);
-    if (tiles - t >= 4) tile_batch<NV, 4>(st, t, c, s);
-    if (tiles - t >= 2) tile_batch<NV, 2>(st, t, c, s);
-    if (tiles - t >= 1) tile_batch<NV, 1>(st, t, c, s);
 }
 
 typedef _Float16 h4 __attribute__((ext_vector_type(4)));
@@ -299,102 +270,6 @@
         o.x = fmaxf(o.x, 0.f); o.y = fmaxf(o.y, 0.f); o.z = fmaxf(o.z, 0.f); o.w = fmaxf(o.w, 0.f);
         *(f32x4*)(out + i * 4) = o;
     }
-}
-
-template <bool SMALL>
-__device__ __forceinline__ void se_gate(const float* __restrict__ stats, int tiles, int c, int mid, int hw, const float* __restrict__ w1,
-                                        const float* __restrict__ w2, int img, float* pooled, float* hid, float* gate) {
-    const int tid = threadIdx.x, lane = tid & 63, wave = __builtin_amdgcn_readfirstlane(tid >> 6);
-    constexpr int MJ = SMALL ? 8 : 16, MW2 = 32;
-    constexpr int W1PRE = SMALL ? 8 : 4;
-    const int c4v = c >> 2;
-    f32x4 w1v[W1PRE][2];
-    float w2v[SMALL ? 2 : 1][SMALL ? MW2 : 1];
-#pragma unroll
-    for (int j = 0; j < W1PRE; ++j)
-#pragma unroll
-        for (int k = 0; k < 2; ++k)
-            w1v[j][k] = *(const f32x4*)(w1 + (long long)min(wave + 4 * j, mid - 1) * c + min(lane + 64 * k, c4v - 1) * 4);
-    if constexpr (SMALL) {
-#pragma unroll
-        for (int q = 0; q < 2; ++q)
-#pragma unroll
-            for (int m = 0; m < MW2; ++m) {
-                const int ch = tid + 256 * q;
-                if (ch < c && m < mid) w2v[q][m] = w2[m * c + ch];
-            }
-    }
-    for (int ch = tid; ch < c; ch += 256) {
-        double acc[1];
-        tile_sums<1>(stats + ((long long)img * tiles * c + ch) * 2, tiles, c, acc);
-        pooled[ch] = (float)(acc[0] / hw);
-    }
-    __syncthreads();
-    {
-        float acc[16];
-#pragma unroll
-        for (int j = 0; j < 16; ++j) acc[j] = 0.f;
-#pragma unroll
-        for (int g = 0; g < MJ / 4; ++g) {
-            if (wave + 16 * g >= mid) break;
-            f32x4 wg[4][2];
-#pragma unroll
-            for (int jj = 0; jj < 4; ++jj)
-#pragma unroll
-                for (int k = 0; k < 2; ++k) {
-                    const int j = 4 * g + jj, m = wave + 4 * j, c4 = lane + 64 * k;
-                    if (j < W1PRE) wg[jj][k] = w1v[j < W1PRE ? j : 0][k];
-                    else wg[jj][k] = *(const f32x4*)(w1 + (long long)min(m, mid - 1) * c + min(c4, c4v - 1) * 4);
-                }
-#pragma unroll
-            for (int jj = 0; jj < 4; ++jj)
-#pragma unroll
-                for (int k = 0; k < 2; ++k) {
-                    const int j = 4 * g + jj, m = wave + 4 * j, c4 = lane + 64 * k;
-                    if (m < mid && c4 < c4v) {
-                        const f32x4 wv = wg[jj][k];
-                        const f32x4 pv = *(const f32x4*)(pooled + c4 * 4);
-                        acc[j] += wv.x * pv.x + wv.y * pv.y + wv.z * pv.z + wv.w * pv.w;
-                    }
-                }
-        }
-#pragma unroll
-        for (int j = 0; j < 16; ++j) {
-            if (wave + 4 * j < mid) {
-                const float v = wave_sum(acc[j]);
-                if (lane == 0) hid[wave + 4 * j] = fmaxf(v, 0.f);
-            }
-        }
-    }
-    __syncthreads();
-    if constexpr (SMALL) {
-#pragma unroll
-        for (int q = 0; q < 2; ++q) {
-            const int ch = tid + 256 * q;
-            if (ch < c) {
-                float acc = 0.f;
-#pragma unroll
-                for (int m = 0; m < MW2; ++m)
-                    if (m < mid) acc += w2v[q][m] * hid[m];
-                gate[ch] = 1.0f / (1.0f + expf(-acc));
-            }
-        }
-    } else {
-        for (int ch = tid; ch < c; ch += 256) {
-            float acc = 0.f;
-            for (int m0 = 0; m0 < mid; m0 += 8) {
-                float wv[8];
-#pragma unroll
-                for (int u = 0; u < 8; ++u)
-                    if (m0 + u < mid) wv[u] = w2[(m0 + u) * c + ch];
-#pragma unroll
-                for (int u = 0; u < 8; ++u)
-                    if (m0 + u < mid) acc += wv[u] * hid[m0 + u];
-            }
-            gate[ch] = 1.0f / (1.0f + expf(-acc));
-        }
-    }
-    __syncthreads();
 }
 
 template <bool SMALL>
@@ -670,6 +545,19 @@
     return REID_OK;
 }
 
+int launch_se_gate(reid_ctx* ctx, const float* stats, int n_img, int tiles, int c, int mid, int hw, const float* w1, const float* w2,
+                   float* gate) {
+    ARG_CHECK(c % 4 == 0 && c <= 512 && mid <= 64 && stats && w1 && w2 && gate);
+    const DsTailApi* api;
+    REID_TRY(ds_tail_api(&api));
+    const int slices = tail_slices(n_img, hw);
+    prof_begin(ctx, REID_K_ELEMENTWISE, 0, ((double)n_img * tiles * c * 2.0 + 2.0 * mid * c + (double)n_img * c) * 4.0);
+    const hipError_t e = api->gate(ctx->stream, (long long)slices * n_img <= 512 && c >= 512 && mid <= 32, stats, n_img, tiles, c, mid, hw, w1, w2, gate);
+    prof_end(ctx);
+    HIP_TRY(e);
+    return REID_OK;
+}
+
 int launch_gem_neck(reid_ctx* ctx, const float* x, int n_img, int hw, int c, const float* p, const float* scale,
                     const float* shift, float* gem_out, float* emb) {
     ARG_CHECK(c % 64 == 0);
diff --git a/real-time-reid-tracking_amd/csrc/reid_internal.h b/real-time-reid-tracking_amd/csrc/reid_internal.h
--- a/real-time-reid-tracking_amd/csrc/reid_internal.h
+++ b/real-time-reid-tracking_amd/csrc/reid_internal.h
@@ -144,6 +144,7 @@
     int general_epi;
     int ablate;
     int* fault;
+    const float* se_gate;
 };
 
 __device__ __forceinline__ float l2sqr_of(float dot, float rs, float cq) { return fmaf(-2.0f, dot, rs + cq); }
@@ -178,6 +179,18 @@
 int launch_lin_x3(reid_ctx* ctx, const Gemm16Params& p, int kind, double flops, double bytes);
 bool conv_x3s_supported(const reid_ctx* ctx, const Gemm16Params& p);
 int launch_conv_x3s(reid_ctx* ctx, const Gemm16Params& p, int kind, double flops, double bytes);
+bool conv_x3s_se_supported(const reid_ctx* ctx, const Gemm16Params& p);
+int launch_conv_x3s_se(reid_ctx* ctx, const Gemm16Params& p, int kind, double flops, double bytes);
+struct DsTailApi {
+    hipError_t (*gate)(hipStream_t, int small, const float* stats, int n_img, int tiles, int c, int mid, int hw, const float* w1, const float* w2, float* gate);
+    hipError_t (*conv)(hipStream_t, const Gemm16Params* p);
+};
+int ds_tail_api(const DsTailApi** out);
+bool conv_split_path(reid_ctx* ctx, int n, int H, int W, int Cin, int Cout, int R, int S, int stride, int pad);
+bool ds_tail_geometry(const reid_ctx* ctx, int n, int H, int W, int Cin, int Cout, int stride, Gemm16Params& q);
+int ds_tail_conv(reid_ctx* ctx, const Gemm16Params& geom, const _Float16* in16, const float* wgt, const float* scale, const float* shift,
+                 const float* y, const float* stats, int tiles, int mid, const float* se_w1, const float* se_w2, float* gate, float* out,
+                 _Float16* out16);
 int launch_gemm_f16_split(reid_ctx* ctx, const Gemm16Params& p, int kind, double flops, double bytes);
 bool two_linear_supported(const reid_ctx*, long long T, int C, int hid);
 int launch_two_linear(reid_ctx*, const _Float16* a16, long long T, int C, int hid, const float* w1, const float* b1, const float* w2,
@@ -267,6 +280,8 @@
                    const float* y, const float* sc, float* out, _Float16* packed = nullptr);
 int launch_se_tail_form(reid_ctx*, int form, const float* stats, int n_img, int tiles, int c, int mid, int hw, const float* w1,
                         const float* w2, const float* y, const float* sc, float* out, _Float16* packed);
+int launch_se_gate(reid_ctx*, const float* stats, int n_img, int tiles, int c, int mid, int hw, const float* w1, const float* w2,
+                   float* gate);
 int launch_se_combine(reid_ctx*, const float* y, const float* sc, const float* s, int n_img, int hw, int c, float* out);
 int launch_in_apply_pack(reid_ctx*, const float* x, const float* stats, int n_img, int tiles, int c, int half, int hw,
                          const float* in_gamma, const float* in_beta, _Float16* packed,
@@ -375,6 +390,8 @@
     int split_x3_small = 2;
     int x3s_sk_cap = 8;
     int conv_x3s = 1;
+    int ds_tail_fused = 1;
+    int ds_tail_launches = 0;
     int x3_l4_narrow_nmt = 31;
     int x3_narrow = 1;
     int x3_unroll = 3;
diff --git a/real-time-reid-tracking_amd/csrc/se_gate.h b/real-time-reid-tracking_amd/csrc/se_gate.h
--- /dev/null
+++ b/real-time-reid-tracking_amd/csrc/se_gate.h
@@ -0,0 +1,132 @@
+#pragma once
+#include <hip/hip_runtime.h>
+#include <math.h>
+
+typedef float f32x4 __attribute__((ext_vector_type(4)));
+
+__device__ __forceinline__ float wave_sum(float v) {
+#pragma unroll
+    for (int o = 32; o > 0; o >>= 1) v += __shfl_xor(v, o);
+    return v;
+}
+
+template <int NV, int B>
+__device__ __forceinline__ void tile_batch(const float* __restrict__ st, int& t, int c, double (&s)[NV]) {
+    float v[B][NV];
+#pragma unroll
+    for (int u = 0; u < B; ++u)
+#pragma unroll
+        for (int k = 0; k < NV; ++k) v[u][k] = st[(long long)(t + u) * c * 2 + k];
+#pragma unroll
+    for (int u = 0; u < B; ++u)
+#pragma unroll
+        for (int k = 0; k < NV; ++k) s[k] += (double)v[u][k];
+    t += B;
+}
+template <int NV>
+__device__ __forceinline__ void tile_sums(const float* __restrict__ st, int tiles, int c, double (&s)[NV]) {
+#pragma unroll
+    for (int k = 0; k < NV; ++k) s[k] = 0.0;
+    int t = 0;
+    while (tiles - t >= 16) tile_batch<NV, 16>(st, t, c, s);
+    if (tiles - t >= 8) tile_batch<NV, 8>(st, t, c, s);
+    if (tiles - t >= 4) tile_batch<NV, 4>(st, t, c, s);
+    if (tiles - t >= 2) tile_batch<NV, 2>(st, t, c, s);
+    if (tiles - t >= 1) tile_batch<NV, 1>(st, t, c, s);
+}
+
+template <bool SMALL>
+__device__ __forceinline__ void se_gate(const float* __restrict__ stats, int tiles, int c, int mid, int hw, const float* __restrict__ w1,
+                                        const float* __restrict__ w2, int img, float* pooled, float* hid, float* gate) {
+    const int tid = threadIdx.x, lane = tid & 63, wave = __builtin_amdgcn_readfirstlane(tid >> 6);
+    constexpr int MJ = SMALL ? 8 : 16, MW2 = 32;
+    constexpr int W1PRE = SMALL ? 8 : 4;
+    const int c4v = c >> 2;
+    f32x4 w1v[W1PRE][2];
+    float w2v[SMALL ? 2 : 1][SMALL ? MW2 : 1];
+#pragma unroll
+    for (int j = 0; j < W1PRE; ++j)
+#pragma unroll
+        for (int k = 0; k < 2; ++k)
+            w1v[j][k] = *(const f32x4*)(w1 + (long long)min(wave + 4 * j, mid - 1) * c + min(lane + 64 * k, c4v - 1) * 4);
+    if constexpr (SMALL) {
+#pragma unroll
+        for (int q = 0; q < 2; ++q)
+#pragma unroll
+            for (int m = 0; m < MW2; ++m) {
+                const int ch = tid + 256 * q;
+                if (ch < c && m < mid) w2v[q][m] = w2[m * c + ch];
+            }
+    }
+    for (int ch = tid; ch < c; ch += 256) {
+        double acc[1];
+        tile_sums<1>(stats + ((long long)img * tiles * c + ch) * 2, tiles, c, acc);
+        pooled[ch] = (float)(acc[0] / hw);
+    }
+    __syncthreads();
+    {
+        float acc[16];
+#pragma unroll
+        for (int j = 0; j < 16; ++j) acc[j] = 0.f;
+#pragma unroll
+        for (int g = 0; g < MJ / 4; ++g) {
+            if (wave + 16 * g >= mid) break;
+            f32x4 wg[4][2];
+#pragma unroll
+            for (int jj = 0; jj < 4; ++jj)
+#pragma unroll
+                for (int k = 0; k < 2; ++k) {
+                    const int j = 4 * g + jj, m = wave + 4 * j, c4 = lane + 64 * k;
+                    if (j < W1PRE) wg[jj][k] = w1v[j < W1PRE ? j : 0][k];
+                    else wg[jj][k] = *(const f32x4*)(w1 + (long long)min(m, mid - 1) * c + min(c4, c4v - 1) * 4);
+                }
+#pragma unroll
+            for (int jj = 0; jj < 4; ++jj)
+#pragma unroll
+                for (int k = 0; k < 2; ++k) {
+                    const int j = 4 * g + jj, m = wave + 4 * j, c4 = lane + 64 * k;
+                    if (m < mid && c4 < c4v) {
+                        const f32x4 wv = wg[jj][k];
+                        const f32x4 pv = *(const f32x4*)(pooled + c4 * 4);
+                        acc[j] += wv.x * pv.x + wv.y * pv.y + wv.z * pv.z + wv.w * pv.w;
+                    }
+                }
+        }
+#pragma unroll
+        for (int j = 0; j < 16; ++j) {
+            if (wave + 4 * j < mid) {
+                const float v = wave_sum(acc[j]);
+                if (lane == 0) hid[wave + 4 * j] = fmaxf(v, 0.f);
+            }
+        }
+    }
+    __syncthreads();
+    if constexpr (SMALL) {
+#pragma unroll
+        for (int q = 0; q < 2; ++q) {
+            const int ch = tid + 256 * q;
+            if (ch < c) {
+                float acc = 0.f;
+#pragma unroll
+                for (int m = 0; m < MW2; ++m)
+                    if (m < mid) acc += w2v[q][m] * hid[m];
+                gate[ch] = 1.0f / (1.0f + expf(-acc));
+            }
+        }
+    } else {
+        for (int ch = tid; ch < c; ch += 256) {
+            float acc = 0.f;
+            for (int m0 = 0; m0 < mid; m0 += 8) {
+                float wv[8];
+#pragma unroll
+                for (int u = 0; u < 8; ++u)
+                    if (m0 + u < mid) wv[u] = w2[(m0 + u) * c + ch];
+#pragma unroll
+                for (int u = 0; u < 8; ++u)
+                    if (m0 + u < mid) acc += wv[u] * hid[m0 + u];
+            }
+            gate[ch] = 1.0f / (1.0f + expf(-acc));
+        }
+    }
+    __syncthreads();
+}
diff --git a/real-time-reid-tracking_amd/engine.py b/real-time-reid-tracking_amd/engine.py
--- a/real-time-reid-tracking_amd/engine.py
+++ b/real-time-reid-tracking_amd/engine.py
@@ -725,6 +725,22 @@
             _ptr(_f32(w2t)), _ptr(ya), _ptr(sa), _ptr(out), _ptr(o16), _ptr(gate)))
         return out, o16, gate
 
+    def debug_ds_tail(self, form, x16, w, scale, shift, y, stats, w1, w2t, stride=2, want_out=True):
+        x16 = np.ascontiguousarray(x16, np.uint16)
+        n, h, ww, c2 = x16.shape
+        w, y, stats = _f32(w), _f32(y), _f32(stats)
+        cout, cin = w.shape
+        if c2 != 2 * cin or y.shape[0] != n or y.shape[2] != cout or stats.shape[0] != n or stats.shape[2:] != (cout, 2):
+            raise ValueError("debug_ds_tail expects x16 [n, h, w, 2 cin], w [cout, cin], y [n, ho wo, cout], stats [n, tiles, cout, 2]")
+        hw = y.shape[1]
+        out = np.empty((n, hw, cout), np.float32) if want_out else None
+        o16 = np.empty((n * hw, 2 * cout), np.uint16)
+        check(_ffi.debug_lib().reid_debug_ds_tail(
+            self.h, C.c_int(form), C.c_int(n), C.c_int(h), C.c_int(ww), C.c_int(cin), C.c_int(cout), C.c_int(stride), C.c_int(w1.shape[0]),
+            C.c_int(stats.shape[1]), _ptr(x16), _ptr(w), _ptr(_f32(scale)), _ptr(_f32(shift)), _ptr(y), _ptr(stats), _ptr(_f32(w1)),
+            _ptr(_f32(w2t)), _ptr(out), _ptr(o16)))
+        return out, o16
+
     def debug_sibling_tail(self, arch, prm, y, shortcut):
         y, shortcut = _f32(y), _f32(shortcut)
         n, h, w, c = y.shape
```
